# MILAB-IIT-CV/ATDN_vSLAM

Measured on AMD Instinct MI355X. Metric: frame-pairs/sec, KITTI 1241x376 odometry inference at 1/2/4/8 MI355X, higher is better.
Workload: dtype f32 via 3xf16 split MFMA (fp32 accumulate); 1 GPU; KITTI seq-03-shaped 376x1241 uint8 frames (resident in HBM) resized to 376x1232, GMA flow 12 GRU iters + CLVO head -> 6-DoF trajectory (BASELINE configs[1]); streams_per_gpu=2, gru_iters=12, parallelism=pairs sharded x1, one all-gather of 512-d features, replicated LSTM scan

## Files before the change

### atdn_vslam_amd/_lib.py

```python
import ctypes as C
import os

_HERE = os.path.dirname(os.path.abspath(__file__))
LIB_PATH = os.environ.get("ATDN_LIB_PATH") or os.path.join(_HERE, "libatdn_hip.so")

_f32p = C.POINTER(C.c_float)
_i64p = C.POINTER(C.c_int64)
_vp = C.c_void_p

SIGNATURES = {
    "atdn_version": (C.c_int, []),
    "atdn_last_error": (C.c_char_p, []),
    "atdn_gma_create": (C.c_int, [C.POINTER(_vp), C.c_int, C.c_int, C.c_int, C.c_int]),
    "atdn_gma_set_low_latency": (C.c_int, [_vp, C.c_int]),
    "atdn_gma_load": (C.c_int, [_vp, C.c_char_p, _vp, _i64p, C.c_int]),
    "atdn_gma_finalize": (C.c_int, [_vp]),
    "atdn_gma_forward": (C.c_int, [_vp, _vp, _vp, C.c_int, C.c_int, _vp, _vp, _vp, _vp]),
    "atdn_gma_forward_predictions": (C.c_int, [_vp, _vp, _vp, C.c_int, C.c_int, _vp, _vp, _vp]),
    "atdn_gma_forward_sequence": (C.c_int, [_vp, _vp, C.c_int, C.c_int, _vp, _vp, _vp, _vp]),
    "atdn_gma_forward_sequence_continued": (C.c_int, [_vp, _vp, C.c_int, C.c_int, _vp, _vp, _vp, _vp]),
    "atdn_gma_debug_read": (C.c_long, [_vp, C.c_char_p, _vp, C.c_long, _vp]),
    "atdn_gma_profile": (C.c_int, [_vp, C.c_int, C.c_int, C.c_int, _f32p, _vp]),
    "atdn_gma_profile_mode": (C.c_int, [_vp, C.c_int, C.c_int, C.c_int, C.c_int, _f32p, _vp]),
    "atdn_gma_set_range_probe": (C.c_int, [_vp, C.c_int]),
    "atdn_gma_range_rows": (C.c_long, [_vp]),
    "atdn_gma_range_row": (C.c_int, [_vp, C.c_long, C.c_char_p, C.c_int, C.POINTER(C.c_int), C.POINTER(C.c_int), _f32p, _i64p, _i64p]),
    "atdn_range_probe": (C.c_int, [_vp, C.c_int64, C.c_int64, C.c_int64, _f32p, _i64p, _i64p, _vp]),
    "atdn_range_probe_launch": (C.c_int, [_vp, C.c_int64, C.c_int64, C.c_int64, _vp, _vp]),
    "atdn_gma_workspace_bytes": (C.c_size_t, [_vp]),
    "atdn_gma_destroy": (None, [_vp]),
    "atdn_clvo_create": (C.c_int, [C.POINTER(_vp), C.c_int, C.c_int, C.c_int]),
    "atdn_clvo_load": (C.c_int, [_vp, C.c_char_p, _vp, _i64p, C.c_int]),
    "atdn_clvo_finalize": (C.c_int, [_vp]),
    "atdn_clvo_encode": (C.c_int, [_vp, _vp, C.c_int, _vp, _vp]),
    "atdn_clvo_step": (C.c_int, [_vp, _vp, C.c_int, C.c_int, _vp, _vp, _vp, _vp]),
    "atdn_clvo_destroy": (None, [_vp]),
    "atdn_vae_create": (C.c_int, [C.POINTER(_vp), C.c_int, C.c_int, C.c_int]),
    "atdn_vae_load": (C.c_int, [_vp, C.c_char_p, _vp, _i64p, C.c_int]),
    "atdn_vae_finalize": (C.c_int, [_vp]),
    "atdn_vae_embedding_shape": (C.c_int, [_vp, C.POINTER(C.c_int), C.POINTER(C.c_int)]),
    "atdn_vae_encode": (C.c_int, [_vp, _vp, C.c_int, _vp, _vp]),
    "atdn_vae_destroy": (None, [_vp]),
    "atdn_clvo_trainer_create": (C.c_int, [C.POINTER(_vp), C.c_int, C.c_int, C.c_int, C.c_int]),
    "atdn_clvo_trainer_load": (C.c_int, [_vp, C.c_char_p, _vp, _i64p, C.c_int]),
    "atdn_clvo_trainer_finalize": (C.c_int, [_vp]),
    "atdn_clvo_trainer_forward_backward": (C.c_int, [_vp, _vp, _vp, _vp, _vp, _vp, _f32p, _vp]),
    "atdn_clvo_trainer_gradients": (C.c_int, [_vp, C.POINTER(_vp), C.POINTER(C.c_long)]),
    "atdn_clvo_trainer_adamw_step": (C.c_int, [_vp, C.c_float, C.c_float, C.c_float, C.c_int, _vp]),
    "atdn_clvo_trainer_set_loss": (C.c_int, [_vp, C.c_float, C.c_int, C.c_int]),
    "atdn_clvo_trainer_loss_terms": (C.c_int, [_vp, _f32p]),
    "atdn_clvo_loss": (C.c_int, [_vp, _vp, _vp, _vp, C.c_int, C.c_int, C.c_float, C.c_int, C.c_int, _f32p, _vp, _vp, _vp]),
    "atdn_clvo_trainer_read": (C.c_long, [_vp, C.c_char_p, C.c_int, _vp, C.c_long, _vp]),
    "atdn_clvo_trainer_destroy": (None, [_vp]),
    "atdn_pose_transform_f32": (C.c_int, [_vp, _vp, _vp]),
    "atdn_pose_rel2abs": (C.c_int, [_vp, _vp, C.c_int, _vp]),
    "atdn_pose_accumulate_f32": (C.c_int, [_vp, _vp, _vp]),
    "atdn_resize_frames": (C.c_int, [_vp, C.c_int, C.c_int, C.c_int, C.c_int, C.c_int, _vp, _vp]),
    "atdn_resize_frames_mode": (C.c_int, [_vp, C.c_int, C.c_int, C.c_int, C.c_int, C.c_int, C.c_int, _vp, _vp]),
    "atdn_resize_frames_u8": (C.c_int, [_vp, C.c_int, C.c_int, C.c_int, C.c_int, C.c_int, C.c_int, _vp, _vp]),
    "atdn_pad_frames": (C.c_int, [_vp, C.c_int, C.c_int, C.c_int, C.c_int, C.c_int, C.c_int, C.c_int, _vp, _vp]),
    "atdn_ingest_create": (C.c_int, [C.POINTER(_vp), C.c_int, C.c_int, C.c_int, C.c_int, C.c_int, C.c_int]),
    "atdn_ingest_frames_u8": (C.c_int, [_vp, _vp, C.c_int, _vp, _vp]),
    "atdn_ingest_destroy": (None, [_vp]),
    "atdn_flow_pack_f16": (C.c_int, [_vp, C.c_int, C.c_int, C.c_int, C.c_int, C.c_int, _vp, _vp]),
    "atdn_flow_gather_clips": (C.c_int, [_vp, C.c_int, C.c_int, C.c_int, _vp, _vp, C.c_int, C.c_int, _vp, _vp]),
    "atdn_map_search": (C.c_int, [_vp, C.c_int, C.c_int, _vp, C.c_int, C.c_int, _vp, _vp, _vp]),
    "atdn_map_gather_images_u8": (C.c_int, [_vp, C.c_int, C.c_long, _vp, C.c_int, _vp, _vp]),
    "atdn_corr_lookup": (C.c_int, [_vp, _vp, _vp, _vp, C.c_int, C.c_int, C.c_int, _vp, _vp, C.c_int, _vp]),
    "atdn_corr_pyramid": (C.c_int, [_vp, _vp, C.c_int, C.c_int, C.c_int, C.c_int, _vp, _vp, _vp, _vp, _vp]),
    "atdn_corr_lookup_bricks": (C.c_int, [_vp, _vp, C.c_int, C.c_int, C.c_int, C.c_int, _vp, _vp, _vp, _vp, _vp, _vp, _vp, _vp,
                                          _vp, _vp]),
    "atdn_conv2d_nhwc": (C.c_int, [_vp, C.c_int, C.c_int, C.c_int, C.c_int, _vp, _vp, C.c_int, C.c_int, C.c_int,
                                   C.c_int, C.c_int, C.c_int, C.c_int, _vp, _vp]),
    "atdn_conv2d_nhwc_sf": (C.c_int, [_vp, C.c_int, C.c_int, C.c_int, C.c_int, _vp, _vp, C.c_int, C.c_int, C.c_int,
                                      C.c_int, C.c_int, C.c_int, _vp, _vp]),
    "atdn_conv2d_nhwc_sf_epi": (C.c_int, [_vp, C.c_int, C.c_int, C.c_int, C.c_int, _vp, _vp, C.c_int, C.c_int, C.c_int,
                                      C.c_int, C.c_int, C.c_int, C.c_int, _vp, _vp]),
}

GMA_STAGES = ("fnet", "corr", "pool", "cnet", "attention", "lookup", "motion_encoder", "aggregate", "gru_zr", "gru_q",
              "flow_head", "mask", "gru_ctx", "attn_logits", "agg_vt", "convc1", "gru_zr_v", "gru_q_v")

_lib = None


def lib():
    global _lib
    if _lib is None:
        if not os.path.exists(LIB_PATH):
            raise RuntimeError(
                "%s is missing: the HIP extension has not been built (python -m atdn_vslam_amd.build). "
                "There is no CPU fallback for the product path." % LIB_PATH)
        import torch
        handle = C.CDLL(LIB_PATH)
        for name, (res, args) in SIGNATURES.items():
            fn = getattr(handle, name)
            fn.restype = res
            fn.argtypes = args
        _lib = handle
    return _lib


def check(rc):
    if rc != 0:
        raise RuntimeError("libatdn_hip: " + lib().atdn_last_error().decode("utf-8", "replace"))


def load_state(load_fn, handle, state):
    import numpy as np
    import torch
    for key, val in state.items():
        if isinstance(val, torch.Tensor):
            if not val.dtype.is_floating_point:
                continue
            arr = val.detach().to("cpu", torch.float32).contiguous().numpy()
        else:
            arr = np.asarray(val)
            if arr.dtype.kind != "f":
                continue
            arr = np.ascontiguousarray(arr, dtype=np.float32)
        shape = (C.c_int64 * max(arr.ndim, 1))(*arr.shape) if arr.ndim else (C.c_int64 * 1)(1)
        check(load_fn(handle, key.encode(), arr.ctypes.data_as(_vp), shape, arr.ndim))
```

### atdn_vslam_amd/csrc/capi.hip

```cpp
#include "../../include/atdn_hip.h"

#include <cmath>
#include <cstring>

#include "clvo.h"
#include "gma.h"
#include "vae.h"
#include "clvo_train.h"
#include "frontend.h"
#include "conv_sf.h"
#include "epilogues_sf.h"

namespace atdn {
extern template TileChoice conv_dispatch<MODE_TAP, EpiBias<ACT_NONE>>(const ConvShape&, EpiBias<ACT_NONE>, hipStream_t);
extern template TileChoice conv_dispatch<MODE_TAP, EpiBias<ACT_RELU>>(const ConvShape&, EpiBias<ACT_RELU>, hipStream_t);
extern template TileChoice conv_dispatch<MODE_ROW, EpiBias<ACT_NONE>>(const ConvShape&, EpiBias<ACT_NONE>, hipStream_t);
extern template TileChoice conv_dispatch<MODE_ROW, EpiBias<ACT_RELU>>(const ConvShape&, EpiBias<ACT_RELU>, hipStream_t);
extern template TileChoice conv_dispatch<MODE_TAP, EpiScale>(const ConvShape&, EpiScale, hipStream_t);

extern template TileChoice conv_sf_dispatch<EpiBias<ACT_NONE>>(const ConvShape&, float, EpiBias<ACT_NONE>, hipStream_t);
extern template TileChoice conv_sf_dispatch<SfBias<ACT_NONE>>(const ConvShape&, float, SfBias<ACT_NONE>, hipStream_t);

static thread_local std::string g_last_error;
void set_last_error(const std::string& msg) { g_last_error = msg; }
}

using namespace atdn;

struct atdn_gma { GmaNet net; atdn_gma(int H, int W, int B, int prec) : net(H, W, B, prec) {} };
struct atdn_clvo { ClvoNet net; atdn_clvo(int H, int W, int B) : net(H, W, B) {} };
struct atdn_vae { VaeEncoder net; atdn_vae(int H, int W, int B) : net(H, W, B) {} };
struct atdn_ingest { FrameIngest in; atdn_ingest(int a, int b, int c, int d, int n, int aa) : in(a, b, c, d, n, aa) {} };
struct atdn_clvo_trainer { ClvoTrainer net; atdn_clvo_trainer(int H, int W, int B, int T) : net(H, W, B, T) {} };

#define ATDN_API_BEGIN try {
#define ATDN_API_END                                      \
  return 0;                                               \
  } catch (const std::exception& e) {                     \
    set_last_error(e.what());                             \
    return 1;                                             \
  } catch (...) {                                         \
    set_last_error("unknown error");                      \
    return 1;                                             \
  }

template <class T>
static void euler_yxz(const T* r, T* R) {
  const T c1 = std::cos(r[0]), c2 = std::cos(r[1]), c3 = std::cos(r[2]);
  const T s1 = std::sin(r[0]), s2 = std::sin(r[1]), s3 = std::sin(r[2]);
  R[0] = c1 * c3 + s1 * s2 * s3; R[1] = c3 * s1 * s2 - c1 * s3; R[2] = c2 * s1;
  R[3] = c2 * s3;                R[4] = c2 * c3;                R[5] = -s2;
  R[6] = c1 * s2 * s3 - c3 * s1; R[7] = c1 * c3 * s2 + s1 * s3; R[8] = c1 * c2;
}
template <class T>
static void make_transform(const T* rot, const T* tr, T* m) {
  T R[9];
  euler_yxz(rot, R);
  for (int i = 0; i < 3; ++i) { for (int j = 0; j < 3; ++j) m[i * 4 + j] = R[i * 3 + j]; m[i * 4 + 3] = tr[i]; }
  m[12] = 0; m[13] = 0; m[14] = 0; m[15] = 1;
}
template <class T>
static void matmul4(const T* a, const T* b, T* c) {
  for (int i = 0; i < 4; ++i)
    for (int j = 0; j < 4; ++j) {
      T s = 0;
      for (int k = 0; k < 4; ++k) s += a[i * 4 + k] * b[k * 4 + j];
      c[i * 4 + j] = s;
    }
}

extern "C" {

int atdn_version(void) { return 100; }
const char* atdn_last_error(void) { return g_last_error.c_str(); }

int atdn_gma_create(atdn_gma** out, int H, int W, int max_batch, int precision) {
  ATDN_API_BEGIN
  ATDN_CHECK(out, "null out pointer");
  *out = new atdn_gma(H, W, max_batch, precision);
  ATDN_API_END
}
int atdn_gma_set_low_latency(atdn_gma* h, int on) {
  ATDN_API_BEGIN
  ATDN_CHECK(h, "null handle");
  h->net.set_low_latency(on != 0);
  ATDN_API_END
}
int atdn_gma_load(atdn_gma* h, const char* key, const float* data, const int64_t* shape, int rank) {
  ATDN_API_BEGIN
  ATDN_CHECK(h && key && data && rank >= 0 && rank <= 4, "bad state-dict entry");
  h->net.state().put(key, data, shape, rank);
  ATDN_API_END
}
int atdn_gma_finalize(atdn_gma* h) {
  ATDN_API_BEGIN
  ATDN_CHECK(h, "null handle");
  h->net.finalize();
  ATDN_API_END
}
int atdn_gma_forward(atdn_gma* h, const float* im1, const float* im2, int B, int iters, const float* flow_init,
                     float* flow_low, float* flow_up, void* stream) {
  ATDN_API_BEGIN
  ATDN_CHECK(h, "null handle");
  h->net.forward(im1, im2, B, iters, flow_init, flow_low, flow_up, (hipStream_t)stream);
  ATDN_API_END
}
int atdn_gma_forward_predictions(atdn_gma* h, const float* im1, const float* im2, int B, int iters, const float* flow_init,
                                 float* flow_predictions, void* stream) {
  ATDN_API_BEGIN
  ATDN_CHECK(h, "null handle");
  h->net.forward_predictions(im1, im2, B, iters, flow_init, flow_predictions, (hipStream_t)stream);
  ATDN_API_END
}
int atdn_gma_forward_sequence(atdn_gma* h, const float* frames, int B, int iters, const float* flow_init,
                              float* flow_low, float* flow_up, void* stream) {
  ATDN_API_BEGIN
  ATDN_CHECK(h, "null handle");
  h->net.forward_sequence(frames, B, iters, flow_init, flow_low, flow_up, (hipStream_t)stream);
  ATDN_API_END
}
int atdn_gma_forward_sequence_continued(atdn_gma* h, const float* frames, int B, int iters, const float* flow_init,
                                        float* flow_low, float* flow_up, void* stream) {
  ATDN_API_BEGIN
  ATDN_CHECK(h, "null handle");
  h->net.forward_sequence(frames, B, iters, flow_init, flow_low, flow_up, (hipStream_t)stream, true);
  ATDN_API_END
}
long atdn_gma_debug_read(atdn_gma* h, const char* name, float* host, long capacity, void* stream) {
  try {
    if (!h || !name || !host) throw Error("null argument");
    const long n = h->net.debug_read(name, host, capacity, (hipStream_t)stream);
    if (n < 0) throw Error(std::string("unknown tensor name: ") + name);
    return n;
  } catch (const std::exception& e) {
    set_last_error(e.what());
    return -1;
  }
}
int atdn_gma_profile(atdn_gma* h, int B, int iters, int reps, float* ms_out, void* stream) {
  ATDN_API_BEGIN
  ATDN_CHECK(h && ms_out, "null argument");
  static_assert(GmaNet::ST_COUNT == ATDN_GMA_STAGES, "stage table out of sync with the header");
  h->net.profile(B, iters, reps, ms_out, (hipStream_t)stream, 0);
  ATDN_API_END
}
int atdn_gma_profile_mode(atdn_gma* h, int B, int iters, int reps, int mode, float* ms_out, void* stream) {
  ATDN_API_BEGIN
  ATDN_CHECK(h && ms_out, "null argument");
  ATDN_CHECK(mode >= 0 && mode <= 2, "mode must be 0 (pair), 1 (sequence) or 2 (continued sequence)");
  h->net.profile(B, iters, reps, ms_out, (hipStream_t)stream, mode);
  ATDN_API_END
}
int atdn_gma_set_range_probe(atdn_gma* h, int on) {
  ATDN_API_BEGIN
  ATDN_CHECK(h, "null handle");
  h->net.set_probe(on != 0);
  ATDN_API_END
}
long atdn_gma_range_rows(atdn_gma* h) {
  if (!h) { set_last_error("null handle"); return -1; }
  return (long)h->net.probe_rows().size();
}
int atdn_gma_range_row(atdn_gma* h, long index, char* name, int name_capacity, int* iteration, int* limited, float* max_abs,
                       int64_t* over, int64_t* nonfinite) {
// ... 172 lines not shown
  } catch (...) { loss3.release(); throw; }
  loss3.release();
  ATDN_API_END
}
long atdn_clvo_trainer_read(atdn_clvo_trainer* h, const char* key, int kind, float* host, long capacity, void* stream) {
  try {
    ATDN_CHECK(h && key && host, "null argument");
    return h->net.read(key, kind, host, capacity, (hipStream_t)stream);
  } catch (const std::exception& e) {
    set_last_error(e.what());
    return -1;
  }
}
void atdn_clvo_trainer_destroy(atdn_clvo_trainer* h) { delete h; }

int atdn_pose_transform_f32(const float* rot, const float* tr, float* mat16) {
  ATDN_API_BEGIN
  ATDN_CHECK(rot && tr && mat16, "null argument");
  make_transform(rot, tr, mat16);
  ATDN_API_END
}
int atdn_pose_rel2abs(const float* rot, const float* tr, int T, double* poses) {
  ATDN_API_BEGIN
  ATDN_CHECK(rot && tr && poses && T >= 0, "bad argument");
  for (int i = 0; i < 16; ++i) poses[i] = (i % 5 == 0) ? 1.0 : 0.0;
  for (int t = 0; t < T; ++t) {
    const double r[3] = {rot[t * 3], rot[t * 3 + 1], rot[t * 3 + 2]};
    const double x[3] = {tr[t * 3], tr[t * 3 + 1], tr[t * 3 + 2]};
    double m[16];
    make_transform(r, x, m);
    matmul4(poses + (long)t * 16, m, poses + (long)(t + 1) * 16);
  }
  ATDN_API_END
}
int atdn_pose_accumulate_f32(float* pose16, const float* rot, const float* tr) {
  ATDN_API_BEGIN
  ATDN_CHECK(pose16 && rot && tr, "null argument");
  float m[16], o[16];
  make_transform(rot, tr, m);
  matmul4(pose16, m, o);
  for (int i = 0; i < 16; ++i) pose16[i] = o[i];
  ATDN_API_END
}

int atdn_corr_lookup(const float* pyr0, const float* pyr1, const float* pyr2, const float* pyr3, int B, int H8,
                     int W8, const float* coords, float* out, int ldo, void* stream) {
  ATDN_API_BEGIN
  ATDN_CHECK(pyr0 && pyr1 && pyr2 && pyr3 && coords && out && B >= 1, "null argument");
  ATDN_CHECK((H8 >> 3) >= 2 && (W8 >> 3) >= 2, "map too small for four pyramid levels");
  PyramidLevels pl;
  const float* b[4] = {pyr0, pyr1, pyr2, pyr3};
  for (int l = 0; l < 4; ++l) { pl.base[l] = b[l]; pl.H[l] = H8 >> l; pl.W[l] = W8 >> l; }
  launch_lookup(pl, coords, (long)B * H8 * W8, out, ldo, (hipStream_t)stream);
  ATDN_API_END
}

int atdn_corr_pyramid(const float* fmap1, const float* fmap2, int B, int H8, int W8, int C, float* pyr0, float* pyr1,
                      float* pyr2, float* pyr3, void* stream) {
  ATDN_API_BEGIN
  ATDN_CHECK(fmap1 && fmap2 && pyr0 && pyr1 && pyr2 && pyr3 && B >= 1 && C % 32 == 0, "bad argument");
  const int N = H8 * W8;
  ConvShape c;
  c.src0 = fmap1; c.ld0 = C; c.sb0 = (long)N * C; c.C0 = C; c.H = 1; c.W = N;
  c.w = fmap2; c.wb = (long)N * C; c.ldw = C; c.N = N; c.nimg = B;
  conv_dispatch<MODE_TAP>(c, EpiScale{1.0f / sqrtf((float)C), pyr0, (long)N * N, N}, (hipStream_t)stream);
  float* p[4] = {pyr0, pyr1, pyr2, pyr3};
  for (int l = 1; l < 4; ++l) launch_avgpool(p[l - 1], H8 >> (l - 1), W8 >> (l - 1), p[l], (long)B * N, (hipStream_t)stream);
  ATDN_API_END
}

int atdn_corr_lookup_bricks(const float* fmap1, const float* fmap2, int B, int H8, int W8, int C, const float* coords,
                            float* pyr0, float* pyr1, float* pyr2, float* pyr3, float* samples,
                            const float* convc1_weight_host, const float* convc1_bias_host, float* cor1, void* stream) {
  ATDN_API_BEGIN
  ATDN_CHECK(fmap1 && fmap2 && B >= 1 && H8 >= 1 && W8 >= 1, "bad argument");
  ATDN_CHECK(C == 256, "the correlation kernel keeps a source strip's whole K = 256 in registers: C must be 256");
  ATDN_CHECK((H8 >> 3) >= 2 && (W8 >> 3) >= 2, "map too small for four pyramid levels");
  ATDN_CHECK(!(samples || cor1) || coords, "a lookup needs coordinates");
  ATDN_CHECK(!cor1 || (convc1_weight_host && convc1_bias_host), "cor1 needs convc1's weight [256][324] and bias [256]");
  hipStream_t st = (hipStream_t)stream;
  const int N = H8 * W8;
  const long n8 = (long)B * N;
  BrickPyramid bp;
  bp.N = N; bp.NPB = brick_pixel_blocks(N);
  DeviceBuf f1, f2, plain[3], fbrick[4], pyr[4], scratch, outsf;
  DeviceBuf* all[] = {&f1, &f2, &plain[0], &plain[1], &plain[2], &fbrick[0], &fbrick[1], &fbrick[2], &fbrick[3],
                      &pyr[0], &pyr[1], &pyr[2], &pyr[3], &scratch, &outsf};
  WeightArena A;
  try {
    sf_counter_attach();
    f1.alloc(n8 * 256); f2.alloc(n8 * 256);
    launch_to_sf(fmap1, f1.p, n8, 256, st);
    launch_to_sf(fmap2, f2.p, n8, 256, st);
    float* rowmajor[4] = {pyr0, pyr1, pyr2, pyr3};
    int pH[4], pW[4];
    for (int l = 0; l < 4; ++l) {
      pH[l] = H8 >> l; pW[l] = W8 >> l;
      bp.H[l] = pH[l]; bp.W[l] = pW[l]; bp.BW[l] = cdiv(pW[l], 8); bp.BH[l] = cdiv(pH[l], 4); bp.NB[l] = bp.BW[l] * bp.BH[l] * 32;
      const float* src = f2.p;
      long src_sb = (long)N * 256;
      if (l > 0) {
        const float* prev = l == 1 ? f2.p : plain[l - 2].p;
        const long prev_sb = l == 1 ? (long)N * 256 : (long)pH[l - 1] * pW[l - 1] * 256;
        src_sb = (long)pH[l] * pW[l] * 256;
        plain[l - 1].alloc((long)B * src_sb);
        launch_pool_features_sf(prev, B, pH[l - 1], pW[l - 1], 256, prev_sb, plain[l - 1].p, src_sb, st);
        src = plain[l - 1].p;
      }
      fbrick[l].alloc((long)B * bp.NB[l] * 256);
      launch_brick_rows(src, src_sb, B, pH[l], pW[l], 256, fbrick[l].p, (long)bp.NB[l] * 256, st);
      pyr[l].alloc((long)B * bp.NPB * kBrickPixelBlock * bp.NB[l]);
      launch_corr_bricks(f1.p, (long)N * 256, fbrick[l].p, (long)bp.NB[l] * 256, B, N, bp.NB[l], 1.0f / sqrtf(256.0f), pyr[l].p, false, st);
      bp.base[l] = pyr[l].p;
      if (rowmajor[l]) launch_unbrick(pyr[l].p, bp.NB[l], N, pH[l], pW[l], n8, rowmajor[l], st);
    }
    if (samples) {
      outsf.alloc(n8 * 352);
      launch_lookup_bricks(bp, coords, n8, outsf.p, st);
      scratch.alloc(n8 * 352);
      launch_from_sf(outsf.p, scratch.p, n8, 352, st);
      ATDN_HIP(hipMemcpy2DAsync(samples, 324 * sizeof(float), scratch.p, 352 * sizeof(float), 324 * sizeof(float), (size_t)n8,
                                hipMemcpyDeviceToDevice, st));
    }
    if (cor1) {
      StateDict sd;
      const int64_t ws[4] = {256, 324, 1, 1}, bs[1] = {256};
      sd.put("c.weight", convc1_weight_host, ws, 4);
      sd.put("c.bias", convc1_bias_host, bs, 1);
      PackedConv L = pack_conv_sf(A, sd, {"c"});
      pack_fragment_major16(A, L);
      A.upload();
      resolve(A, L);
      DeviceBuf csf;
      csf.alloc(n8 * 256);
      try {
        launch_lookup_conv(bp, coords, n8, nullptr, L.wf16, L.wscale, L.b, csf.p, false, st);
        launch_from_sf(csf.p, cor1, n8, 256, st);
        ATDN_HIP(hipStreamSynchronize(st));
      } catch (...) { csf.release(); throw; }
      csf.release();
    }
    ATDN_HIP(hipStreamSynchronize(st));
  } catch (...) {
    (void)hipDeviceSynchronize();
    for (auto* b : all) b->release();
    A.release();
    throw;
  }
  for (auto* b : all) b->release();
  A.release();
  ATDN_API_END
}

int atdn_conv2d_nhwc(const float* src, int nimg, int H, int W, int Cin, const float* weight_host,
                     const float* bias_host, int Cout, int KH, int KW, int stride, int padH, int padW, int relu,
                     float* dst, void* stream) {
  ATDN_API_BEGIN
  ATDN_CHECK(src && weight_host && dst && nimg >= 1, "null argument");
  const bool row = (Cin == 4 || Cin == 16);
  ATDN_CHECK(row || Cin % 32 == 0, "Cin must be 4, 16 or a multiple of 32");
  StateDict sd;
  const int64_t ws[4] = {Cout, Cin, KH, KW};
  sd.put("c.weight", weight_host, ws, 4);
  std::vector<float> zb(Cout, 0.f);
  const int64_t bs[1] = {Cout};
  sd.put("c.bias", bias_host ? bias_host : zb.data(), bs, 1);
  WeightArena A;
  PackedConv L = pack_conv(A, sd, {"c"}, row ? MODE_ROW : MODE_TAP, Cin);
  A.upload();
  resolve(A, L);
  ConvShape s;
  s.src0 = src; s.ld0 = Cin; s.sb0 = (long)H * W * Cin; s.C0 = L.C; s.H = H; s.W = W;
  s.KH = KH; s.KW = KW; s.stride = stride; s.padH = padH; s.padW = padW;
  s.w = L.w; s.ldw = L.ldw; s.N = Cout; s.nimg = nimg;
  const int Ho = conv_out(H, KH, stride, padH), Wo = conv_out(W, KW, stride, padW);
  hipStream_t st = (hipStream_t)stream;
  try {
    if (row) {
      if (relu) conv_dispatch<MODE_ROW>(s, EpiBias<ACT_RELU>{L.b, dst, (long)Ho * Wo * Cout, Cout, 1.f}, st);
      else conv_dispatch<MODE_ROW>(s, EpiBias<ACT_NONE>{L.b, dst, (long)Ho * Wo * Cout, Cout, 1.f}, st);
    } else {
      if (relu) conv_dispatch<MODE_TAP>(s, EpiBias<ACT_RELU>{L.b, dst, (long)Ho * Wo * Cout, Cout, 1.f}, st);
      else conv_dispatch<MODE_TAP>(s, EpiBias<ACT_NONE>{L.b, dst, (long)Ho * Wo * Cout, Cout, 1.f}, st);
    }
    ATDN_HIP(hipStreamSynchronize(st));
  } catch (...) {
    A.release();
    throw;
  }
  A.release();
  ATDN_API_END
}

int atdn_resize_frames(const float* src, int planes, int Hin, int Win, int Hout, int Wout, float* dst, void* stream) {
  return atdn_resize_frames_mode(src, planes, Hin, Win, Hout, Wout, ATDN_RESIZE_ANTIALIAS, dst, stream);
}
int atdn_resize_frames_mode(const float* src, int planes, int Hin, int Win, int Hout, int Wout, int antialias, float* dst,
                            void* stream) {
  ATDN_API_BEGIN
  ATDN_CHECK(src && dst && planes >= 1 && Hin >= 1 && Win >= 1 && Hout >= 1 && Wout >= 1, "bad argument");
  ATDN_CHECK(antialias == 0 || antialias == 1, "antialias must be ATDN_RESIZE_BILINEAR or ATDN_RESIZE_ANTIALIAS");
  launch_resize<float>(src, planes, Hin, Win, Hout, Wout, antialias, dst, (hipStream_t)stream);
  ATDN_API_END
}
int atdn_resize_frames_u8(const uint8_t* src, int planes, int Hin, int Win, int Hout, int Wout, int antialias, float* dst,
                          void* stream) {
  ATDN_API_BEGIN
  ATDN_CHECK(src && dst && planes >= 1 && Hin >= 1 && Win >= 1 && Hout >= 1 && Wout >= 1, "bad argument");
  ATDN_CHECK(antialias == 0 || antialias == 1, "antialias must be ATDN_RESIZE_BILINEAR or ATDN_RESIZE_ANTIALIAS");
  launch_resize<unsigned char>(src, planes, Hin, Win, Hout, Wout, antialias, dst, (hipStream_t)stream);
  ATDN_API_END
}
int atdn_pad_frames(const float* src, int planes, int H, int W, int left, int right, int top, int bottom, float* dst,
                    void* stream) {
  ATDN_API_BEGIN
  ATDN_CHECK(src && dst && planes >= 1 && H >= 1 && W >= 1 && left >= 0 && right >= 0 && top >= 0 && bottom >= 0, "bad argument");
  launch_pad_replicate(src, planes, H, W, left, right, top, bottom, dst, (hipStream_t)stream);
  ATDN_API_END
}
int atdn_ingest_create(atdn_ingest** out, int Hin, int Win, int Hout, int Wout, int max_frames, int antialias) {
  ATDN_API_BEGIN
  ATDN_CHECK(out, "null out pointer");
  ATDN_CHECK(antialias == 0 || antialias == 1, "antialias must be ATDN_RESIZE_BILINEAR or ATDN_RESIZE_ANTIALIAS");
  *out = new atdn_ingest(Hin, Win, Hout, Wout, max_frames, antialias);
  ATDN_API_END
}
int atdn_ingest_frames_u8(atdn_ingest* h, const uint8_t* host_frames, int n_frames, float* dst, void* stream) {
  ATDN_API_BEGIN
  ATDN_CHECK(h, "null handle");
  h->in.ingest(host_frames, n_frames, dst, (hipStream_t)stream);
  ATDN_API_END
}
void atdn_ingest_destroy(atdn_ingest* h) { delete h; }

int atdn_conv2d_nhwc_sf_epi(const float* src, int nimg, int H, int W, int Cin, const float* weight_host,
                            const float* bias_host, int Cout, int KH, int KW, int stride, int padH, int padW, int sf_store,
                            float* dst, void* stream) {
  ATDN_API_BEGIN
  ATDN_CHECK(src && weight_host && dst && nimg >= 1 && Cin % 32 == 0, "bad argument (Cin must be a multiple of 32)");
  ATDN_CHECK(!sf_store || Cout % 32 == 0, "the split-f16 store needs Cout % 32 == 0");
  StateDict sd;
  const int64_t ws[4] = {Cout, Cin, KH, KW};
  sd.put("c.weight", weight_host, ws, 4);
  std::vector<float> zb(Cout, 0.f);
  const int64_t bs[1] = {Cout};
  sd.put("c.bias", bias_host ? bias_host : zb.data(), bs, 1);
  WeightArena A;
  PackedConv L = pack_conv_sf(A, sd, {"c"});
  A.upload();
  resolve(A, L);
  hipStream_t st = (hipStream_t)stream;
  float* tmp = nullptr;
  const long rows = (long)nimg * H * W;
  ATDN_HIP(hipMalloc(&tmp, (size_t)rows * Cin * sizeof(float)));
  try {
    launch_to_sf(src, tmp, rows, Cin, st);
    ConvShape s;
    s.src0 = tmp; s.ld0 = Cin; s.sb0 = (long)H * W * Cin; s.C0 = L.C; s.H = H; s.W = W;
    s.KH = KH; s.KW = KW; s.stride = stride; s.padH = padH; s.padW = padW;
    s.w = L.w; s.ldw = L.ldw; s.N = Cout; s.nimg = nimg;
    const int Ho = conv_out(H, KH, stride, padH), Wo = conv_out(W, KW, stride, padW);
    s.wfrag16 = L.wf16;
    if (sf_store) {
      float* osf = nullptr;
      const long orows = (long)nimg * Ho * Wo;
      ATDN_HIP(hipMalloc(&osf, (size_t)orows * Cout * sizeof(float)));
      try {
        conv_sf_dispatch(s, L.wscale, SfBias<ACT_NONE>{L.b, osf, (long)Ho * Wo * Cout, Cout}, st);
        launch_from_sf(osf, dst, orows, Cout, st);
        ATDN_HIP(hipStreamSynchronize(st));
      } catch (...) {
        (void)hipFree(osf);
        throw;
      }
      (void)hipFree(osf);
    } else {
      conv_sf_dispatch(s, L.wscale, EpiBias<ACT_NONE>{L.b, dst, (long)Ho * Wo * Cout, Cout, 1.f}, st);
      ATDN_HIP(hipStreamSynchronize(st));
    }
  } catch (...) {
    (void)hipFree(tmp);
    A.release();
    throw;
  }
  (void)hipFree(tmp);
  A.release();
  ATDN_API_END
}

int atdn_conv2d_nhwc_sf(const float* src, int nimg, int H, int W, int Cin, const float* weight_host,
                        const float* bias_host, int Cout, int KH, int KW, int stride, int padH, int padW, float* dst,
                        void* stream) {
  return atdn_conv2d_nhwc_sf_epi(src, nimg, H, W, Cin, weight_host, bias_host, Cout, KH, KW, stride, padH, padW, 0, dst, stream);
}

}
```

### atdn_vslam_amd/csrc/conv_sf6.h

```cpp
#pragma once
#include <cstdlib>
#include <type_traits>
#include "conv_sf.h"

namespace atdn {

struct Conv2Geom {
  const float* src0; const float* src1;
  long sb0, sb1;
  int ld0, ld1, C0, C1;
  int H, W, Ho, Wo;
  int KH, KW, padH, padW;
  int PH, PW;
  int tiles_x, tiles_y;
  int nimg, ntile_n;
  const float* w; int ldw; int N;
  float wscale;
  const float* in_mean; const float* in_rstd;
};

inline bool conv_halo_eligible(const ConvShape& s) {
  if (s.stride != 1 || s.wb != 0) return false;
  return (s.KH == 3 && s.KW == 3) || (s.KH == 1 && s.KW == 5) || (s.KH == 5 && s.KW == 1);
}

template <class E, class = void> struct epi_gen6 : std::integral_constant<int, 0> {};
template <class E> struct epi_gen6<E, std::void_t<decltype(E::kGen6)>> : std::integral_constant<int, E::kGen6> {};
template <class E, class = void> struct EpiAux4 { struct type {}; };
template <class E> struct EpiAux4<E, std::void_t<typename E::Aux4>> { using type = typename E::Aux4; };
template <class E, class = void> struct epi_flowhead : std::false_type {};
template <class E> struct epi_flowhead<E, std::void_t<decltype(E::kFlowHead)>> : std::bool_constant<E::kFlowHead> {};
template <class E, class = void> struct epi_ring3 : std::false_type {};
template <class E> struct epi_ring3<E, std::void_t<decltype(E::kRing3)>> : std::bool_constant<E::kRing3> {};
template <class E, class = void> struct epi_rawacc : std::false_type {};
template <class E> struct epi_rawacc<E, std::void_t<decltype(E::kRawAcc)>> : std::bool_constant<E::kRawAcc> {};
template <class E, class = void> struct epi_vec4 : std::false_type {};
template <class E> struct epi_vec4<E, std::void_t<decltype(E::kVec4)>> : std::bool_constant<E::kVec4> {};

typedef float f32x4v __attribute__((ext_vector_type(4)));
struct SfAcc { f32x4v b[2][2]; };

#ifdef ATDN_CONV_STAMP
#define ATDN_CONV_STAMP_SLOTS 4096
extern __device__ unsigned long long atdn_conv_stamps_dev[4][ATDN_CONV_STAMP_SLOTS][12];
template <class E> struct conv_stamp_kind : std::integral_constant<int, -1> {};
#endif

template <int TH, int TW, int BN, int WM, int WN, int KH, int KW, class Epi, bool FAST = false, bool NORM = false, int ABL = 0>
__device__ __forceinline__ void conv_sf6_body(const Conv2Geom& g, const Epi& ep, const int bidx) {
  static_assert(ABL == 0 || !NORM, "ablation builds exist for the plain patch loader");
  static_assert(TW == 16, "the 16x16x32 loop is built for 16-pixel tile rows");
  constexpr int NIMG = 2;
  constexpr int NW = WM * WN, NT = NW * 64;
  constexpr int TM = TH * TW / 32 / WM, TN = BN / 32 / WN;
  static_assert(TM * WM * 32 == TH * TW && TN * WN * 32 == BN, "wave grid must tile the block");
  static_assert(32 % TW == 0 || TW % 32 == 0, "a 32-pixel MFMA row tile must cover whole tile rows");
  constexpr int NTAP = KH * KW;
  constexpr int RSTEP = NT / 8;
  constexpr int PROWS = (TH + KH - 1) * (TW + KW - 1);
  constexpr int PW = TW + KW - 1;
  constexpr int NP = (PROWS + RSTEP - 1) / RSTEP;
  constexpr int ROWB = 160;
  constexpr int RS = PW * ROWB;
  constexpr bool SWAP = epi_vec4<Epi>::value;
  constexpr int PSZ = (TH + KH - 1) * RS;
  __shared__ __attribute__((aligned(256))) char Pbytes[NIMG * PSZ];

  const int tid = threadIdx.x;
  const int tiles_img = g.tiles_x * g.tiles_y;
  const int nblk = g.nimg * tiles_img * g.ntile_n;
  const int id = xcd_remap(bidx, nblk);
  const int tile_n = id % g.ntile_n;
  const int tmg = id / g.ntile_n;
  const int img = tmg / tiles_img;
  const int tloc = tmg - img * tiles_img;
  const int ty0 = (tloc / g.tiles_x) * TH, tx0 = (tloc % g.tiles_x) * TW;
  const int n0 = tile_n * BN;
  const int lane = tid & 63, wave = tid >> 6;
#ifdef ATDN_CONV_STAMP
  constexpr int kStamp = conv_stamp_kind<Epi>::value;
  unsigned long long st_r0 = 0, st_t0 = 0, st_t1 = 0, st_t2 = 0, st_bar = 0;
  unsigned long long st_e_slab = 0, st_e_wait = 0, st_e_apply = 0;
  if constexpr (kStamp >= 0) { st_r0 = __builtin_amdgcn_s_memrealtime(); st_t0 = __builtin_amdgcn_s_memtime(); }
#endif

  const int jrow = (tid >> 3) & 7;
  const int s = tid & 7, r0 = !NORM ? tid >> 3 : ((tid >> 6) << 3) + 2 * (jrow & 1) + ((jrow >> 1) & 1) + 4 * (jrow >> 2);
  static_assert((TH + KH - 1) * RS / 16 <= 4096, "LDS offset field");
  unsigned pmeta[NP];
#pragma unroll
  for (int k = 0; k < NP; ++k) {
    const int prow = r0 + RSTEP * k;
    unsigned off = 0;
    const int py = prow / PW, px = prow - py * PW;
    if (prow < PROWS) {
      const int iy = ty0 - g.padH + py, ix = tx0 - g.padW + px;
      if ((unsigned)iy < (unsigned)g.H && (unsigned)ix < (unsigned)g.W) off = (unsigned)(iy * g.W + ix) + 1u;
    }
    pmeta[k] = (off << 12) | (unsigned)((py * RS + px * ROWB + 16 * s) >> 4);
    if (prow >= PROWS) pmeta[k] = pmeta[0];
  }
  const float* s0 = g.src0 + (long)img * g.sb0;
  const float* s1 = g.src1 ? g.src1 + (long)img * g.sb1 : nullptr;
  const int nck = (g.C0 + g.C1) >> 5;

  float4 pr[NP];
  auto fetch_patch = [&](int c) {
    const int cc = c << 5;
    const float* sp; int ld, co;
    if (cc < g.C0) { sp = s0; ld = g.ld0; co = cc; } else { sp = s1; ld = g.ld1; co = cc - g.C0; }
#pragma unroll
    for (int k = 0; k < NP; ++k)
      pr[k] = *reinterpret_cast<const float4*>(sp + (long)((pmeta[k] >> 12) ? (pmeta[k] >> 12) - 1 : 0) * ld + co + 4 * s);
  };
  auto store_patch = [&](int buf) {
#pragma unroll
    for (int k = 0; k < NP; ++k)
      *reinterpret_cast<float4*>(Pbytes + buf * PSZ + ((pmeta[k] & 0xFFFu) << 4)) = keep_if((pmeta[k] >> 12) != 0, pr[k]);
  };
  float4 nmu = make_float4(0.f, 0.f, 0.f, 0.f), nrs = make_float4(1.f, 1.f, 1.f, 1.f);
  auto fetch_norm = [&](int c) {
    nmu = *reinterpret_cast<const float4*>(g.in_mean + (long)img * g.C0 + (c << 5) + 4 * s);
    nrs = *reinterpret_cast<const float4*>(g.in_rstd + (long)img * g.C0 + (c << 5) + 4 * s);
  };
  bool norm_sat = false;
  auto store_row_norm = [&](int buf, int k, float4 mu, float4 rs) {
    const float hi = (pmeta[k] >> 12) != 0 ? 65504.f : 0.f;
    float4 v = pr[k];
    v.x = (v.x - mu.x) * rs.x; v.y = (v.y - mu.y) * rs.y; v.z = (v.z - mu.z) * rs.z; v.w = (v.w - mu.w) * rs.w;
    const float m = fmaxf(fmaxf(v.x, v.y), fmaxf(v.z, v.w));
    norm_sat |= !(m <= 65504.f);
    v.x = __builtin_amdgcn_fmed3f(v.x, 0.f, hi); v.y = __builtin_amdgcn_fmed3f(v.y, 0.f, hi);
    v.z = __builtin_amdgcn_fmed3f(v.z, 0.f, hi); v.w = __builtin_amdgcn_fmed3f(v.w, 0.f, hi);
    const unsigned h0 = sf_cvt_pk_(v.x, v.y), h1 = sf_cvt_pk_(v.z, v.w);
    const unsigned l0 = sf_residual_pk_(h0, v.x, v.y), l1 = sf_residual_pk_(h1, v.z, v.w);
    char* px = Pbytes + buf * PSZ + (((pmeta[k] & 0xFFFu) - (unsigned)s) << 4);
    *reinterpret_cast<uint2*>(px + 8 * s) = make_uint2(h0, h1);
    *reinterpret_cast<uint2*>(px + 64 + 8 * s) = make_uint2(l0, l1);
  };

  const int wm = wave / WN, wn = wave % WN;
  SfAcc acc[TM][TN];
#pragma unroll
  for (int i = 0; i < TM; ++i)
#pragma unroll
    for (int j = 0; j < TN; ++j) {
#pragma unroll
      for (int e = 0; e < 16; ++e) acc[i][j].b[e >> 3][(e >> 2) & 1][e & 3] = 0.f;
    }
  {
    const int n16 = lane & 15, g16 = lane >> 4;
    int a_off[TM];
#pragma unroll
    for (int i = 0; i < TM; ++i) a_off[i] = ((wm * TM + i) * 2) * RS + n16 * ROWB + 16 * g16;
    const char* Pb = Pbytes;
    const int nblk16 = (g.N + 15) >> 4;
    const float* wrow[TN][2];
#pragma unroll
    for (int j = 0; j < TN; ++j)
#pragma unroll
      for (int cb = 0; cb < 2; ++cb)
        wrow[j][cb] = g.w + (long)min(((n0 >> 4) + (wn * TN + j) * 2 + cb), nblk16 - 1) * (NTAP * nck) * 512 + lane * 4;
    constexpr int RT = (NTAP % 3 == 0 || epi_ring3<Epi>::value) ? 3 : 2;
    constexpr int CU = (NTAP % RT == 0) ? 1 : RT;
    constexpr int NS = CU * NTAP;
    static_assert(NS % RT == 0, "ring size must divide the K steps of an unrolled iteration");
    struct WFrag { f16x8 hi[TN][2], lo[TN][2]; };
    WFrag wr[RT];
    auto load_w = [&](WFrag& f, int c0, int st, int cb) __attribute__((always_inline)) {
      const int cc = min(c0 + st / NTAP, nck - 1);
      const int q = (st % NTAP) * nck + cc;
#pragma unroll
      for (int j = 0; j < TN; ++j) {
        f.hi[j][cb] = *reinterpret_cast<const f16x8*>(wrow[j][cb] + (long)q * 512);
        if constexpr (!FAST) f.lo[j][cb] = *reinterpret_cast<const f16x8*>(wrow[j][cb] + (long)q * 512 + 256);
      }
    };
    fetch_patch(0);
    if constexpr (NORM) fetch_norm(0);
#pragma unroll
    for (int st = 0; st < RT - 1; ++st) { load_w(wr[st], 0, st, 0); load_w(wr[st], 0, st, 1); }
    if constexpr ((ABL & 1) != 0) { load_w(wr[RT - 1], 0, RT - 1, 0); load_w(wr[RT - 1], 0, RT - 1, 1); }
    if constexpr (NORM) {
#pragma unroll
      for (int k = 0; k < NP; ++k) store_row_norm(0, k, nmu, nrs);
    } else {
      store_patch(0);
    }
    __syncthreads();
#ifdef ATDN_CONV_STAMP
    if constexpr (kStamp >= 0) st_t1 = __builtin_amdgcn_s_memtime();
#endif
    f16x8 ah[2][TM], al[2][TM];
    auto read_a = [&](int half, int tap) __attribute__((always_inline)) {
      const char* arow = Pb + (tap / KW + half) * RS + (tap % KW) * ROWB;
#pragma unroll
      for (int i = 0; i < TM; ++i) {
        ah[half][i] = *reinterpret_cast<const f16x8*>(arow + a_off[i]);
        if constexpr (!FAST) al[half][i] = *reinterpret_cast<const f16x8*>(arow + a_off[i] + 64);
      }
    };
    auto mfma_half = [&](int half, const WFrag& w) __attribute__((always_inline)) {
#pragma unroll
      for (int i = 0; i < TM; ++i)
#pragma unroll
        for (int j = 0; j < TN; ++j)
#pragma unroll
          for (int cb = 0; cb < 2; ++cb) {
            f32x4v c = acc[i][j].b[half][cb];
            if constexpr (SWAP) {
              if constexpr (!FAST) {
                c = __builtin_amdgcn_mfma_f32_16x16x32_f16(w.hi[j][cb], al[half][i], c, 0, 0, 0);
                c = __builtin_amdgcn_mfma_f32_16x16x32_f16(w.lo[j][cb], ah[half][i], c, 0, 0, 0);
              }
              c = __builtin_amdgcn_mfma_f32_16x16x32_f16(w.hi[j][cb], ah[half][i], c, 0, 0, 0);
            } else {
              if constexpr (!FAST) {
                c = __builtin_amdgcn_mfma_f32_16x16x32_f16(al[half][i], w.hi[j][cb], c, 0, 0, 0);
                c = __builtin_amdgcn_mfma_f32_16x16x32_f16(ah[half][i], w.lo[j][cb], c, 0, 0, 0);
              }
              c = __builtin_amdgcn_mfma_f32_16x16x32_f16(ah[half][i], w.hi[j][cb], c, 0, 0, 0);
            }
            acc[i][j].b[half][cb] = c;
          }
    };
    constexpr int NMF = (FAST ? 1 : 3) * TM * TN * 2;
    constexpr int NH = 2 * NTAP;
    static_assert(!NORM || NH - 1 - NP >= 1, "normalise-on-load spreads its NP patch rows over the half-steps of a chunk");
    read_a(0, 0);
    if constexpr (KH != 3 || !Epi::kStats) __builtin_amdgcn_s_setprio(2);
    for (int c0 = 0; c0 < nck; c0 += CU) {
#pragma unroll
      for (int cu = 0; cu < CU; ++cu) {
        const int c = c0 + cu;
        const bool live = CU == 1 || c < nck;
        const int cn = min(c + 1, nck - 1);
#pragma unroll
        for (int hs = 0; hs < NH; ++hs) {
          const int tap = hs >> 1, half = hs & 1;
          const int st = cu * NTAP + tap;
          __builtin_amdgcn_sched_barrier(0);
          if (!(ABL & 2) && hs == 0) { fetch_patch(cn); if constexpr (NORM) fetch_norm(cn); }
          if (!(ABL & 1)) {
            if (RT == 2) { if (half == 0) { load_w(wr[(st + 1) % RT], c0, st + 1, 0); load_w(wr[(st + 1) % RT], c0, st + 1, 1); } }
            else load_w(wr[(st + RT - 1) % RT], c0, st + RT - 1, half);
          }
          if (!(ABL & 4) && hs + 1 < NH) read_a((hs + 1) & 1, (hs + 1) >> 1);
          if constexpr (NORM) {
            if (hs >= NH - 1 - NP && hs <= NH - 2) store_row_norm((c + 1) & 1, hs - (NH - 1 - NP), nmu, nrs);
          } else {
            if (!(ABL & 2) && hs == NH - 2) store_patch((c + 1) & 1);
          }
          if (live) mfma_half(half, wr[st % RT]);
          {
            constexpr int nds = 2 * TM;
            const int nvm = (RT == 2 ? (half == 0 ? 4 * TN : 0) : 2 * TN) + (hs == 0 ? NP : 0);
            const int ndw = NORM ? ((hs >= NH - 1 - NP && hs <= NH - 2) ? 2 : 0) : ((hs == NH - 2) ? NP : 0);
#pragma unroll
            for (int k = 0; k < NMF; ++k) {
              __builtin_amdgcn_sched_group_barrier(0x008, 1, 0);
              if (hs + 1 < NH && k < nds) __builtin_amdgcn_sched_group_barrier(0x100, 1, 0);
              else if (k - ((hs + 1 < NH) ? nds : 0) < nvm) __builtin_amdgcn_sched_group_barrier(0x020, 1, 0);
              else if (k - ((hs + 1 < NH) ? nds : 0) - nvm < ndw) __builtin_amdgcn_sched_group_barrier(0x200, 1, 0);
            }
          }
        }
        if (!(ABL & 2)) {
#ifdef ATDN_CONV_STAMP
          unsigned long long st_b0 = 0;
          if constexpr (kStamp >= 0) { asm volatile("s_waitcnt lgkmcnt(0)" ::: "memory"); st_b0 = __builtin_amdgcn_s_memtime(); }
#endif
          asm volatile("s_waitcnt lgkmcnt(0)\n\ts_barrier" ::: "memory");
#ifdef ATDN_CONV_STAMP
          if constexpr (kStamp >= 0) st_bar += __builtin_amdgcn_s_memtime() - st_b0;
#endif
          Pb = Pbytes + ((c + 1) & 1) * PSZ;
        }
        if (!(ABL & 4)) read_a(0, 0);
      }
    }
  }

#ifdef ATDN_CONV_STAMP
  if constexpr (kStamp >= 0) st_t2 = __builtin_amdgcn_s_memtime();
  auto stamp_out = [&]() __attribute__((always_inline)) {
    if constexpr (kStamp >= 0) {
      asm volatile("s_waitcnt vmcnt(0) lgkmcnt(0)" ::: "memory");
      const unsigned long long t3 = __builtin_amdgcn_s_memtime(), r1 = __builtin_amdgcn_s_memrealtime();
      const unsigned hw = __builtin_amdgcn_s_getreg((31 << 11) | 4), xcc = __builtin_amdgcn_s_getreg((31 << 11) | 20);
      if (wave == 0 && lane == 0 && bidx < ATDN_CONV_STAMP_SLOTS) {
        unsigned long long* o = atdn_conv_stamps_dev[kStamp * 2 + (KH == 5 ? 1 : 0)][bidx];
        o[0] = st_r0; o[1] = r1; o[2] = st_t1 - st_t0; o[3] = st_t2 - st_t1; o[4] = st_bar; o[5] = t3 - st_t2;
        o[6] = ((unsigned long long)xcc << 32) | hw; o[7] = t3 - st_t0;
        o[8] = st_e_slab; o[9] = st_e_wait; o[10] = st_e_apply; o[11] = 0;
      }
    }
  };
#endif
  if constexpr (KH != 3 || !Epi::kStats) __builtin_amdgcn_s_setprio(0);
  if constexpr (NORM) sf_report(norm_sat);
  if constexpr ((ABL & 8) != 0) {
    float tot = 0.f;
#pragma unroll
    for (int i = 0; i < TM; ++i)
#pragma unroll
      for (int j = 0; j < TN; ++j)
#pragma unroll
        for (int e = 0; e < 16; ++e) tot += acc[i][j].b[e >> 3][(e >> 2) & 1][e & 3];
    if (tot == 1.2345e-30f) ep(img, 0, 0, tot);
    return;
  }
  if constexpr (SWAP) {
    static_assert(NW * 32 * LDS_LD * 4 <= NIMG * PSZ, "transpose slabs must fit in the patch images");
    __syncthreads();
    float* tb = reinterpret_cast<float*>(Pbytes) + wave * (32 * LDS_LD);
    const int trow = lane >> 3, tcol = (lane & 7) * 4;
    auto tile_pixel = [&](int i, int q) {
      const int p = (wm * TM + i) * 32 + 8 * q + trow;
      const int oy = ty0 + p / TW, ox = tx0 + p % TW;
      if constexpr ((ABL & 16) != 0) return p;
      return (oy < g.Ho && ox < g.Wo) ? oy * g.Wo + ox : -1;
    };
    constexpr bool RAW = epi_rawacc<Epi>::value && !epi_flowhead<Epi>::value;
    auto slab_write = [&](const SfAcc& a) __attribute__((always_inline)) {
      const float sc = RAW ? 1.0f : g.wscale;
#pragma unroll
      for (int hh = 0; hh < 2; ++hh)
#pragma unroll
        for (int cb = 0; cb < 2; ++cb)
          *reinterpret_cast<float4*>(tb + (16 * hh + (lane & 15)) * LDS_LD + 16 * cb + 4 * (lane >> 4)) =
              RAW ? make_float4(a.b[hh][cb][0], a.b[hh][cb][1], a.b[hh][cb][2], a.b[hh][cb][3])
                  : make_float4(a.b[hh][cb][0] * sc, a.b[hh][cb][1] * sc, a.b[hh][cb][2] * sc, a.b[hh][cb][3] * sc);
    };
    if constexpr (epi_flowhead<Epi>::value) {
      static_assert(!epi_flowhead<Epi>::value || (WM == 1 && TN == 1 && TW == 16), "one block holds all output channels of its pixels");
      constexpr int RP = 20;
      static_assert(32 * RP <= 32 * LDS_LD, "the exchange rows live inside the wave's slab");
      {
        const int n16 = lane & 15, g16 = lane >> 4;
        const int c8 = n0 + wn * 32 + 8 * g16;
        const float4 bq0 = *reinterpret_cast<const float4*>(ep.bias + c8), bq1 = *reinterpret_cast<const float4*>(ep.bias + c8 + 4);
        const float b8[8] = {bq0.x, bq0.y, bq0.z, bq0.w, bq1.x, bq1.y, bq1.z, bq1.w};
        f16x8 w2h[2], w2l[2];
#pragma unroll
        for (int rbk = 0; rbk < 2; ++rbk) {
          const int u = 16 * rbk + n16;
          const float* wr = ep.w2 + (long)min(u, 17) * g.N + c8;
          const float4 wa = *reinterpret_cast<const float4*>(wr), wb = *reinterpret_cast<const float4*>(wr + 4);
          const float w8[8] = {wa.x, wa.y, wa.z, wa.w, wb.x, wb.y, wb.z, wb.w};
#pragma unroll
          for (int e = 0; e < 8; ++e) {
            const float w = u < 18 ? w8[e] * ep.w2mul : 0.f;
            w2h[rbk][e] = (_Float16)w;
            w2l[rbk][e] = (_Float16)(w - (float)w2h[rbk][e]);
          }
        }
        bool sat = false;
#pragma unroll
        for (int i = 0; i < TM; ++i) {
          slab_write(acc[i][0]);
          asm volatile("s_waitcnt lgkmcnt(0)" ::: "memory");
          __builtin_amdgcn_wave_barrier();
          f16x8 xh[2], xl[2];
#pragma unroll
          for (int pb = 0; pb < 2; ++pb) {
            const float* src = tb + (16 * pb + n16) * LDS_LD + 8 * g16;
            const float4 xa = *reinterpret_cast<const float4*>(src), xb = *reinterpret_cast<const float4*>(src + 4);
            const float x8[8] = {xa.x, xa.y, xa.z, xa.w, xb.x, xb.y, xb.z, xb.w};
#pragma unroll
            for (int e = 0; e < 8; ++e) {
              const SfPair sp = sf_split_flag(fmaxf(x8[e] + b8[e], 0.f), sat);
              xh[pb][e] = sp.hi; xl[pb][e] = sp.lo;
            }
          }
          asm volatile("s_waitcnt lgkmcnt(0)" ::: "memory");
          __builtin_amdgcn_wave_barrier();
#pragma unroll
          for (int pb = 0; pb < 2; ++pb) {
            f32x4v d0 = {0.f, 0.f, 0.f, 0.f}, d1 = {0.f, 0.f, 0.f, 0.f};
            if constexpr (!FAST) {
              d0 = __builtin_amdgcn_mfma_f32_16x16x32_f16(w2h[0], xl[pb], d0, 0, 0, 0);
              d0 = __builtin_amdgcn_mfma_f32_16x16x32_f16(w2l[0], xh[pb], d0, 0, 0, 0);
              d1 = __builtin_amdgcn_mfma_f32_16x16x32_f16(w2h[1], xl[pb], d1, 0, 0, 0);
              d1 = __builtin_amdgcn_mfma_f32_16x16x32_f16(w2l[1], xh[pb], d1, 0, 0, 0);
            }
            d0 = __builtin_amdgcn_mfma_f32_16x16x32_f16(w2h[0], xh[pb], d0, 0, 0, 0);
            d1 = __builtin_amdgcn_mfma_f32_16x16x32_f16(w2h[1], xh[pb], d1, 0, 0, 0);
            float* rp = tb + (16 * pb + n16) * RP;
            *reinterpret_cast<float4*>(rp + 4 * g16) = make_float4(d0[0] * ep.w2inv, d0[1] * ep.w2inv, d0[2] * ep.w2inv, d0[3] * ep.w2inv);
            if (g16 == 0) *reinterpret_cast<float2*>(rp + 16) = make_float2(d1[0] * ep.w2inv, d1[1] * ep.w2inv);
          }
          __syncthreads();
          for (int idx = tid; idx < 32 * 18; idx += NT) {
            const int px = idx / 18, u = idx - px * 18;
            const float* rq = reinterpret_cast<const float*>(Pbytes) + px * RP + u;
            float sum = 0.f;
#pragma unroll
            for (int w = 0; w < NW; ++w) sum += rq[w * (32 * LDS_LD)];
            const int p = i * 32 + px;
            const int oy = ty0 + p / TW, ox = tx0 + p % TW;
            if (oy < g.Ho && ox < g.Wo)
              ep.G[(long)(n0 / (NW * 32)) * ep.gstride + ((long)img * ep.npix + (long)oy * g.Wo + ox) * 18 + u] = sum;
          }
          __syncthreads();
// ... 430 lines not shown
```

### atdn_vslam_amd/csrc/gma.h

```cpp
#pragma once
#include <vector>
#include <map>
#include <memory>

#include "attention.h"
#include "conv_dispatch.h"
#include "kernels.h"
#include "range_probe.h"
#include "weights.h"

namespace atdn {

struct EncoderWeights {
  PackedConv stem;
  struct Block { PackedConv c1, c2, ds; bool has_ds = false; } blk[6];
  PackedConv head;
};

class DeviceBuf {
 public:
  float* p = nullptr;
  long n = 0;
  void alloc(long count) {
    n = count;
    ATDN_HIP(hipMalloc(&p, (size_t)count * sizeof(float)));
  }
  void release() { if (p) { (void)hipFree(p); p = nullptr; } }
};

class GmaNet {
 public:
  GmaNet(int H, int W, int max_batch, int precision);
  ~GmaNet();
  StateDict& state() { return sd_; }
  void finalize();
  void forward(const float* im1, const float* im2, int B, int iters, const float* flow_init, float* flow_low,
               float* flow_up, hipStream_t st);
  void forward_predictions(const float* im1, const float* im2, int B, int iters, const float* flow_init, float* preds,
                           hipStream_t st);
  void forward_sequence(const float* frames, int B, int iters, const float* flow_init, float* flow_low, float* flow_up,
                        hipStream_t st, bool continued = false);
  long debug_read(const char* name, float* host, long capacity, hipStream_t st);
  size_t workspace_bytes() const { return ws_bytes_; }
  enum Stage { ST_FNET = 0, ST_CORR, ST_POOL, ST_CNET, ST_ATTN, ST_LOOKUP, ST_MOTION, ST_AGG, ST_GRU_ZR, ST_GRU_Q, ST_FLOWHEAD,
               ST_MASK, ST_GRU_CTX, ST_ATTN_LOGITS, ST_AGG_VT, ST_CONVC1, ST_GRU_ZR_V, ST_GRU_Q_V, ST_COUNT };
  void profile(int B, int iters, int reps, float* ms, hipStream_t st, int mode = 0);

  int H, W, H8, W8, N, ldN, maxB, precision;
  int dev_ = 0;
  bool norm_on_load_ = false;
  bool classic_ = false;
  bool low_latency_ = false;
  void set_low_latency(bool on);
  DeviceBuf attn_part_;
  DeviceBuf enc2_[4];
  hipStream_t par_stream_ = nullptr;
  std::vector<hipEvent_t> par_events_;
  size_t par_next_ = 0;
  bool par_ = false;
  bool par_ok_ = true;
  void fork(hipStream_t from, hipStream_t to);
  DeviceBuf fbrick_[4], fplain_[3], coords_used_;
  int brickBW_[4], brickBH_[4], brickNB_[4];
  BrickPyramid brick_pyramid() const;
  DeviceBuf rowmax_, rinv_;

  struct ProbeRow { std::string name; int iter; bool limited; float max_abs; long long over, nonfinite; };
  static constexpr int kProbeMaxRows = 1536;
  void set_probe(bool on);
  const std::vector<ProbeRow>& probe_rows() const { return probe_rows_; }

 private:
  bool probe_ = false;
  int probe_it_ = -1;
  RangeSlot* probe_slots_ = nullptr;
  std::vector<ProbeRow> probe_rows_;
  void probe_begin(hipStream_t st);
  void probe_end(hipStream_t st);
  void probe(const std::string& name, bool limited, const float* p, long rows, long cols, long ld, hipStream_t st);
  void run_body(int B, int iters, hipStream_t st);
  void run_encoder(const EncoderWeights& E, bool instance, int nimg, hipStream_t st, float** out_buf, int* outH,
                   int* outW);
  void iteration(int B, hipStream_t st);
  void run_body_sf(int B, int iters, hipStream_t st);
  void run_encoder_sf(const EncoderWeights& E, bool instance, int nimg, hipStream_t st, float** out_buf, int first_img = 0,
                      DeviceBuf* bufs = nullptr);
  void iteration_sf(int B, hipStream_t st);
  void capture(int B, int iters);
  void launch_body(int B, int iters, hipStream_t st);
  int seq_ = 0;
  int last_frame_ = -1;
  float* preds_out_ = nullptr;
  long preds_stride_ = 0;
  void mask_head_sf(int B, hipStream_t st);
  void mask_head(int B, hipStream_t st);
  int last_B_ = 0;

  StateDict sd_;
  WeightArena arena_;
  bool ready_ = false;
  bool use_graph_ = true;
  EncoderWeights fnet_, cnet_;
  PackedConv convc1_, convc2_, convf1_, convf2_, convm_, to_v_, to_qk_;
  long convf1_sf_off_ = -1;
  float convf1_wscale_ = 1.f;
  float fh2_mul_ = 1.f;
  long fh2_w32_off_ = -1;
  DeviceBuf fhG_;
  PackedConv gru_zr_[2], gru_q_[2], fh1_, fh2_, mask0_, mask2_;
  PackedConv gru_zr_ctx_[2], gru_q_ctx_[2];
  const float* gamma_ = nullptr;
  long gamma_off_ = -1;

  DeviceBuf img4_, enc_[4], scratch_, pcnt_, fin_, fmap_, psum_, pm2_, mean_[3], rstd_[3];
  DeviceBuf pyr_[4], h_[2], x_, qk_, attn_, vT_, corrfeat_, cor1_, corflo_, flo1_, z_, rh_, fh_, mask_;
  DeviceBuf coords1_, flow4_, pre_zr_[2], pre_q_[2];
  int pyrH_[4], pyrW_[4];
  size_t ws_bytes_ = 0;

  struct Timer;
  Timer* timer_ = nullptr;
  void mark(int stage, hipStream_t st);

  hipStream_t cap_stream_ = nullptr;
  std::map<std::pair<int, int>, hipGraphExec_t> graphs_;
};

}
```

### atdn_vslam_amd/csrc/gma.hip

```cpp
#include "gma.h"
#include "small_convs.h"
#include "conv_sf.h"
#include "epilogues_sf.h"

namespace atdn { const float* zero_line(); }

namespace atdn {

extern template TileChoice conv_dispatch<MODE_TAP, EpiBias<ACT_NONE>>(const ConvShape&, EpiBias<ACT_NONE>, hipStream_t);
extern template TileChoice conv_dispatch<MODE_TAP, EpiBias<ACT_RELU>>(const ConvShape&, EpiBias<ACT_RELU>, hipStream_t);
extern template TileChoice conv_dispatch<MODE_ROW, EpiBias<ACT_RELU>>(const ConvShape&, EpiBias<ACT_RELU>, hipStream_t);
extern template TileChoice conv_dispatch<MODE_TAP, EpiBiasStats>(const ConvShape&, EpiBiasStats, hipStream_t);
extern template TileChoice conv_dispatch<MODE_ROW, EpiBiasStats>(const ConvShape&, EpiBiasStats, hipStream_t);
extern template TileChoice conv_dispatch<MODE_TAP, EpiBiasReluAddRelu>(const ConvShape&, EpiBiasReluAddRelu, hipStream_t);
extern template TileChoice conv_dispatch<MODE_TAP, EpiContextSplit>(const ConvShape&, EpiContextSplit, hipStream_t);
extern template TileChoice conv_dispatch<MODE_TAP, EpiScale>(const ConvShape&, EpiScale, hipStream_t);
extern template TileChoice conv_dispatch<MODE_TAP, EpiQK>(const ConvShape&, EpiQK, hipStream_t);
extern template TileChoice conv_dispatch<MODE_TAP, EpiStoreT>(const ConvShape&, EpiStoreT, hipStream_t);
extern template TileChoice conv_dispatch<MODE_TAP, EpiAggregate>(const ConvShape&, EpiAggregate, hipStream_t);
extern template TileChoice conv_dispatch<MODE_TAP, EpiGruZR>(const ConvShape&, EpiGruZR, hipStream_t);
extern template TileChoice conv_dispatch<MODE_TAP, EpiGruQ>(const ConvShape&, EpiGruQ, hipStream_t);
extern template TileChoice conv_dispatch<MODE_TAP, EpiFlowDelta>(const ConvShape&, EpiFlowDelta, hipStream_t);

extern template TileChoice conv_dispatch<MODE_ROW, SfBias<ACT_RELU>>(const ConvShape&, SfBias<ACT_RELU>, hipStream_t);
#define ATDN_EXTERN_SF(EPI) extern template TileChoice conv_sf_dispatch<EPI>(const ConvShape&, float, EPI, hipStream_t);
ATDN_EXTERN_SF(SfBias<ACT_NONE>) ATDN_EXTERN_SF(SfBias<ACT_RELU>) ATDN_EXTERN_SF(EpiBias<ACT_NONE>)
ATDN_EXTERN_SF(EpiBiasStats) ATDN_EXTERN_SF(SfBiasReluAddRelu) ATDN_EXTERN_SF(SfContextSplit)
ATDN_EXTERN_SF(SfQK) ATDN_EXTERN_SF(SfVT)
ATDN_EXTERN_SF(SfGruZR) ATDN_EXTERN_SF(SfGruQ)
extern template void conv_sf_dispatch_pair<SfBias<ACT_RELU>>(const ConvShape&, float, SfBias<ACT_RELU>, const ConvShape&, float,
                                                             SfBias<ACT_RELU>, hipStream_t);

namespace {

struct FastGuard {
  bool prev;
  explicit FastGuard(bool on) : prev(sf_fast_mode()) { sf_fast_mode() = on; }
  ~FastGuard() { sf_fast_mode() = prev; }
};

constexpr int XLD = 384;
constexpr int CORR_LD = 352;

ConvShape conv_shape(const PackedConv& L, const float* src, int ld, long sb, int nimg, int H, int W, int stride,
                     int padH, int padW) {
  ConvShape s;
  s.src0 = src; s.ld0 = ld; s.sb0 = sb; s.C0 = L.C;
  s.H = H; s.W = W; s.KH = L.KH; s.KW = L.KW; s.stride = stride; s.padH = padH; s.padW = padW;
  s.w = L.w; s.wfrag16 = L.wf16; s.ldw = L.ldw; s.N = L.N; s.nimg = nimg;
  return s;
}

EncoderWeights pack_encoder(WeightArena& A, const StateDict& sd, const std::string& p, bool batchnorm, bool sf) {
  EncoderWeights E;
  auto fold = [&](const std::string& norm) { return bn_affine(sd, norm); };
  auto pack_conv = [&](WeightArena& A_, const StateDict& sd_, const std::vector<std::string>& names, int mode, int cpix,
                       const ChannelAffine* f = nullptr) {
    return (sf && mode == MODE_TAP) ? pack_conv_sf(A_, sd_, names, f) : atdn::pack_conv(A_, sd_, names, mode, cpix, f);
  };
  if (batchnorm) { auto a = fold(p + "norm1"); E.stem = pack_conv(A, sd, {p + "conv1"}, MODE_ROW, 4, &a); }
  else E.stem = pack_conv(A, sd, {p + "conv1"}, MODE_ROW, 4);
  if (sf) pack_stem_sf(A, E.stem);
  int bi = 0;
  for (int li = 1; li <= 3; ++li)
    for (int k = 0; k < 2; ++k, ++bi) {
      const std::string q = p + "layer" + std::to_string(li) + "." + std::to_string(k) + ".";
      auto& B = E.blk[bi];
      B.has_ds = (li > 1 && k == 0);
      if (batchnorm) {
        auto a1 = fold(q + "norm1"), a2 = fold(q + "norm2");
        B.c1 = pack_conv(A, sd, {q + "conv1"}, MODE_TAP, 0, &a1);
        B.c2 = pack_conv(A, sd, {q + "conv2"}, MODE_TAP, 0, &a2);
        if (B.has_ds) { auto a3 = fold(q + "norm3"); B.ds = pack_conv(A, sd, {q + "downsample.0"}, MODE_TAP, 0, &a3); }
      } else {
        B.c1 = pack_conv(A, sd, {q + "conv1"}, MODE_TAP, 0);
        B.c2 = pack_conv(A, sd, {q + "conv2"}, MODE_TAP, 0);
        if (B.has_ds) B.ds = pack_conv(A, sd, {q + "downsample.0"}, MODE_TAP, 0);
      }
    }
  E.head = pack_conv(A, sd, {p + "conv2"}, MODE_TAP, 0);
  return E;
}

void resolve_encoder(const WeightArena& A, EncoderWeights& E) {
  resolve(A, E.stem);
  for (auto& b : E.blk) { resolve(A, b.c1); resolve(A, b.c2); if (b.has_ds) resolve(A, b.ds); }
  resolve(A, E.head);
}

}

struct GmaNet::Timer {
  std::vector<std::pair<int, hipEvent_t>> marks;
  hipEvent_t start = nullptr;
};

void GmaNet::mark(int stage, hipStream_t st) {
  if (!timer_) return;
  hipEvent_t e;
  ATDN_HIP(hipEventCreate(&e));
  ATDN_HIP(hipEventRecord(e, st));
  timer_->marks.emplace_back(stage, e);
}

void GmaNet::profile(int B, int iters, int reps, float* ms, hipStream_t st, int mode) {
  ATDN_CHECK(ready_ && B >= 1 && B <= maxB && reps >= 1, "bad profile request");
  ATDN_CHECK(mode == 0 || precision >= 1, "sequence modes are built for the split-f16 pipeline");
  ATDN_CHECK(!probe_, "switch the range probe off before profiling: its launches would be timed with the stages");
  for (int i = 0; i < ST_COUNT; ++i) ms[i] = 0.f;
  seq_ = mode;
  last_frame_ = 0;
  for (int r = 0; r < reps; ++r) {
    Timer t;
    timer_ = &t;
    if (precision >= 1) launch_init_coords_sf(nullptr, B, H8, W8, coords1_.p, flow4_.p, x_.p, XLD, 254, st);
    else launch_init_coords(nullptr, B, H8, W8, coords1_.p, flow4_.p, x_.p + 254, XLD, st);
    ATDN_HIP(hipEventCreate(&t.start));
    ATDN_HIP(hipEventRecord(t.start, st));
    try { if (precision >= 1) { FastGuard fg(precision == 2); run_body_sf(B, iters, st); } else run_body(B, iters, st); } catch (...) { timer_ = nullptr; throw; }
    timer_ = nullptr;
    ATDN_HIP(hipStreamSynchronize(st));
    hipEvent_t prev = t.start;
    for (auto& m : t.marks) {
      float d = 0.f;
      ATDN_HIP(hipEventElapsedTime(&d, prev, m.second));
      ms[m.first] += d;
      prev = m.second;
    }
    for (auto& m : t.marks) (void)hipEventDestroy(m.second);
    (void)hipEventDestroy(t.start);
  }
}

GmaNet::GmaNet(int H_, int W_, int max_batch, int precision_) : H(H_), W(W_), maxB(max_batch), precision(precision_) {
  ATDN_CHECK(precision >= 0 && precision <= 2, "precision must be 0 (fp32 MFMA), 1 (split-f16 MFMA) or 2 (plain f16 MFMA)");
  ATDN_CHECK(H % 8 == 0 && W % 8 == 0 && H >= 64 && W >= 64, "frame size must be a multiple of 8 (use the padder)");
  ATDN_CHECK(max_batch >= 1 && max_batch <= 64, "max_batch out of range");
  H8 = H / 8; W8 = W / 8; N = H8 * W8; ldN = round_up(N, 32);
  norm_on_load_ = precision == 1;
  classic_ = precision == 0;
  const char* ng = getenv("ATDN_NO_GRAPH");
  use_graph_ = !(ng && ng[0] == '1');
  (void)hipGetDevice(&dev_);
}

void GmaNet::fork(hipStream_t from, hipStream_t to) {
  ATDN_CHECK(par_next_ < par_events_.size(), "out of branch events");
  hipEvent_t e = par_events_[par_next_++];
  ATDN_HIP(hipEventRecord(e, from));
  ATDN_HIP(hipStreamWaitEvent(to, e, 0));
}

void GmaNet::set_low_latency(bool on) {
  ATDN_CHECK(!ready_, "set_low_latency: call it before finalize() (the workspace and the captured graphs depend on it)");
  low_latency_ = on;
}

GmaNet::~GmaNet() {
  DeviceGuard dg(dev_);
  (void)hipDeviceSynchronize();
  for (auto& kv : graphs_) (void)hipGraphExecDestroy(kv.second);
  if (cap_stream_) (void)hipStreamDestroy(cap_stream_);
  if (par_stream_) (void)hipStreamDestroy(par_stream_);
  for (auto& e : par_events_) (void)hipEventDestroy(e);
  DeviceBuf* all[] = {&img4_, &enc_[0], &enc_[1], &enc_[2], &enc_[3], &scratch_, &pcnt_, &fin_, &fmap_, &psum_, &pm2_, &mean_[0], &mean_[1], &mean_[2], &rstd_[0],
                      &rstd_[1], &rstd_[2], &pyr_[0], &pyr_[1], &pyr_[2], &pyr_[3], &h_[0], &h_[1], &x_, &qk_, &attn_, &vT_,
                      &corrfeat_, &cor1_, &corflo_, &flo1_, &z_, &rh_, &fh_, &mask_, &coords1_, &flow4_, &pre_zr_[0],
                      &pre_zr_[1], &pre_q_[0], &pre_q_[1], &rowmax_, &rinv_,
                      &fbrick_[0], &fbrick_[1], &fbrick_[2], &fbrick_[3], &fplain_[0], &fplain_[1], &fplain_[2], &coords_used_, &fhG_,
                      &attn_part_, &enc2_[0], &enc2_[1], &enc2_[2], &enc2_[3]};
  for (auto* b : all) b->release();
  if (probe_slots_) (void)hipFree(probe_slots_);
  arena_.release();
}

void GmaNet::set_probe(bool on) {
  ATDN_CHECK(!on || precision == 0,
             "the range probe needs an exact-fp32 handle (ATDN_PRECISION_F32): only that path writes every intermediate tensor "
             "as plain fp32 and never clamps; the split-f16 / f16 paths store range-limited values and fuse some tensors away");
  probe_ = on;
}

void GmaNet::probe_begin(hipStream_t st) {
  if (!probe_slots_) ATDN_HIP(hipMalloc(&probe_slots_, kProbeMaxRows * sizeof(RangeSlot)));
  ATDN_HIP(hipMemsetAsync(probe_slots_, 0, kProbeMaxRows * sizeof(RangeSlot), st));
  probe_rows_.clear();
  probe_it_ = -1;
}

void GmaNet::probe(const std::string& name, bool limited, const float* p, long rows, long cols, long ld, hipStream_t st) {
  ATDN_CHECK((int)probe_rows_.size() < kProbeMaxRows, "range probe: slot table full");
  launch_range_probe(p, rows, cols, ld, probe_slots_ + probe_rows_.size(), st);
  probe_rows_.push_back({name, probe_it_, limited, 0.f, 0, 0});
}

void GmaNet::probe_end(hipStream_t st) {
  std::vector<RangeSlot> host(probe_rows_.size());
  if (!host.empty())
    ATDN_HIP(hipMemcpyAsync(host.data(), probe_slots_, host.size() * sizeof(RangeSlot), hipMemcpyDeviceToHost, st));
  ATDN_HIP(hipStreamSynchronize(st));
  for (size_t i = 0; i < host.size(); ++i) {
    ProbeRow& r = probe_rows_[i];
    static_assert(sizeof(float) == sizeof(unsigned int), "fp32");
    memcpy(&r.max_abs, &host[i].max_bits, sizeof(float));
    r.over = (long long)host[i].over;
    r.nonfinite = (long long)host[i].nonfinite;
  }
}

void GmaNet::finalize() {
  ATDN_CHECK(!ready_, "finalize called twice");
  const std::string u = "update_block.";
  const bool sf = precision >= 1;
  auto tap = [&](const std::vector<std::string>& names, bool has_bias = true) {
    return sf ? pack_conv_sf(arena_, sd_, names, nullptr, has_bias)
              : pack_conv(arena_, sd_, names, MODE_TAP, 0, nullptr, has_bias);
  };
  fnet_ = pack_encoder(arena_, sd_, "fnet.", false, sf);
  cnet_ = pack_encoder(arena_, sd_, "cnet.", true, sf);
  convc1_ = tap({u + "encoder.convc1"});
  if (sf) pack_fragment_major16(arena_, convc1_);
  convc2_ = tap({u + "encoder.convc2"});
  convf1_ = pack_conv(arena_, sd_, {u + "encoder.convf1"}, MODE_ROW, 4);
  {
    const HostTensor& w = sd_.get(u + "encoder.convf1.weight");
    ATDN_CHECK(w.shape[0] == 128 && w.shape[1] == 2 && w.shape[2] == 7 && w.shape[3] == 7, "convf1 is 7x7, 2 -> 128");
    float mx = 0.f;
    for (float v : w.data) mx = std::max(mx, std::fabs(v));
    int e = 0;
    if (mx > 0.f) (void)std::frexp(mx, &e);
    const int p = 1 - e;
    convf1_wscale_ = std::ldexp(1.0f, -p);
    convf1_sf_off_ = arena_.alloc(4L * 2 * 4 * 2 * 64 * 4);
    _Float16* f = reinterpret_cast<_Float16*>(arena_.at(convf1_sf_off_));
    for (int wv = 0; wv < 4; ++wv)
      for (int cb = 0; cb < 2; ++cb)
        for (int s = 0; s < 4; ++s)
          for (int lane = 0; lane < 64; ++lane)
            for (int i = 0; i < 8; ++i) {
              const int n = 32 * wv + 16 * cb + (lane & 15), g = lane >> 4;
              const int ky = 2 * s + (g >> 1), kx = 4 * (g & 1) + (i >> 1), c = i & 1;
              const float v = (ky < 7 && kx < 7) ? std::ldexp(w.data[(((long)n * 2 + c) * 7 + ky) * 7 + kx], p) : 0.f;
              const _Float16 hi = (_Float16)v, lo = (_Float16)(v - (float)hi);
              const long frag = (((long)wv * 2 + cb) * 4 + s) * 2;
              f[(frag * 64 + lane) * 8 + i] = hi;
              f[((frag + 1) * 64 + lane) * 8 + i] = lo;
            }
  }
  convf2_ = tap({u + "encoder.convf2"});
  convm_ = tap({u + "encoder.conv"});
  to_v_ = tap({u + "aggregator.to_v"}, false);
  to_qk_ = tap({"att.to_qk"}, false);
  for (int p = 0; p < 2; ++p) {
    const std::string t = std::to_string(p + 1);
    if (sf) {
      const std::vector<std::pair<int, int>> rest = {{0, 128}, {256, 512}}, ctx = {{128, 256}};
      gru_zr_[p] = pack_conv_sf_channels(arena_, sd_, {u + "gru.convz" + t, u + "gru.convr" + t}, rest, true);
      gru_q_[p] = pack_conv_sf_channels(arena_, sd_, {u + "gru.convq" + t}, rest, true);
      gru_zr_ctx_[p] = pack_conv_sf_channels(arena_, sd_, {u + "gru.convz" + t, u + "gru.convr" + t}, ctx, false);
      gru_q_ctx_[p] = pack_conv_sf_channels(arena_, sd_, {u + "gru.convq" + t}, ctx, false);
    } else {
      gru_zr_[p] = tap({u + "gru.convz" + t, u + "gru.convr" + t});
      gru_q_[p] = tap({u + "gru.convq" + t});
    }
  }
  fh1_ = tap({u + "flow_head.conv1"});
  fh2_ = tap({u + "flow_head.conv2"});
  if (sf) {
    const HostTensor& w = sd_.get(u + "flow_head.conv2.weight");
    ATDN_CHECK(w.shape.size() == 4 && w.shape[0] == 2 && w.shape[1] == 256 && w.shape[2] == 3 && w.shape[3] == 3, "flow head conv2 shape");
    fh2_w32_off_ = arena_.alloc(18 * 256);
    for (int o = 0; o < 2; ++o)
      for (int c = 0; c < 256; ++c)
        for (int t = 0; t < 9; ++t) arena_.at(fh2_w32_off_)[(t * 2 + o) * 256 + c] = w.data[((long)o * 256 + c) * 9 + t];
    float mx = 0.f;
    for (float v : w.data) mx = std::max(mx, std::fabs(v));
    int e = 0;
    if (mx > 0.f) (void)std::frexp(mx, &e);
    fh2_mul_ = std::ldexp(1.0f, 1 - e);
  }
  mask0_ = tap({u + "mask.0"});
  mask2_ = tap({u + "mask.2"});
  gamma_off_ = pack_vector(arena_, sd_.get(u + "aggregator.gamma").data);
  arena_.upload();
  resolve_encoder(arena_, fnet_);
  resolve_encoder(arena_, cnet_);
  for (PackedConv* L : {&convc1_, &convc2_, &convf1_, &convf2_, &convm_, &to_v_, &to_qk_, &gru_zr_[0], &gru_zr_[1],
                        &gru_q_[0], &gru_q_[1], &fh1_, &fh2_, &mask0_, &mask2_})
    resolve(arena_, *L);
  if (sf) for (PackedConv* L : {&gru_zr_ctx_[0], &gru_zr_ctx_[1], &gru_q_ctx_[0], &gru_q_ctx_[1]}) resolve(arena_, *L);
  gamma_ = arena_.dev(gamma_off_);

  const int B = maxB;
  const int H2 = conv_out(H, 7, 2, 3), W2 = conv_out(W, 7, 2, 3);
  const long n8 = (long)B * N;
  img4_.alloc(2L * B * H * W * 4);
  for (int i = 0; i < (sf ? 4 : 3); ++i) enc_[i].alloc(2L * B * H2 * W2 * 64);
  fmap_.alloc(2L * B * N * 256);
  const long groups = (long)cdiv(H2 * W2, 64) * 4 + 8;
  psum_.alloc(2L * B * groups * 128); pm2_.alloc(2L * B * groups * 128); pcnt_.alloc(2L * B * groups); fin_.alloc(2L * B * 32 * 128 * 4 * 2);
  for (int i = 0; i < 3; ++i) { mean_[i].alloc(2L * B * 128); rstd_[i].alloc(2L * B * 128); }
  pyrH_[0] = H8; pyrW_[0] = W8;
  for (int l = 1; l < 4; ++l) { pyrH_[l] = pyrH_[l - 1] / 2; pyrW_[l] = pyrW_[l - 1] / 2; }
  ATDN_CHECK(pyrH_[3] >= 2 && pyrW_[3] >= 2, "frame too small for a 4-level pyramid");
  for (int l = 0; l < 4; ++l) {
    brickBW_[l] = cdiv(pyrW_[l], 8); brickBH_[l] = cdiv(pyrH_[l], 4); brickNB_[l] = brickBW_[l] * brickBH_[l] * 32;
    pyr_[l].alloc(classic_ ? n8 * pyrH_[l] * pyrW_[l] : (long)B * brick_pixel_blocks(N) * kBrickPixelBlock * brickNB_[l]);
  }
  if (sf) {
    for (int l = 0; l < 4; ++l) fbrick_[l].alloc((long)B * brickNB_[l] * 256);
    for (int l = 1; l < 4; ++l) fplain_[l - 1].alloc((long)B * pyrH_[l] * pyrW_[l] * 256);
    coords_used_.alloc(n8 * 2);
  }
  h_[0].alloc(n8 * 128); h_[1].alloc(n8 * 128); x_.alloc(n8 * XLD);
  const AttnGeom ag = attn_geom(B, N, ldN);
  qk_.alloc(n8 * 256); attn_.alloc(std::max(n8 * ldN, attn_floats(ag))); vT_.alloc((long)B * 128 * ldN);
  if (sf) { rowmax_.alloc((long)B * ag.Npad); rinv_.alloc((long)B * ag.Npad); }
  if (sf && low_latency_ && attn_v_splits(attn_geom(1, N, ldN)) > 1) attn_part_.alloc(8L * B * ag.Npad * 128);
  if (sf && low_latency_) {
    for (int i = 0; i < 4; ++i) enc2_[i].alloc((long)B * H2 * W2 * 64);
    ATDN_HIP(hipStreamCreateWithFlags(&par_stream_, hipStreamNonBlocking));
    par_events_.resize(2 * (1 + 64));
    for (auto& e : par_events_) ATDN_HIP(hipEventCreateWithFlags(&e, hipEventDisableTiming));
  }
  corrfeat_.alloc(n8 * CORR_LD); cor1_.alloc(n8 * 256); corflo_.alloc(n8 * 256); flo1_.alloc(n8 * 128);
  z_.alloc(n8 * 128); rh_.alloc(n8 * 128); fh_.alloc(n8 * 256); mask_.alloc(n8 * 576);
  if (sf) fhG_.alloc(2 * n8 * 18);
  coords1_.alloc(n8 * 2); flow4_.alloc(n8 * 4);
  if (sf) for (int p = 0; p < 2; ++p) { pre_zr_[p].alloc(n8 * 256); pre_q_[p].alloc(n8 * 128); }
  ATDN_HIP(hipMemset(corrfeat_.p, 0, corrfeat_.n * sizeof(float)));
  ATDN_HIP(hipMemset(vT_.p, 0, vT_.n * sizeof(float)));
  ATDN_HIP(hipMemset(attn_.p, 0, attn_.n * sizeof(float)));
  ATDN_HIP(hipMemset(flow4_.p, 0, flow4_.n * sizeof(float)));
  ATDN_HIP(hipDeviceSynchronize());
  ws_bytes_ = 0;
  DeviceBuf* all[] = {&img4_, &enc_[0], &enc_[1], &enc_[2], &enc_[3], &fmap_, &psum_, &pm2_, &pyr_[0], &pyr_[1], &pyr_[2],
                      &pyr_[3], &h_[0], &h_[1], &x_, &qk_, &attn_, &vT_, &corrfeat_, &cor1_, &corflo_, &flo1_, &z_,
                      &rh_, &fh_, &mask_, &coords1_, &flow4_};
  for (auto* b : all) ws_bytes_ += (size_t)b->n * sizeof(float);
  (void)zero_line();
  sf_counter_attach();
  ATDN_HIP(hipStreamCreateWithFlags(&cap_stream_, hipStreamNonBlocking));
  ready_ = true;
}

void GmaNet::run_encoder(const EncoderWeights& E, bool instance, int nimg, hipStream_t st, float** out_buf, int* outH,
                         int* outW) {
  int h = conv_out(H, 7, 2, 3), w = conv_out(W, 7, 2, 3);
  float* P = enc_[0].p; float* Q = enc_[1].p; float* R = enc_[2].p;
  auto stats_conv = [&](auto mode_tag, const PackedConv& L, const float* src, int ld, int ih, int iw, int stride,
                        int pad, float* dst, int slot) {
    constexpr int MODE = decltype(mode_tag)::value;
    ConvShape s = conv_shape(L, src, ld, (long)ih * iw * ld, nimg, ih, iw, stride, pad, pad);
    const int oh = conv_out(ih, L.KH, stride, pad), ow = conv_out(iw, L.KW, stride, pad);
    EpiBiasStats ep{L.b, dst, (long)oh * ow * L.N, L.N, psum_.p, pm2_.p, 0};
    TileChoice t = conv_dispatch<MODE>(s, ep, st);
    const int groups = cdiv(oh * ow, t.BM) * (t.BM / 32);
    ATDN_CHECK((long)nimg * groups * L.N <= psum_.n, "statistics scratch too small");
    launch_in_finalize_cnt(psum_.p, pm2_.p, nullptr, nimg, groups, oh * ow, L.N, 1e-5f, mean_[slot].p, rstd_[slot].p,
                           reinterpret_cast<double*>(fin_.p), st);
  };
  using TapT = std::integral_constant<int, MODE_TAP>;
  using RowT = std::integral_constant<int, MODE_ROW>;
  auto pr = [&](int bi, const char* leaf, bool limited, const float* p, long pixels, int ch) {
    if (!probe_) return;
    std::string name = instance ? "fnet." : "cnet.";
    if (bi >= 0) name += "layer" + std::to_string(bi / 2 + 1) + "." + std::to_string(bi % 2);
    probe(name + leaf, limited, p, (long)nimg * pixels, ch, ch, st);
  };

  if (instance) {
    stats_conv(RowT{}, E.stem, img4_.p, 4, H, W, 2, 3, P, 0);
    pr(-1, "conv1.raw", false, P, (long)h * w, 64);
    launch_in_apply(P, mean_[0].p, rstd_[0].p, nullptr, nullptr, nullptr, nimg, (long)h * w, 64, st);
  } else {
    ConvShape s = conv_shape(E.stem, img4_.p, 4, (long)H * W * 4, nimg, H, W, 2, 3, 3);
    conv_dispatch<MODE_ROW>(s, EpiBias<ACT_RELU>{E.stem.b, P, (long)h * w * 64, 64, 1.f}, st);
  }
  pr(-1, "conv1.out", true, P, (long)h * w, 64);
  int c = 64;
  for (int bi = 0; bi < 6; ++bi) {
    const auto& Bk = E.blk[bi];
    const int stride = Bk.has_ds ? 2 : 1;
    const int co = Bk.c1.N;
    const int oh = conv_out(h, 3, stride, 1), ow = conv_out(w, 3, stride, 1);
    const long ohw = (long)oh * ow;
    if (instance) {
      stats_conv(TapT{}, Bk.c1, P, c, h, w, stride, 1, Q, 0);
      pr(bi, ".conv1.raw", false, Q, ohw, co);
      launch_in_apply(Q, mean_[0].p, rstd_[0].p, nullptr, nullptr, nullptr, nimg, ohw, co, st);
      pr(bi, ".conv1.out", true, Q, ohw, co);
      stats_conv(TapT{}, Bk.c2, Q, co, oh, ow, 1, 1, R, 0);
      pr(bi, ".conv2.raw", false, R, ohw, co);
      if (Bk.has_ds) {
        stats_conv(TapT{}, Bk.ds, P, c, h, w, 2, 0, Q, 1);
        pr(bi, ".downsample.raw", false, Q, ohw, co);
        launch_in_apply(R, mean_[0].p, rstd_[0].p, Q, mean_[1].p, rstd_[1].p, nimg, ohw, co, st);
      } else {
        launch_in_apply(R, mean_[0].p, rstd_[0].p, P, nullptr, nullptr, nimg, ohw, co, st);
      }
      std::swap(P, R);
    } else {
      ConvShape s1 = conv_shape(Bk.c1, P, c, (long)h * w * c, nimg, h, w, stride, 1, 1);
      conv_dispatch<MODE_TAP>(s1, EpiBias<ACT_RELU>{Bk.c1.b, Q, ohw * co, co, 1.f}, st);
      pr(bi, ".conv1.out", true, Q, ohw, co);
      ConvShape s2 = conv_shape(Bk.c2, Q, co, ohw * co, nimg, oh, ow, 1, 1, 1);
      if (Bk.has_ds) {
        ConvShape sd = conv_shape(Bk.ds, P, c, (long)h * w * c, nimg, h, w, 2, 0, 0);
        conv_dispatch<MODE_TAP>(sd, EpiBias<ACT_NONE>{Bk.ds.b, R, ohw * co, co, 1.f}, st);
        pr(bi, ".downsample.out", true, R, ohw, co);
        conv_dispatch<MODE_TAP>(s2, EpiBiasReluAddRelu{Bk.c2.b, R, ohw * co, co, P, ohw * co, co}, st);
      } else {
        conv_dispatch<MODE_TAP>(s2, EpiBiasReluAddRelu{Bk.c2.b, P, ohw * co, co, R, ohw * co, co}, st);
        std::swap(P, R);
      }
    }
    pr(bi, "", true, P, ohw, co);
    h = oh; w = ow; c = co;
  }
  *out_buf = P; *outH = h; *outW = w;
}

void GmaNet::iteration(int B, hipStream_t st) {
  const long n8 = (long)B * N;
  PyramidLevels pl;
  for (int l = 0; l < 4; ++l) { pl.base[l] = pyr_[l].p; pl.H[l] = pyrH_[l]; pl.W[l] = pyrW_[l]; }
  launch_lookup(pl, coords1_.p, n8, corrfeat_.p, CORR_LD, st);
  mark(ST_LOOKUP, st);
  auto pr = [&](const char* name, bool limited, const float* p, long rows, long cols, long ld) {
    if (probe_) probe(name, limited, p, rows, cols, ld, st);
  };
  pr("corr_lookup", true, corrfeat_.p, n8, 324, CORR_LD);

  ConvShape s = conv_shape(convc1_, corrfeat_.p, CORR_LD, (long)N * CORR_LD, B, H8, W8, 1, 0, 0);
  conv_dispatch<MODE_TAP>(s, EpiBias<ACT_RELU>{convc1_.b, cor1_.p, (long)N * 256, 256, 1.f}, st);
  mark(ST_CONVC1, st);
  pr("encoder.convc1", true, cor1_.p, n8, 256, 256);
  s = conv_shape(convc2_, cor1_.p, 256, (long)N * 256, B, H8, W8, 1, 1, 1);
  conv_dispatch<MODE_TAP>(s, EpiBias<ACT_RELU>{convc2_.b, corflo_.p, (long)N * 256, 256, 1.f}, st);
  pr("encoder.convc2", true, corflo_.p, n8, convc2_.N, 256);
  s = conv_shape(convf1_, flow4_.p, 4, (long)N * 4, B, H8, W8, 1, 3, 3);
  conv_dispatch<MODE_ROW>(s, EpiBias<ACT_RELU>{convf1_.b, flo1_.p, (long)N * 128, 128, 1.f}, st);
  pr("encoder.convf1", true, flo1_.p, n8, 128, 128);
  s = conv_shape(convf2_, flo1_.p, 128, (long)N * 128, B, H8, W8, 1, 1, 1);
  conv_dispatch<MODE_TAP>(s, EpiBias<ACT_RELU>{convf2_.b, corflo_.p + 192, (long)N * 256, 256, 1.f}, st);
  pr("encoder.convf2", true, corflo_.p + 192, n8, convf2_.N, 256);
  s = conv_shape(convm_, corflo_.p, 256, (long)N * 256, B, H8, W8, 1, 1, 1);
  float* mf = x_.p + 128;
  conv_dispatch<MODE_TAP>(s, EpiBias<ACT_RELU>{convm_.b, mf, (long)N * XLD, XLD, 1.f}, st);
  mark(ST_MOTION, st);
  pr("encoder.conv", true, mf, n8, convm_.N, XLD);

  s = conv_shape(to_v_, mf, XLD, (long)N * XLD, B, H8, W8, 1, 0, 0);
  conv_dispatch<MODE_TAP>(s, EpiStoreT{vT_.p, (long)128 * ldN, ldN}, st);
  mark(ST_AGG_VT, st);
  pr("aggregator.to_v", true, vT_.p, (long)B * 128, N, ldN);
  ConvShape a;
  a.src0 = attn_.p; a.ld0 = ldN; a.sb0 = (long)N * ldN; a.C0 = ldN; a.H = 1; a.W = N;
  a.w = vT_.p; a.wb = (long)128 * ldN; a.ldw = ldN; a.N = 128; a.nimg = B;
  conv_dispatch<MODE_TAP>(a, EpiAggregate{gamma_, mf, (long)N * XLD, XLD, x_.p + 256, (long)N * XLD, XLD}, st);
  mark(ST_AGG, st);
  pr("aggregator.out", true, x_.p + 256, n8, 128, XLD);

  for (int p = 0; p < 2; ++p) {
    const float* hin = h_[p].p;
    float* hout = h_[p ^ 1].p;
    const int ph = p ? 2 : 0, pw = p ? 0 : 2;
    ConvShape g = conv_shape(gru_zr_[p], hin, 128, (long)N * 128, B, H8, W8, 1, ph, pw);
    g.C0 = 128; g.src1 = x_.p; g.ld1 = XLD; g.sb1 = (long)N * XLD; g.C1 = XLD;
    conv_dispatch<MODE_TAP>(g, EpiGruZR{gru_zr_[p].b, hin, z_.p, rh_.p, (long)N * 128}, st);
    mark(p ? ST_GRU_ZR_V : ST_GRU_ZR, st);
    pr(p ? "gru.z2" : "gru.z1", false, z_.p, n8, 128, 128);
    pr(p ? "gru.rh2" : "gru.rh1", true, rh_.p, n8, 128, 128);
    g.src0 = rh_.p; g.w = gru_q_[p].w; g.ldw = gru_q_[p].ldw; g.N = gru_q_[p].N;
    conv_dispatch<MODE_TAP>(g, EpiGruQ{gru_q_[p].b, hin, z_.p, hout, (long)N * 128}, st);
    mark(p ? ST_GRU_Q_V : ST_GRU_Q, st);
    pr(p ? "gru.h2" : "gru.h1", true, hout, n8, 128, 128);
  }

  s = conv_shape(fh1_, h_[0].p, 128, (long)N * 128, B, H8, W8, 1, 1, 1);
  conv_dispatch<MODE_TAP>(s, EpiBias<ACT_RELU>{fh1_.b, fh_.p, (long)N * 256, 256, 1.f}, st);
  pr("flow_head.conv1", true, fh_.p, n8, 256, 256);
  s = conv_shape(fh2_, fh_.p, 256, (long)N * 256, B, H8, W8, 1, 1, 1);
  conv_dispatch<MODE_TAP>(s, EpiFlowDelta{fh2_.b, coords1_.p, flow4_.p, x_.p + 254, XLD, (long)N * XLD, W8, (long)N}, st);
  mark(ST_FLOWHEAD, st);
  pr("flow", true, flow4_.p, n8, 2, 4);
  pr("coords1", false, coords1_.p, n8, 2, 2);
}

void GmaNet::run_body(int B, int iters, hipStream_t st) {
  float* f; int fh, fw;
// ... 3 lines not shown
  conv_dispatch<MODE_TAP>(s, EpiBias<ACT_NONE>{fnet_.head.b, fmap_.p, (long)N * 256, 256, 1.f}, st);
  mark(ST_FNET, st);
  auto pr = [&](const char* name, bool limited, const float* p, long rows, long cols, long ld) {
    if (probe_) probe(name, limited, p, rows, cols, ld, st);
  };
  pr("fnet.conv2", true, fmap_.p, 2L * B * N, 256, 256);

  ConvShape c;
  c.src0 = fmap_.p; c.ld0 = 256; c.sb0 = (long)N * 256; c.C0 = 256; c.H = 1; c.W = N;
  c.w = fmap_.p + (long)B * N * 256; c.wb = (long)N * 256; c.ldw = 256; c.N = N; c.nimg = B;
  conv_dispatch<MODE_TAP>(c, EpiScale{1.0f / sqrtf(256.0f), pyr_[0].p, (long)N * N, N}, st);
  mark(ST_CORR, st);
  pr("corr.0", false, pyr_[0].p, (long)B * N, N, N);
  for (int l = 1; l < 4; ++l) {
    launch_avgpool(pyr_[l - 1].p, pyrH_[l - 1], pyrW_[l - 1], pyr_[l].p, (long)B * N, st);
    if (probe_) probe("corr." + std::to_string(l), false, pyr_[l].p, (long)B * N, (long)pyrH_[l] * pyrW_[l], (long)pyrH_[l] * pyrW_[l], st);
  }
  mark(ST_POOL, st);

  run_encoder(cnet_, false, B, st, &f, &fh, &fw);
  s = conv_shape(cnet_.head, f, 128, (long)N * 128, B, H8, W8, 1, 0, 0);
  conv_dispatch<MODE_TAP>(s, EpiContextSplit{cnet_.head.b, h_[0].p, (long)N * 128, x_.p, (long)N * XLD, XLD}, st);
  mark(ST_CNET, st);
  pr("net0", true, h_[0].p, (long)B * N, 128, 128);
  pr("inp", true, x_.p, (long)B * N, 128, XLD);

  s = conv_shape(to_qk_, x_.p, XLD, (long)N * XLD, B, H8, W8, 1, 0, 0);
  conv_dispatch<MODE_TAP>(s, EpiQK{1.0f / sqrtf(128.0f), 128, qk_.p, (long)N * 256, 256}, st);
  pr("att.qk", true, qk_.p, (long)B * N, 256, 256);
  ConvShape q;
  q.src0 = qk_.p; q.ld0 = 256; q.sb0 = (long)N * 256; q.C0 = 128; q.H = 1; q.W = N;
  q.w = qk_.p + 128; q.wb = (long)N * 256; q.ldw = 256; q.N = N; q.nimg = B;
  conv_dispatch<MODE_TAP>(q, EpiScale{1.0f, attn_.p, (long)N * ldN, ldN}, st);
  mark(ST_ATTN_LOGITS, st);
  pr("att.logits", false, attn_.p, (long)B * N, N, ldN);
  launch_softmax_rows(attn_.p, (long)B * N, N, ldN, st);
  mark(ST_ATTN, st);
  pr("att.attn", false, attn_.p, (long)B * N, N, ldN);

  for (int it = 0; it < iters; ++it) {
    probe_it_ = it;
    iteration(B, st);
    if (preds_out_) {
      mask_head(B, st);
      launch_upsample(mask_.p, flow4_.p, B, H8, W8, nullptr, preds_out_ + it * preds_stride_, st);
      pr("flow_up", false, preds_out_ + it * preds_stride_, 1, preds_stride_, preds_stride_);
    }
  }
  probe_it_ = -1;
  if (!preds_out_) mask_head(B, st);
  mark(ST_MASK, st);
}

void GmaNet::mask_head(int B, hipStream_t st) {
  ConvShape s = conv_shape(mask0_, h_[0].p, 128, (long)N * 128, B, H8, W8, 1, 1, 1);
  conv_dispatch<MODE_TAP>(s, EpiBias<ACT_RELU>{mask0_.b, fh_.p, (long)N * 256, 256, 1.f}, st);
  if (probe_) probe("mask.0", true, fh_.p, (long)B * N, 256, 256, st);
  s = conv_shape(mask2_, fh_.p, 256, (long)N * 256, B, H8, W8, 1, 0, 0);
  conv_dispatch<MODE_TAP>(s, EpiBias<ACT_NONE>{mask2_.b, mask_.p, (long)N * 576, 576, 0.25f}, st);
  if (probe_) probe("mask", false, mask_.p, (long)B * N, 576, 576, st);
}

void GmaNet::run_encoder_sf(const EncoderWeights& E, bool instance, int nimg, hipStream_t st, float** out_buf, int first_img,
                            DeviceBuf* bufs) {
  const float* images = img4_.p + (long)first_img * H * W * 4;
  int h = conv_out(H, 7, 2, 3), w = conv_out(W, 7, 2, 3);
  DeviceBuf* eb = bufs ? bufs : enc_;
  float* X = eb[0].p; float* R = eb[1].p; float* Y = eb[2].p; float* O = eb[3].p;
  auto stats_sf = [&](const PackedConv& L, const float* src, int ld, int ih, int iw, int stride, int pad, float* dst,
                      int slot, int in_slot = -1) {
    ConvShape s = conv_shape(L, src, ld, (long)ih * iw * ld, nimg, ih, iw, stride, pad, pad);
    if (in_slot >= 0) { s.in_mean = mean_[in_slot].p; s.in_rstd = rstd_[in_slot].p; }
    const int oh = conv_out(ih, L.KH, stride, pad), ow = conv_out(iw, L.KW, stride, pad);
    EpiBiasStats ep{L.b, dst, (long)oh * ow * L.N, L.N, psum_.p, pm2_.p, 0, pcnt_.p};
    TileChoice t = conv_sf_dispatch(s, L.wscale, ep, st);
    const int groups = t.groups_per_img;
    ATDN_CHECK((long)nimg * groups * L.N <= psum_.n && (long)nimg * groups <= pcnt_.n, "statistics scratch too small");
    if (t.counted)
      launch_in_finalize_cnt(psum_.p, pm2_.p, pcnt_.p, nimg, groups, oh * ow, L.N, 1e-5f, mean_[slot].p,
                             rstd_[slot].p, reinterpret_cast<double*>(fin_.p), st);
    else
      launch_in_finalize_cnt(psum_.p, pm2_.p, nullptr, nimg, groups, oh * ow, L.N, 1e-5f, mean_[slot].p, rstd_[slot].p,
                             reinterpret_cast<double*>(fin_.p), st);
  };
  const bool stem_raw = instance && norm_on_load_;
  if (stem_raw) {
    const int groups = stem_sf_groups(h, w);
    ATDN_CHECK((long)nimg * groups * 64 <= psum_.n && (long)nimg * groups <= pcnt_.n, "statistics scratch too small");
    launch_stem_sf(3, images, nimg, H, W, E.stem.wf, E.stem.wscale, E.stem.b, X, psum_.p, pm2_.p, pcnt_.p, nullptr, nullptr, st);
    launch_in_finalize_cnt(psum_.p, pm2_.p, pcnt_.p, nimg, groups, h * w, 64, 1e-5f, mean_[2].p, rstd_[2].p,
                           reinterpret_cast<double*>(fin_.p), st);
  } else if (instance) {
    const int groups = stem_sf_groups(h, w);
    ATDN_CHECK((long)nimg * groups * 64 <= psum_.n && (long)nimg * groups <= pcnt_.n, "statistics scratch too small");
    launch_stem_sf(1, images, nimg, H, W, E.stem.wf, E.stem.wscale, E.stem.b, nullptr, psum_.p, pm2_.p, pcnt_.p, nullptr,
                   nullptr, st);
    launch_in_finalize_cnt(psum_.p, pm2_.p, pcnt_.p, nimg, groups, h * w, 64, 1e-5f, mean_[0].p, rstd_[0].p,
                           reinterpret_cast<double*>(fin_.p), st);
    launch_stem_sf(2, images, nimg, H, W, E.stem.wf, E.stem.wscale, E.stem.b, X, nullptr, nullptr, nullptr, mean_[0].p,
                   rstd_[0].p, st);
  } else {
    launch_stem_sf(0, images, nimg, H, W, E.stem.wf, E.stem.wscale, E.stem.b, X, nullptr, nullptr, nullptr, nullptr,
                   nullptr, st);
  }
  int c = 64;
  for (int bi = 0; bi < 6; ++bi) {
    const auto& Bk = E.blk[bi];
    const int stride = Bk.has_ds ? 2 : 1;
    const int co = Bk.c1.N;
    const int oh = conv_out(h, 3, stride, 1), ow = conv_out(w, 3, stride, 1);
    const long ohw = (long)oh * ow;
    if (instance && norm_on_load_) {
      const bool raw_in = stem_raw && bi == 0;
      ATDN_CHECK(!raw_in || !Bk.has_ds, "the block behind the stem has no downsample branch");
      stats_sf(Bk.c1, X, c, h, w, stride, 1, R, 0, raw_in ? 2 : -1);
      stats_sf(Bk.c2, R, co, oh, ow, 1, 1, Y, 1, 0);
      if (Bk.has_ds) {
        stats_sf(Bk.ds, X, c, h, w, 2, 0, R, 0);
        launch_in_apply_sf(Y, O, mean_[1].p, rstd_[1].p, nullptr, R, mean_[0].p, rstd_[0].p, nimg, ohw, co, st);
      } else if (raw_in) {
        launch_in_apply_sf(Y, O, mean_[1].p, rstd_[1].p, nullptr, X, mean_[2].p, rstd_[2].p, nimg, ohw, co, st, true);
      } else {
        launch_in_apply_sf(Y, O, mean_[1].p, rstd_[1].p, X, nullptr, nullptr, nullptr, nimg, ohw, co, st);
      }
    } else if (instance) {
      stats_sf(Bk.c1, X, c, h, w, stride, 1, R, 0);
      launch_in_apply_sf(R, Y, mean_[0].p, rstd_[0].p, nullptr, nullptr, nullptr, nullptr, nimg, ohw, co, st);
      stats_sf(Bk.c2, Y, co, oh, ow, 1, 1, R, 0);
      if (Bk.has_ds) {
        stats_sf(Bk.ds, X, c, h, w, 2, 0, Y, 1);
        launch_in_apply_sf(R, O, mean_[0].p, rstd_[0].p, nullptr, Y, mean_[1].p, rstd_[1].p, nimg, ohw, co, st);
      } else {
        launch_in_apply_sf(R, O, mean_[0].p, rstd_[0].p, X, nullptr, nullptr, nullptr, nimg, ohw, co, st);
      }
    } else {
      const float* res = X;
      if (Bk.has_ds) {
        ConvShape sd = conv_shape(Bk.ds, X, c, (long)h * w * c, nimg, h, w, 2, 0, 0);
        conv_sf_dispatch(sd, Bk.ds.wscale, SfBias<ACT_NONE>{Bk.ds.b, R, ohw * co, co}, st);
        res = R;
      }
      ConvShape s1 = conv_shape(Bk.c1, X, c, (long)h * w * c, nimg, h, w, stride, 1, 1);
      conv_sf_dispatch(s1, Bk.c1.wscale, SfBias<ACT_RELU>{Bk.c1.b, Y, ohw * co, co}, st);
      ConvShape s2 = conv_shape(Bk.c2, Y, co, ohw * co, nimg, oh, ow, 1, 1, 1);
      conv_sf_dispatch(s2, Bk.c2.wscale, SfBiasReluAddRelu{Bk.c2.b, res, ohw * co, co, O, ohw * co, co}, st);
    }
    std::swap(X, O);
    h = oh; w = ow; c = co;
  }
  ATDN_CHECK(h == H8 && w == W8, "encoder geometry mismatch");
  *out_buf = X;
}

void GmaNet::iteration_sf(int B, hipStream_t st) {
  const long n8 = (long)B * N;
  ConvShape s;
  if (par_) fork(st, par_stream_);
  launch_lookup_conv(brick_pyramid(), coords1_.p, n8, coords_used_.p, convc1_.wf16, convc1_.wscale, convc1_.b, cor1_.p,
                     sf_fast_mode(), st);
  mark(ST_LOOKUP, st);
  s = conv_shape(convc2_, cor1_.p, 256, (long)N * 256, B, H8, W8, 1, 1, 1);
  const ConvShape sf2 = conv_shape(convf2_, flo1_.p, 128, (long)N * 128, B, H8, W8, 1, 1, 1);
  if (par_) {
    launch_flow_conv7_sf(flow4_.p, B, H8, W8, arena_.dev(convf1_sf_off_), convf1_wscale_, convf1_.b, flo1_.p, sf_fast_mode(), par_stream_);
    conv_sf_dispatch(sf2, convf2_.wscale, SfBias<ACT_RELU>{convf2_.b, corflo_.p + 192, (long)N * 256, 256}, par_stream_);
    conv_sf_dispatch(s, convc2_.wscale, SfBias<ACT_RELU>{convc2_.b, corflo_.p, (long)N * 256, 256}, st);
    fork(par_stream_, st);
  } else {
    launch_flow_conv7_sf(flow4_.p, B, H8, W8, arena_.dev(convf1_sf_off_), convf1_wscale_, convf1_.b, flo1_.p, sf_fast_mode(), st);
    conv_sf_dispatch_pair(s, convc2_.wscale, SfBias<ACT_RELU>{convc2_.b, corflo_.p, (long)N * 256, 256},
                          sf2, convf2_.wscale, SfBias<ACT_RELU>{convf2_.b, corflo_.p + 192, (long)N * 256, 256}, st);
  }
  s = conv_shape(convm_, corflo_.p, 256, (long)N * 256, B, H8, W8, 1, 1, 1);
  float* mf = x_.p + 128;
  conv_sf_dispatch(s, convm_.wscale, SfBias<ACT_RELU>{convm_.b, mf, (long)N * XLD, XLD}, st);
  mark(ST_MOTION, st);

  ConvShape v;
  v.src0 = to_v_.w; v.ld0 = 128; v.sb0 = 0; v.C0 = 128; v.H = 1; v.W = 128;
  v.w = mf; v.wb = (long)N * XLD; v.ldw = XLD; v.N = N; v.nimg = B;
  conv_sf_dispatch(v, to_v_.wscale, SfVT{vT_.p, (long)128 * ldN, ldN}, st);
  mark(ST_AGG_VT, st);
  launch_attn_v(attn_.p, rinv_.p, attn_geom(B, N, ldN), vT_.p, gamma_, mf, x_.p + 256, (long)N * XLD, XLD,
                sf_fast_mode(), st, attn_part_.p);
  mark(ST_AGG, st);

  for (int p = 0; p < 2; ++p) {
    const float* hin = h_[p].p;
    float* hout = h_[p ^ 1].p;
    const int ph = p ? 2 : 0, pw = p ? 0 : 2;
    ConvShape g = conv_shape(gru_zr_[p], hin, 128, (long)N * 128, B, H8, W8, 1, ph, pw);
    g.C0 = 128; g.src1 = x_.p + 128; g.ld1 = XLD; g.sb1 = (long)N * XLD; g.C1 = 256;
    conv_sf_dispatch(g, gru_zr_[p].wscale,
                     SfGruZR{gru_zr_[p].b, hin, z_.p, rh_.p, (long)N * 128, pre_zr_[p].p, (long)N * 256}, st);
    mark(p ? ST_GRU_ZR_V : ST_GRU_ZR, st);
    g.src0 = rh_.p; g.w = gru_q_[p].w; g.wfrag16 = gru_q_[p].wf16; g.ldw = gru_q_[p].ldw; g.N = gru_q_[p].N;
    conv_sf_dispatch(g, gru_q_[p].wscale, SfGruQ{gru_q_[p].b, hin, z_.p, hout, (long)N * 128, pre_q_[p].p}, st);
    mark(p ? ST_GRU_Q_V : ST_GRU_Q, st);
  }

  s = conv_shape(fh1_, h_[0].p, 128, (long)N * 128, B, H8, W8, 1, 1, 1);
  const SfFlowDelta fd{fh2_.b, coords1_.p, flow4_.p, x_.p, XLD, (long)N * XLD, 254, W8, (long)N};
  const long fh_gs = (long)maxB * N * 18;
  launch_flow_head_fused(s, fh1_.wscale, SfFlowHeadPartial{fh1_.b, arena_.dev(fh2_w32_off_), fhG_.p, (long)N, fh2_mul_, 1.0f / fh2_mul_, fh_gs}, st);
  launch_flow_gather(fhG_.p, fh_gs, B, H8, W8, fd, st);
  mark(ST_FLOWHEAD, st);
}

void GmaNet::run_body_sf(int B, int iters, hipStream_t st) {
  float* f;
  const int nfeat = seq_ == 0 ? 2 * B : seq_ == 1 ? B + 1 : B;
  hipStream_t sB = par_ ? par_stream_ : st;
  if (par_) fork(st, sB);
  run_encoder_sf(fnet_, true, nfeat, st, &f, seq_ == 2 ? 1 : 0);
  ConvShape s = conv_shape(fnet_.head, f, 128, (long)N * 128, nfeat, H8, W8, 1, 0, 0);
  float* fdst = fmap_.p + (seq_ == 2 ? (long)N * 256 : 0);
  conv_sf_dispatch(s, fnet_.head.wscale, SfBias<ACT_NONE>{fnet_.head.b, fdst, (long)N * 256, 256}, st);
  mark(ST_FNET, st);

  const float* target = fmap_.p + (long)(seq_ ? 1 : B) * N * 256;
  for (int l = 0; l < 4; ++l) {
    const float* plain = target;
    long plain_sb = (long)N * 256;
    if (l > 0) {
      const float* prev = l == 1 ? target : fplain_[l - 2].p;
      const long prev_sb = l == 1 ? (long)N * 256 : (long)pyrH_[l - 1] * pyrW_[l - 1] * 256;
      plain_sb = (long)pyrH_[l] * pyrW_[l] * 256;
      launch_pool_features_sf(prev, B, pyrH_[l - 1], pyrW_[l - 1], 256, prev_sb, fplain_[l - 1].p, plain_sb, st);
      plain = fplain_[l - 1].p;
    }
    launch_brick_rows(plain, plain_sb, B, pyrH_[l], pyrW_[l], 256, fbrick_[l].p, (long)brickNB_[l] * 256, st);
    launch_corr_bricks(fmap_.p, (long)N * 256, fbrick_[l].p, (long)brickNB_[l] * 256, B, N, brickNB_[l], 1.0f / sqrtf(256.0f), pyr_[l].p,
                       sf_fast_mode(), st);
    if (l == 0) mark(ST_CORR, st);
  }
  mark(ST_POOL, st);

  run_encoder_sf(cnet_, false, B, sB, &f, 0, par_ ? enc2_ : nullptr);
  s = conv_shape(cnet_.head, f, 128, (long)N * 128, B, H8, W8, 1, 0, 0);
  conv_sf_dispatch(s, cnet_.head.wscale,
                   SfContextSplit{cnet_.head.b, h_[0].p, (long)N * 128, x_.p, (long)N * XLD, XLD}, sB);
  mark(ST_CNET, st);

  s = conv_shape(to_qk_, x_.p, XLD, (long)N * XLD, B, H8, W8, 1, 0, 0);
  conv_sf_dispatch(s, to_qk_.wscale, SfQK{1.0f / sqrtf(128.0f), 128, qk_.p, (long)N * 256, 256}, sB);
  {
    const AttnGeom ag = attn_geom(B, N, ldN);
    launch_qk_rowmax(qk_.p, ag, rowmax_.p, sB);
    mark(ST_ATTN_LOGITS, st);
    launch_qk_softmax(qk_.p, ag, rowmax_.p, attn_.p, rinv_.p, sf_fast_mode(), sB);
  }
  mark(ST_ATTN, st);

  for (int p = 0; p < 2; ++p) {
    const int ph = p ? 2 : 0, pw = p ? 0 : 2;
    ConvShape g = conv_shape(gru_zr_ctx_[p], x_.p, XLD, (long)N * XLD, B, H8, W8, 1, ph, pw);
    conv_sf_dispatch(g, gru_zr_ctx_[p].wscale, EpiBias<ACT_NONE>{nullptr, pre_zr_[p].p, (long)N * 256, 256, 1.f}, sB);
    g = conv_shape(gru_q_ctx_[p], x_.p, XLD, (long)N * XLD, B, H8, W8, 1, ph, pw);
    conv_sf_dispatch(g, gru_q_ctx_[p].wscale, EpiBias<ACT_NONE>{nullptr, pre_q_[p].p, (long)N * 128, 128, 1.f}, sB);
  }
  mark(ST_GRU_CTX, st);
  if (par_) fork(sB, st);

  for (int it = 0; it < iters; ++it) {
    iteration_sf(B, st);
    if (preds_out_) {
      mask_head_sf(B, st);
      launch_upsample(mask_.p, flow4_.p, B, H8, W8, nullptr, preds_out_ + it * preds_stride_, st);
    }
  }
  if (!preds_out_) mask_head_sf(B, st);
  mark(ST_MASK, st);
}

void GmaNet::mask_head_sf(int B, hipStream_t st) {
  ConvShape s = conv_shape(mask0_, h_[0].p, 128, (long)N * 128, B, H8, W8, 1, 1, 1);
  conv_sf_dispatch(s, mask0_.wscale, SfBias<ACT_RELU>{mask0_.b, fh_.p, (long)N * 256, 256}, st);
  s = conv_shape(mask2_, fh_.p, 256, (long)N * 256, B, H8, W8, 1, 0, 0);
  conv_sf_dispatch(s, mask2_.wscale, EpiBias<ACT_NONE>{mask2_.b, mask_.p, (long)N * 576, 576, 0.25f}, st);
}

void GmaNet::capture(int B, int iters) {
  static const bool par_force = getenv("ATDN_PAR_FORCE") && getenv("ATDN_PAR_FORCE")[0] == '1';
  const bool want_par = low_latency_ && precision >= 1 && (B <= 2 || par_force) && par_stream_ != nullptr && !preds_out_ && par_ok_;
  for (int attempt = want_par ? 0 : 1; attempt < 2; ++attempt) {
    hipGraph_t graph = nullptr;
    hipGraphExec_t exec = nullptr;
    ATDN_HIP(hipStreamBeginCapture(cap_stream_, hipStreamCaptureModeThreadLocal));
    par_ = attempt == 0;
    par_next_ = 0;
    try {
      if (precision >= 1) { FastGuard fg(precision == 2); run_body_sf(B, iters, cap_stream_); } else run_body(B, iters, cap_stream_);
      par_ = false;
      ATDN_HIP(hipStreamEndCapture(cap_stream_, &graph));
      ATDN_HIP(hipGraphInstantiate(&exec, graph, nullptr, nullptr, 0));
    } catch (...) {
      const bool was_par = par_ || attempt == 0;
      par_ = false;
      hipGraph_t g2 = nullptr;
      (void)hipStreamEndCapture(cap_stream_, &g2);
      if (g2) (void)hipGraphDestroy(g2);
      if (graph) (void)hipGraphDestroy(graph);
      (void)hipGetLastError();
      if (attempt == 0 && was_par) {
        fprintf(stderr, "atdn: the flow graph could not be captured with parallel branches; capturing it as one chain\n");
        par_ok_ = false;
        continue;
      }
      throw;
    }
    (void)hipGraphDestroy(graph);
    graphs_[{B, iters * 4 + seq_}] = exec;
    return;
  }
}

void GmaNet::forward_sequence(const float* frames, int B, int iters, const float* flow_init, float* flow_low,
                               float* flow_up, hipStream_t st, bool continued) {
  ATDN_CHECK(ready_, "weights not finalized");
  ATDN_CHECK(precision >= 1, "sequence mode is built for the split-f16 pipeline");
  ATDN_CHECK(B >= 1 && B <= maxB, "batch exceeds max_batch of this handle");
  ATDN_CHECK(iters >= 1 && iters <= 64, "iters out of range");
  ATDN_CHECK(frames && flow_low && flow_up, "null tensor");
  const long frame = 3L * H * W;
  if (continued) {
    ATDN_CHECK(last_frame_ >= 1, "continued sequence call without a previous sequence call on this handle");
    ATDN_HIP(hipMemcpyAsync(fmap_.p, fmap_.p + (long)last_frame_ * N * 256, (size_t)N * 256 * sizeof(float),
                            hipMemcpyDeviceToDevice, st));
    seq_ = 2;
  } else {
    seq_ = 1;
  }
  last_frame_ = 0;
  launch_prep_images(frames, frames + (long)B * frame, B, H, W, img4_.p, st, 1);
  launch_init_coords_sf(flow_init, B, H8, W8, coords1_.p, flow4_.p, x_.p, XLD, 254, st);
  launch_body(B, iters, st);
  launch_upsample(mask_.p, flow4_.p, B, H8, W8, flow_low, flow_up, st);
  last_frame_ = B;
}

void GmaNet::launch_body(int B, int iters, hipStream_t st) {
  last_B_ = B;
  if (use_graph_ && !probe_) {
    auto key = std::make_pair(B, iters * 4 + seq_);
    if (!graphs_.count(key)) capture(B, iters);
    ATDN_HIP(hipGraphLaunch(graphs_[key], st));
  } else {
    if (precision >= 1) { FastGuard fg(precision == 2); run_body_sf(B, iters, st); } else run_body(B, iters, st);
  }
}

void GmaNet::forward(const float* im1, const float* im2, int B, int iters, const float* flow_init, float* flow_low,
                     float* flow_up, hipStream_t st) {
  ATDN_CHECK(ready_, "weights not finalized");
  ATDN_CHECK(B >= 1 && B <= maxB, "batch exceeds max_batch of this handle");
  ATDN_CHECK(iters >= 1 && iters <= 64, "iters out of range");
  ATDN_CHECK(im1 && im2 && flow_low && flow_up, "null tensor");
  seq_ = 0;
  last_frame_ = 0;
  if (probe_) probe_begin(st);
  launch_prep_images(im1, im2, B, H, W, img4_.p, st, B);
  if (precision >= 1) launch_init_coords_sf(flow_init, B, H8, W8, coords1_.p, flow4_.p, x_.p, XLD, 254, st);
  else launch_init_coords(flow_init, B, H8, W8, coords1_.p, flow4_.p, x_.p + 254, XLD, st);
  if (probe_) {
    probe("image", true, img4_.p, 2L * B * H * W, 3, 4, st);
    probe("flow_init", true, flow4_.p, (long)B * N, 2, 4, st);
  }
  launch_body(B, iters, st);
  launch_upsample(mask_.p, flow4_.p, B, H8, W8, flow_low, flow_up, st);
  if (probe_) {
    probe("flow_low", false, flow_low, 1, 2L * B * N, 2L * B * N, st);
    probe("flow_up", false, flow_up, 1, 2L * B * H * W, 2L * B * H * W, st);
    probe_end(st);
  }
}

void GmaNet::forward_predictions(const float* im1, const float* im2, int B, int iters, const float* flow_init, float* preds,
                                 hipStream_t st) {
  ATDN_CHECK(ready_, "weights not finalized");
  ATDN_CHECK(B >= 1 && B <= maxB, "batch exceeds max_batch of this handle");
  ATDN_CHECK(iters >= 1 && iters <= 64, "iters out of range");
  ATDN_CHECK(im1 && im2 && preds, "null tensor");
  seq_ = 0;
  last_frame_ = 0;
  last_B_ = B;
  if (probe_) probe_begin(st);
  launch_prep_images(im1, im2, B, H, W, img4_.p, st, B);
  if (precision >= 1) launch_init_coords_sf(flow_init, B, H8, W8, coords1_.p, flow4_.p, x_.p, XLD, 254, st);
  else launch_init_coords(flow_init, B, H8, W8, coords1_.p, flow4_.p, x_.p + 254, XLD, st);
  if (probe_) {
    probe("image", true, img4_.p, 2L * B * H * W, 3, 4, st);
    probe("flow_init", true, flow4_.p, (long)B * N, 2, 4, st);
  }
  struct Guard {
    GmaNet* n; ~Guard() { n->preds_out_ = nullptr; n->preds_stride_ = 0; }
  } guard{this};
  preds_out_ = preds;
  preds_stride_ = (long)B * 2 * H * W;
  if (precision >= 1) { FastGuard fg(precision == 2); run_body_sf(B, iters, st); } else run_body(B, iters, st);
  if (probe_) probe_end(st);
}

BrickPyramid GmaNet::brick_pyramid() const {
  BrickPyramid bp;
  for (int l = 0; l < 4; ++l) {
    bp.base[l] = pyr_[l].p; bp.H[l] = pyrH_[l]; bp.W[l] = pyrW_[l];
    bp.BW[l] = brickBW_[l]; bp.BH[l] = brickBH_[l]; bp.NB[l] = brickNB_[l];
  }
  bp.N = N; bp.NPB = brick_pixel_blocks(N);
  return bp;
}

long GmaNet::debug_read(const char* name, float* host, long capacity, hipStream_t st) {
  const std::string k(name);
  if (!classic_ && k.size() == 4 && k.compare(0, 3, "pyr") == 0 && k[3] >= '0' && k[3] <= '3') {
    const int l = k[3] - '0';
    const long rows = (long)maxB * N, total = rows * pyrH_[l] * pyrW_[l];
    if (scratch_.n < total) { scratch_.release(); scratch_.alloc(total); }
    launch_unbrick(pyr_[l].p, brickNB_[l], N, pyrH_[l], pyrW_[l], rows, scratch_.p, st);
    ATDN_HIP(hipStreamSynchronize(st));
    const long n = std::min(capacity, total);
    ATDN_HIP(hipMemcpy(host, scratch_.p, (size_t)n * sizeof(float), hipMemcpyDeviceToHost));
    return n;
  }
  if (!classic_ && k == "corrfeat") {
    launch_lookup_bricks(brick_pyramid(), coords_used_.p, (long)(last_B_ > 0 ? last_B_ : maxB) * N, corrfeat_.p, st);
  }
  if (k == "sf_clamped") {
    ATDN_CHECK(capacity >= 1, "sf_clamped needs room for one float");
    host[0] = (float)sf_counter_read_reset(st);
    return 1;
  }
  const DeviceBuf* b = nullptr;
  if (k == "fmap") b = &fmap_; else if (k == "pyr0") b = &pyr_[0]; else if (k == "pyr1") b = &pyr_[1];
  else if (k == "pyr2") b = &pyr_[2]; else if (k == "pyr3") b = &pyr_[3]; else if (k == "net") b = &h_[0];
  else if (k == "x") b = &x_; else if (k == "attn") b = &attn_; else if (k == "corrfeat") b = &corrfeat_;
  else if (k == "mask") b = &mask_; else if (k == "coords1") b = &coords1_; else if (k == "flow4") b = &flow4_;
  else if (k == "qk") b = &qk_; else if (k == "img4") b = &img4_;
  else if (k == "cor1") b = &cor1_;
  if (!b) return -1;
  long n = std::min(capacity, b->n);
  if (k == "attn" && !classic_) {
    const long rows = (long)maxB * N * ldN;
    if (scratch_.n < rows) { scratch_.release(); scratch_.alloc(rows); }
    ATDN_HIP(hipMemsetAsync(scratch_.p, 0, (size_t)rows * sizeof(float), st));
    launch_attn_decode(attn_.p, rinv_.p, attn_geom(maxB, N, ldN), scratch_.p, st);
    ATDN_HIP(hipStreamSynchronize(st));
    n = std::min(capacity, rows);
    ATDN_HIP(hipMemcpy(host, scratch_.p, (size_t)n * sizeof(float), hipMemcpyDeviceToHost));
    return n;
  }
  const bool is_sf = precision >= 1 && (k == "fmap" || k == "net" || k == "x" || k == "attn" || k == "corrfeat" || k == "qk" || k == "cor1");
  const float* src = b->p;
  if (is_sf) {
    if (scratch_.n < b->n) { scratch_.release(); scratch_.alloc(b->n); }
    launch_from_sf(b->p, scratch_.p, b->n / 32, 32, st);
    src = scratch_.p;
  }
  ATDN_HIP(hipStreamSynchronize(st));
  ATDN_HIP(hipMemcpy(host, src, (size_t)n * sizeof(float), hipMemcpyDeviceToHost));
  return n;
}

}
```

### atdn_vslam_amd/csrc/sf.h

```cpp
#pragma once
#include "common.h"

namespace atdn {

typedef _Float16 f16x8 __attribute__((ext_vector_type(8)));

struct SfPair { _Float16 hi, lo; };

namespace {
__device__ unsigned int* sf_clamp_counter_tu_ = nullptr;
__global__ void sf_counter_set_kernel_(unsigned int* p) { sf_clamp_counter_tu_ = p; }
void sf_counter_set_tu_(unsigned int* p) {
  hipLaunchKernelGGL(sf_counter_set_kernel_, dim3(1), dim3(1), 0, nullptr, p);
}
}
void sf_counter_register(void (*setter)(unsigned int*));
namespace {
struct SfCounterRegistration { SfCounterRegistration() { sf_counter_register(&sf_counter_set_tu_); } };
static SfCounterRegistration sf_counter_registration_;
}
void sf_counter_attach();
unsigned int sf_counter_read_reset(hipStream_t st);

__device__ __forceinline__ SfPair sf_split_flag(float v, bool& clamped) {
  clamped |= !(fabsf(v) <= 65504.f);
  v = fminf(fmaxf(v, -65504.f), 65504.f);
  SfPair p;
  p.hi = (_Float16)v;
  p.lo = (_Float16)(v - (float)p.hi);
  return p;
}
__device__ __forceinline__ void sf_report(bool clamped) {
  if (__builtin_expect(clamped, 0)) {
    unsigned int* c = *const_cast<unsigned int* volatile*>(&sf_clamp_counter_tu_);
    const unsigned long long act = __builtin_amdgcn_ballot_w64(true);
    if (c && (unsigned)__builtin_amdgcn_mbcnt_hi((unsigned)(act >> 32), __builtin_amdgcn_mbcnt_lo((unsigned)act, 0u)) == 0u)
      atomicAdd(c, (unsigned)__builtin_popcountll(act));
  }
}

__device__ __forceinline__ SfPair sf_split(float v) {
  if (__builtin_expect(!(fabsf(v) <= 65504.f), 0)) {
    unsigned int* c = *const_cast<unsigned int* volatile*>(&sf_clamp_counter_tu_);
    const unsigned long long act = __builtin_amdgcn_ballot_w64(true);
    if (c && (unsigned)__builtin_amdgcn_mbcnt_hi((unsigned)(act >> 32), __builtin_amdgcn_mbcnt_lo((unsigned)act, 0u)) == 0u)
      atomicAdd(c, (unsigned)__builtin_popcountll(act));
  }
  v = fminf(fmaxf(v, -65504.f), 65504.f);
  SfPair p;
  p.hi = (_Float16)v;
  p.lo = (_Float16)(v - (float)p.hi);
  return p;
}

__device__ __forceinline__ _Float16* sf_ptr(float* base, long off, int c) {
  return reinterpret_cast<_Float16*>(base + off + (c & ~31)) + (c & 31);
}
__device__ __forceinline__ const _Float16* sf_ptr(const float* base, long off, int c) {
  return reinterpret_cast<const _Float16*>(base + off + (c & ~31)) + (c & 31);
}
__device__ __forceinline__ void sf_store(float* base, long off, int c, float v) {
  const SfPair p = sf_split(v);
  _Float16* q = sf_ptr(base, off, c);
  q[0] = p.hi;
  q[32] = p.lo;
}
typedef _Float16 f16x4 __attribute__((ext_vector_type(4)));
__device__ __forceinline__ SfPair sf_split_nocheck_(float v) {
  SfPair p;
  p.hi = (_Float16)v;
  p.lo = (_Float16)(v - (float)p.hi);
  return p;
}
__device__ __forceinline__ void sf_store4(float* base, long off, int c, float4 v) {
  const float m = (fabsf(v.x) + fabsf(v.y)) + (fabsf(v.z) + fabsf(v.w));
  if (__builtin_expect(!(m <= 65504.f), 0)) {
    const SfPair a = sf_split(v.x), b = sf_split(v.y), d = sf_split(v.z), e = sf_split(v.w);
    _Float16* q = sf_ptr(base, off, c);
    *reinterpret_cast<f16x4*>(q) = f16x4{a.hi, b.hi, d.hi, e.hi};
    *reinterpret_cast<f16x4*>(q + 32) = f16x4{a.lo, b.lo, d.lo, e.lo};
    return;
  }
  const SfPair a = sf_split_nocheck_(v.x), b = sf_split_nocheck_(v.y), d = sf_split_nocheck_(v.z), e = sf_split_nocheck_(v.w);
  _Float16* q = sf_ptr(base, off, c);
  *reinterpret_cast<f16x4*>(q) = f16x4{a.hi, b.hi, d.hi, e.hi};
  *reinterpret_cast<f16x4*>(q + 32) = f16x4{a.lo, b.lo, d.lo, e.lo};
}
typedef _Float16 f16x2 __attribute__((ext_vector_type(2)));
typedef float f32x2 __attribute__((ext_vector_type(2)));
__device__ __forceinline__ unsigned sf_cvt_pk_(float a, float b) {
  const f32x2 x = {a, b};
  return __builtin_bit_cast(unsigned, __builtin_convertvector(x, f16x2));
}
__device__ __forceinline__ unsigned sf_residual_pk_(unsigned hp, float a, float b) {
  unsigned d;
  asm("v_fma_mixlo_f16 %0, %1, -1.0, %2 op_sel_hi:[1,0,0]" : "=v"(d) : "v"(hp), "v"(a));
  asm("v_fma_mixhi_f16 %0, %1, -1.0, %2 op_sel:[1,0,0] op_sel_hi:[1,0,0]" : "+v"(d) : "v"(hp), "v"(b));
  return d;
}
__device__ __forceinline__ void sf_store4_flag(float* base, long off, int c, float4 v, bool& clamped) {
  const float lim = 65504.f;
  const float m = fmaxf(fmaxf(fabsf(v.x), fabsf(v.y)), fmaxf(fabsf(v.z), fabsf(v.w)));
  clamped |= !(m <= lim) | __builtin_isunordered(v.x, v.y) | __builtin_isunordered(v.z, v.w);
  v.x = __builtin_amdgcn_fmed3f(v.x, -lim, lim); v.y = __builtin_amdgcn_fmed3f(v.y, -lim, lim);
  v.z = __builtin_amdgcn_fmed3f(v.z, -lim, lim); v.w = __builtin_amdgcn_fmed3f(v.w, -lim, lim);
  const unsigned h0 = sf_cvt_pk_(v.x, v.y), h1 = sf_cvt_pk_(v.z, v.w);
  const unsigned l0 = sf_residual_pk_(h0, v.x, v.y), l1 = sf_residual_pk_(h1, v.z, v.w);
  _Float16* q = sf_ptr(base, off, c);
  *reinterpret_cast<uint2*>(q) = make_uint2(h0, h1);
  *reinterpret_cast<uint2*>(q + 32) = make_uint2(l0, l1);
}
__device__ __forceinline__ float sf_join_lo_(unsigned hi, unsigned lo) {
  return (float)__builtin_bit_cast(f16x2, hi)[0] + (float)__builtin_bit_cast(f16x2, lo)[0];
}
__device__ __forceinline__ float sf_join_hi_(unsigned hi, unsigned lo) {
  return (float)__builtin_bit_cast(f16x2, hi)[1] + (float)__builtin_bit_cast(f16x2, lo)[1];
}
__device__ __forceinline__ float4 sf_load4(const float* base, long off, int c) {
  const _Float16* q = sf_ptr(base, off, c);
  const uint2 hi = *reinterpret_cast<const uint2*>(q), lo = *reinterpret_cast<const uint2*>(q + 32);
  return make_float4(sf_join_lo_(hi.x, lo.x), sf_join_hi_(hi.x, lo.x), sf_join_lo_(hi.y, lo.y), sf_join_hi_(hi.y, lo.y));
}
__device__ __forceinline__ unsigned sf_byte_offset_(unsigned off, int c) {
  return 4u * (off + (unsigned)(c & ~31)) + 2u * (unsigned)(c & 31);
}
__device__ __forceinline__ void sf_store4_flag_u(float* base, unsigned off, int c, float4 v, bool& clamped) {
  const float lim = 65504.f;
  const float m = fmaxf(fmaxf(fabsf(v.x), fabsf(v.y)), fmaxf(fabsf(v.z), fabsf(v.w)));
  clamped |= !(m <= lim) | __builtin_isunordered(v.x, v.y) | __builtin_isunordered(v.z, v.w);
  v.x = __builtin_amdgcn_fmed3f(v.x, -lim, lim); v.y = __builtin_amdgcn_fmed3f(v.y, -lim, lim);
  v.z = __builtin_amdgcn_fmed3f(v.z, -lim, lim); v.w = __builtin_amdgcn_fmed3f(v.w, -lim, lim);
  const unsigned h0 = sf_cvt_pk_(v.x, v.y), h1 = sf_cvt_pk_(v.z, v.w);
  const unsigned l0 = sf_residual_pk_(h0, v.x, v.y), l1 = sf_residual_pk_(h1, v.z, v.w);
  char* q = reinterpret_cast<char*>(base) + sf_byte_offset_(off, c);
  *reinterpret_cast<uint2*>(q) = make_uint2(h0, h1);
  *reinterpret_cast<uint2*>(q + 64) = make_uint2(l0, l1);
}
__device__ __forceinline__ float4 sf_load4u(const float* base, unsigned off, int c) {
  const char* q = reinterpret_cast<const char*>(base) + sf_byte_offset_(off, c);
  const uint2 hi = *reinterpret_cast<const uint2*>(q), lo = *reinterpret_cast<const uint2*>(q + 64);
  return make_float4(sf_join_lo_(hi.x, lo.x), sf_join_hi_(hi.x, lo.x), sf_join_lo_(hi.y, lo.y), sf_join_hi_(hi.y, lo.y));
}
__device__ __forceinline__ float sf_load(const float* base, long off, int c) {
  const _Float16* q = sf_ptr(base, off, c);
  return (float)q[0] + (float)q[32];
}

}
```

### atdn_vslam_amd/csrc/small_convs.h

```cpp
#pragma once
#include "common.h"
#include "epilogues_sf.h"

namespace atdn {

void launch_flow_conv7_sf(const float* flow4, int nimg, int H, int W, const float* wfrag, float wscale, const float* bias,
                          float* out_sf, bool fast, hipStream_t st);
struct ConvShape;
void launch_flow_head_fused(const ConvShape& s, float wscale, const SfFlowHeadPartial& ep, hipStream_t st);
void launch_flow_gather(const float* G, long gstride, int nimg, int H, int W, const SfFlowDelta& ep, hipStream_t st);

}
```

### atdn_vslam_amd/csrc/small_convs.hip

```cpp
#include <algorithm>
#include "small_convs.h"
#include "sf.h"

namespace atdn {

constexpr int FC_PR = 2 + 6 + 1;
constexpr int FC_PP = 24;
template <bool FAST>
__global__ __launch_bounds__(256, 3) void flow_conv7_sf_kernel(const float4* __restrict__ flow4, int nimg, int H, int W,
                                                               const float* __restrict__ wfrag, float wscale,
                                                               const float* __restrict__ bias, float* __restrict__ out, long ob,
                                                               int tiles_x, int tiles_img) {
  typedef float f32x4v __attribute__((ext_vector_type(4)));
  typedef unsigned int u32x4 __attribute__((ext_vector_type(4)));
  __shared__ unsigned int plane[2][2][FC_PR * FC_PP];
  const int tid = threadIdx.x, lane = tid & 63, wave = tid >> 6;
  const int n16 = lane & 15, g16 = lane >> 4;
  const int ntiles = nimg * tiles_img;

  f16x8 wh[2][4], wl[2][4];
  {
    const char* wb = reinterpret_cast<const char*>(wfrag) + lane * 16;
#pragma unroll
    for (int cb = 0; cb < 2; ++cb)
#pragma unroll
      for (int s = 0; s < 4; ++s) {
        const long f = (((long)wave * 2 + cb) * 4 + s) * 2;
        wh[cb][s] = *reinterpret_cast<const f16x8*>(wb + f * 1024);
        if (!FAST) wl[cb][s] = *reinterpret_cast<const f16x8*>(wb + (f + 1) * 1024);
      }
  }
  float4 b4[2];
#pragma unroll
  for (int cb = 0; cb < 2; ++cb) b4[cb] = *reinterpret_cast<const float4*>(bias + 32 * wave + 16 * cb + 4 * g16);

  const int ppy = tid / FC_PP, ppx = tid - ppy * FC_PP;
  const bool pin = tid < FC_PR * FC_PP;
  bool clamped = false;
  auto fetch = [&](int t) -> float2 {
    const int img = t / tiles_img, tloc = t - img * tiles_img;
    const int iy = (tloc / tiles_x) * 2 - 3 + ppy, ix = (tloc % tiles_x) * 16 - 3 + ppx;
    float2 v = make_float2(0.f, 0.f);
    if (pin && (unsigned)iy < (unsigned)H && (unsigned)ix < (unsigned)W) {
      const float4 f = flow4[((long)img * H + iy) * W + ix];
      v = make_float2(f.x, f.y);
    }
    return v;
  };
  auto stash = [&](int buf, float2 v) {
    if (pin) {
      const SfPair x = sf_split_flag(v.x, clamped), y = sf_split_flag(v.y, clamped);
      typedef _Float16 f16x2 __attribute__((ext_vector_type(2)));
      plane[buf][0][tid] = __builtin_bit_cast(unsigned int, f16x2{x.hi, y.hi});
      plane[buf][1][tid] = __builtin_bit_cast(unsigned int, f16x2{x.lo, y.lo});
    }
  };

  int t = blockIdx.x;
  if (t < ntiles) stash(0, fetch(t));
  __syncthreads();
  for (int it = 0; t < ntiles; t += gridDim.x, ++it) {
    const int buf = it & 1;
    const int tn = t + gridDim.x;
    float2 nxt = make_float2(0.f, 0.f);
    if (tn < ntiles) nxt = fetch(tn);

    f32x4v acc[2][2];
#pragma unroll
    for (int rb = 0; rb < 2; ++rb)
#pragma unroll
      for (int cb = 0; cb < 2; ++cb)
#pragma unroll
        for (int e = 0; e < 4; ++e) acc[rb][cb][e] = 0.f;
#pragma unroll
    for (int s = 0; s < 4; ++s)
#pragma unroll
      for (int rb = 0; rb < 2; ++rb) {
        const int p = (rb + 2 * s + (g16 >> 1)) * FC_PP + n16 + 4 * (g16 & 1);
        u32x4 h4, l4;
#pragma unroll
        for (int k = 0; k < 4; ++k) { h4[k] = plane[buf][0][p + k]; if (!FAST) l4[k] = plane[buf][1][p + k]; }
        const f16x8 ph = __builtin_bit_cast(f16x8, h4);
#pragma unroll
        for (int cb = 0; cb < 2; ++cb) {
          f32x4v c = acc[rb][cb];
          if (!FAST) {
            const f16x8 pl = __builtin_bit_cast(f16x8, l4);
            c = __builtin_amdgcn_mfma_f32_16x16x32_f16(wh[cb][s], pl, c, 0, 0, 0);
            c = __builtin_amdgcn_mfma_f32_16x16x32_f16(wl[cb][s], ph, c, 0, 0, 0);
          }
          c = __builtin_amdgcn_mfma_f32_16x16x32_f16(wh[cb][s], ph, c, 0, 0, 0);
          acc[rb][cb] = c;
        }
      }
    {
      const int img = t / tiles_img, tloc = t - img * tiles_img;
      const int oy0 = (tloc / tiles_x) * 2, ox = (tloc % tiles_x) * 16 + n16;
#pragma unroll
      for (int rb = 0; rb < 2; ++rb) {
        const int oy = oy0 + rb;
        if (oy < H && ox < W) {
          const long off = (long)img * ob + ((long)oy * W + ox) * 128;
#pragma unroll
          for (int cb = 0; cb < 2; ++cb) {
            const float4 o = make_float4(fmaxf(acc[rb][cb][0] * wscale + b4[cb].x, 0.f), fmaxf(acc[rb][cb][1] * wscale + b4[cb].y, 0.f),
                                         fmaxf(acc[rb][cb][2] * wscale + b4[cb].z, 0.f), fmaxf(acc[rb][cb][3] * wscale + b4[cb].w, 0.f));
            sf_store4_flag(out, off, 32 * wave + 16 * cb + 4 * g16, o, clamped);
          }
        }
      }
    }
    if (tn < ntiles) stash(buf ^ 1, nxt);
    __syncthreads();
  }
  sf_report(clamped);
}

void launch_flow_conv7_sf(const float* flow4, int nimg, int H, int W, const float* wfrag, float wscale, const float* bias,
                          float* out_sf, bool fast, hipStream_t st) {
  const int tx = cdiv(W, 16), ty = cdiv(H, 2);
  const int ntiles = nimg * tx * ty;
  const int grid = std::min(ntiles, 256 * 3);
  if (fast)
    hipLaunchKernelGGL(flow_conv7_sf_kernel<true>, dim3(grid), dim3(256), 0, st, reinterpret_cast<const float4*>(flow4), nimg, H, W,
                       wfrag, wscale, bias, out_sf, (long)H * W * 128, tx, tx * ty);
  else
    hipLaunchKernelGGL(flow_conv7_sf_kernel<false>, dim3(grid), dim3(256), 0, st, reinterpret_cast<const float4*>(flow4), nimg, H, W,
                       wfrag, wscale, bias, out_sf, (long)H * W * 128, tx, tx * ty);
  ATDN_HIP(hipGetLastError());
}

__global__ __launch_bounds__(256) void flow_gather_kernel(const float* __restrict__ G, long gstride, int H, int W, long total,
                                                          const SfFlowDelta ep) {
  const long i = (long)blockIdx.x * 256 + threadIdx.x;
  if (i >= total) return;
  const long HW = (long)H * W;
  const int img = (int)(i / HW), m = (int)(i - img * HW);
  const int y = m / W, x = m - y * W;
  float s0 = 0.f, s1 = 0.f;
#pragma unroll
  for (int t = 0; t < 9; ++t) {
    const int sy = y + t / 3 - 1, sx = x + t % 3 - 1;
    if ((unsigned)sy < (unsigned)H && (unsigned)sx < (unsigned)W) {
      const float* gp = G + ((long)img * HW + (long)sy * W + sx) * 18 + 2 * t;
      float2 g = *reinterpret_cast<const float2*>(gp);
      if (gstride) {
        const float2 g1 = *reinterpret_cast<const float2*>(gp + gstride);
        g.x += g1.x; g.y += g1.y;
      }
      s0 += g.x; s1 += g.y;
    }
  }
  const SfFlowDelta::Aux a0 = ep.load(img, m, 0), a1 = ep.load(img, m, 1);
  ep.apply(img, m, 0, s0, a0);
  ep.apply(img, m, 1, s1, a1);
}

void launch_flow_gather(const float* G, long gstride, int nimg, int H, int W, const SfFlowDelta& ep, hipStream_t st) {
  const long total = (long)nimg * H * W;
  hipLaunchKernelGGL(flow_gather_kernel, dim3((unsigned)cdivl(total, 256)), dim3(256), 0, st, G, gstride, H, W, total, ep);
  ATDN_HIP(hipGetLastError());
}

}
```

### atdn_vslam_amd/csrc/weights.h

```cpp
#pragma once
#include <cmath>
#include <cstring>
#include <map>
#include <string>
#include <vector>

#include "conv_mfma.h"

namespace atdn {

struct HostTensor {
  std::vector<int64_t> shape;
  std::vector<float> data;
  long numel() const { long n = 1; for (auto d : shape) n *= d; return n; }
};

class StateDict {
 public:
  void put(const std::string& key, const float* data, const int64_t* shape, int rank) {
    std::string k = key;
    if (k.rfind("module.", 0) == 0) k = k.substr(7);
    HostTensor t;
    t.shape.assign(shape, shape + rank);
    const long n = t.numel();
// ... 58 lines not shown
  const auto& rm = sd.get(p + ".running_mean"); const auto& rv = sd.get(p + ".running_var");
  ChannelAffine a;
  const size_t n = w.data.size();
  a.scale.resize(n); a.shift.resize(n);
  for (size_t i = 0; i < n; ++i) {
    a.scale[i] = (double)w.data[i] / std::sqrt((double)rv.data[i] + eps);
    a.shift[i] = (double)b.data[i] - (double)rm.data[i] * a.scale[i];
  }
  return a;
}

inline PackedConv pack_conv(WeightArena& A, const StateDict& sd, const std::vector<std::string>& names, int mode,
                            int Cpix, const ChannelAffine* fold = nullptr, bool has_bias = true) {
  PackedConv L;
  const HostTensor& w0 = sd.get(names[0] + ".weight");
  ATDN_CHECK(w0.shape.size() == 4, "conv weight must be 4-d");
  const int Cin = (int)w0.shape[1], KH = (int)w0.shape[2], KW = (int)w0.shape[3];
  L.mode = mode; L.KH = KH; L.KW = KW;
  L.C = (mode == MODE_TAP) ? round_up(Cin, 32) : Cpix;
  ATDN_CHECK(L.C >= Cin, "channel padding smaller than Cin");
  L.ldw = packed_k(mode, KH, KW, L.C);
  int N = 0;
  for (auto& nm : names) N += (int)sd.get(nm + ".weight").shape[0];
  L.N = N;
  L.w_off = A.alloc((long)N * L.ldw);
  L.b_off = A.alloc(N);
  int n0 = 0;
  for (auto& nm : names) {
    const HostTensor& w = sd.get(nm + ".weight");
    ATDN_CHECK((int)w.shape[1] == Cin && (int)w.shape[2] == KH && (int)w.shape[3] == KW, "stacked convs must agree");
    const int Co = (int)w.shape[0];
    const float* bias = (has_bias && sd.has(nm + ".bias")) ? sd.get(nm + ".bias").data.data() : nullptr;
    for (int n = 0; n < Co; ++n) {
      const double sc = fold ? fold->scale[n0 + n] : 1.0;
      float* row = A.at(L.w_off + (long)(n0 + n) * L.ldw);
      for (int c = 0; c < Cin; ++c)
        for (int ky = 0; ky < KH; ++ky)
          for (int kx = 0; kx < KW; ++kx) {
            const double v = (double)w.data[(((long)n * Cin + c) * KH + ky) * KW + kx] * sc;
            const long k = (mode == MODE_TAP) ? ((long)(ky * KW + kx) * L.C + c)
                                              : ((long)ky * round_up(KW * L.C, 32) + kx * L.C + c);
            row[k] = (float)v;
          }
      double bv = bias ? (double)bias[n] : 0.0;
      if (fold) bv = bv * sc + fold->shift[n0 + n];
      A.at(L.b_off)[n0 + n] = (float)bv;
    }
    n0 += Co;
  }
  return L;
}

inline void pack_fragment_major16(WeightArena& A, PackedConv& L) {
  const int nq = L.ldw / 32, nblk = (L.N + 15) / 16;
  L.wf16_off = A.alloc((long)nblk * nq * 512);
  const float* w = A.at(L.w_off);
  float* f = A.at(L.wf16_off);
  for (int nb = 0; nb < nblk; ++nb)
    for (int q = 0; q < nq; ++q)
      for (int hl = 0; hl < 2; ++hl)
        for (int lane = 0; lane < 64; ++lane) {
          const int r = lane & 15, gq = lane >> 4, row = nb * 16 + r, slot = 4 * hl + gq;
          float* d = f + ((((long)nb * nq + q) * 2 + hl) * 64 + lane) * 4;
          if (row < L.N) std::memcpy(d, w + (long)row * L.ldw + q * 32 + slot * 4, 16);
          else std::memset(d, 0, 16);
        }
}

inline PackedConv pack_conv_sf(WeightArena& A, const StateDict& sd, const std::vector<std::string>& names,
                               const ChannelAffine* fold = nullptr, bool has_bias = true) {
  PackedConv L = pack_conv(A, sd, names, MODE_TAP, 0, fold, has_bias);
  float* w = A.at(L.w_off);
  const long total = (long)L.N * L.ldw;
  float mx = 0.f;
  for (long i = 0; i < total; ++i) mx = std::max(mx, std::fabs(w[i]));
  int e = 0;
  if (mx > 0.f) (void)std::frexp(mx, &e);
  const int p = 1 - e;
  L.wscale = std::ldexp(1.0f, -p);
  std::vector<float> row(L.ldw);
  for (int n = 0; n < L.N; ++n) {
    float* r = w + (long)n * L.ldw;
    std::memcpy(row.data(), r, L.ldw * sizeof(float));
    _Float16* hrow = reinterpret_cast<_Float16*>(r);
    for (int q = 0; q < L.ldw / 32; ++q)
      for (int j = 0; j < 32; ++j) {
        const float v = std::ldexp(row[q * 32 + j], p);
        const _Float16 hi = (_Float16)v;
        const _Float16 lo = (_Float16)(v - (float)hi);
        hrow[q * 64 + j] = hi;
        hrow[q * 64 + 32 + j] = lo;
      }
  }
  if ((L.KH == 3 && L.KW == 3) || (L.KH == 1 && L.KW == 5) || (L.KH == 5 && L.KW == 1)) {
    pack_fragment_major16(A, L);
  }
  return L;
}

inline void pack_stem_sf(WeightArena& A, PackedConv& L) {
  ATDN_CHECK(L.mode == MODE_ROW && L.KH == 7 && L.KW == 7 && L.C == 4 && L.ldw == 224 && L.N == 64, "stem shape");
  L.wf_off = A.alloc(2L * 14 * 2 * 256);
  const float* w = A.at(L.w_off);
  float mx = 0.f;
  for (long i = 0; i < (long)L.N * L.ldw; ++i) mx = std::max(mx, std::fabs(w[i]));
  int e = 0;
  if (mx > 0.f) (void)std::frexp(mx, &e);
  const int p = 1 - e;
  L.wscale = std::ldexp(1.0f, -p);
  _Float16* f = reinterpret_cast<_Float16*>(A.at(L.wf_off));
  for (int nt = 0; nt < 2; ++nt)
    for (int q = 0; q < 14; ++q)
      for (int lane = 0; lane < 64; ++lane) {
        const int r = lane & 31, h = lane >> 5;
        for (int m = 0; m < 8; ++m) {
          const float v = std::ldexp(w[(long)(nt * 32 + r) * L.ldw + 16 * q + 8 * h + m], p);
          const _Float16 hi = (_Float16)v;
          f[(((long)(nt * 14 + q) * 2 + 0) * 64 + lane) * 8 + m] = hi;
          f[(((long)(nt * 14 + q) * 2 + 1) * 64 + lane) * 8 + m] = (_Float16)(v - (float)hi);
        }
      }
}

inline PackedConv pack_conv_sf_channels(WeightArena& A, const StateDict& sd, const std::vector<std::string>& names,
                                        const std::vector<std::pair<int, int>>& ranges, bool has_bias) {
  StateDict tmp;
  std::vector<std::string> tnames;
  for (size_t t = 0; t < names.size(); ++t) {
    const HostTensor& w = sd.get(names[t] + ".weight");
    const int Co = (int)w.shape[0], Ci = (int)w.shape[1], KH = (int)w.shape[2], KW = (int)w.shape[3];
    int Cn = 0;
    for (auto& r : ranges) Cn += r.second - r.first;
    std::vector<float> out((size_t)Co * Cn * KH * KW);
    for (int n = 0; n < Co; ++n) {
      int c2 = 0;
      for (auto& r : ranges)
        for (int c = r.first; c < r.second; ++c, ++c2)
          std::memcpy(&out[((size_t)n * Cn + c2) * KH * KW], &w.data[((size_t)n * Ci + c) * KH * KW],
                      sizeof(float) * KH * KW);
    }
    const std::string key = "s" + std::to_string(t);
    const int64_t shp[4] = {Co, Cn, KH, KW};
    tmp.put(key + ".weight", out.data(), shp, 4);
    if (has_bias && sd.has(names[t] + ".bias")) {
      const HostTensor& b = sd.get(names[t] + ".bias");
      const int64_t bs[1] = {Co};
      tmp.put(key + ".bias", b.data.data(), bs, 1);
    }
    tnames.push_back(key);
  }
  return pack_conv_sf(A, tmp, tnames, nullptr, has_bias);
}

inline long pack_vector(WeightArena& A, const std::vector<float>& v) {
  const long off = A.alloc((long)v.size());
  std::memcpy(A.at(off), v.data(), v.size() * sizeof(float));
  return off;
}

inline void resolve(const WeightArena& A, PackedConv& L) {
  L.w = A.dev(L.w_off);
  L.b = A.dev(L.b_off);
  L.wf = L.wf_off >= 0 ? A.dev(L.wf_off) : nullptr;
  L.wf16 = L.wf16_off >= 0 ? A.dev(L.wf16_off) : nullptr;
}

}
```

### include/atdn_hip.h

```cpp
#ifndef ATDN_HIP_H
#define ATDN_HIP_H

#include <stddef.h>
#include <stdint.h>

#ifdef __cplusplus
extern "C" {
#endif

typedef struct atdn_gma atdn_gma;
typedef struct atdn_clvo atdn_clvo;
typedef struct atdn_vae atdn_vae;
typedef struct atdn_clvo_trainer atdn_clvo_trainer;

int atdn_version(void);
const char* atdn_last_error(void);


#define ATDN_PRECISION_F32 0
#define ATDN_PRECISION_SPLIT_F16 1
#define ATDN_PRECISION_F16 2
int atdn_gma_create(atdn_gma** out, int H, int W, int max_batch, int precision);

int atdn_gma_set_low_latency(atdn_gma* h, int on);

int atdn_gma_load(atdn_gma* h, const char* key, const float* data, const int64_t* shape, int rank);

int atdn_gma_finalize(atdn_gma* h);

int atdn_gma_forward(atdn_gma* h, const float* im1, const float* im2, int B, int iters, const float* flow_init,
                     float* flow_low, float* flow_up, void* stream);

int atdn_gma_forward_predictions(atdn_gma* h, const float* im1, const float* im2, int B, int iters, const float* flow_init,
                                 float* flow_predictions, void* stream);

int atdn_gma_forward_sequence(atdn_gma* h, const float* frames, int B, int iters, const float* flow_init,
                              float* flow_low, float* flow_up, void* stream);
int atdn_gma_forward_sequence_continued(atdn_gma* h, const float* frames, int B, int iters, const float* flow_init,
                                        float* flow_low, float* flow_up, void* stream);

long atdn_gma_debug_read(atdn_gma* h, const char* name, float* host, long capacity, void* stream);

#define ATDN_GMA_STAGES 18
int atdn_gma_profile(atdn_gma* h, int B, int iters, int reps, float* ms_out, void* stream);
int atdn_gma_profile_mode(atdn_gma* h, int B, int iters, int reps, int mode, float* ms_out, void* stream);

int atdn_gma_set_range_probe(atdn_gma* h, int on);
long atdn_gma_range_rows(atdn_gma* h);
int atdn_gma_range_row(atdn_gma* h, long index, char* name, int name_capacity, int* iteration, int* limited, float* max_abs,
                       int64_t* over, int64_t* nonfinite);
int atdn_range_probe(const float* x, int64_t rows, int64_t cols, int64_t ld, float* max_abs, int64_t* over, int64_t* nonfinite,
                     void* stream);
int atdn_range_probe_launch(const float* x, int64_t rows, int64_t cols, int64_t ld, void* slot, void* stream);

size_t atdn_gma_workspace_bytes(atdn_gma* h);
void atdn_gma_destroy(atdn_gma* h);


int atdn_clvo_create(atdn_clvo** out, int H, int W, int max_batch);
int atdn_clvo_load(atdn_clvo* h, const char* key, const float* data, const int64_t* shape, int rank);
int atdn_clvo_finalize(atdn_clvo* h);

int atdn_clvo_encode(atdn_clvo* h, const float* flow, int B, float* feat, void* stream);

int atdn_clvo_step(atdn_clvo* h, const float* feat, int T, int Bs, float* state, float* rot, float* tr, void* stream);
void atdn_clvo_destroy(atdn_clvo* h);

int atdn_clvo_trainer_create(atdn_clvo_trainer** out, int H, int W, int batch, int sequence_length);
int atdn_clvo_trainer_load(atdn_clvo_trainer* h, const char* key, const float* data, const int64_t* shape, int rank);
int atdn_clvo_trainer_finalize(atdn_clvo_trainer* h);
int atdn_clvo_trainer_forward_backward(atdn_clvo_trainer* h, const float* flows, const float* true_rot, const float* true_tr,
                                       float* pred_rot, float* pred_tr, float* loss_out, void* stream);
int atdn_clvo_trainer_gradients(atdn_clvo_trainer* h, float** device_ptr, long* count);
int atdn_clvo_trainer_set_loss(atdn_clvo_trainer* h, float alpha, int w, int mode);
int atdn_clvo_trainer_loss_terms(atdn_clvo_trainer* h, float* terms3_host);
int atdn_clvo_loss(const float* pred_rot, const float* pred_tr, const float* true_rot, const float* true_tr, int B, int T, float alpha,
                   int w, int mode, float* loss3_host, float* d_rot, float* d_tr, void* stream);
int atdn_clvo_trainer_adamw_step(atdn_clvo_trainer* h, float lr, float weight_decay, float eps, int step, void* stream);
long atdn_clvo_trainer_read(atdn_clvo_trainer* h, const char* key, int kind, float* host, long capacity, void* stream);
void atdn_clvo_trainer_destroy(atdn_clvo_trainer* h);

int atdn_vae_create(atdn_vae** out, int H, int W, int max_batch);
int atdn_vae_load(atdn_vae* h, const char* key, const float* data, const int64_t* shape, int rank);
int atdn_vae_finalize(atdn_vae* h);
int atdn_vae_embedding_shape(const atdn_vae* h, int* out_h, int* out_w);
int atdn_vae_encode(atdn_vae* h, const float* images, int B, float* mu, void* stream);
void atdn_vae_destroy(atdn_vae* h);


int atdn_pose_transform_f32(const float* rot, const float* tr, float* mat16);
int atdn_pose_rel2abs(const float* rot, const float* tr, int T, double* poses);
int atdn_pose_accumulate_f32(float* pose16, const float* rot, const float* tr);


#define ATDN_RESIZE_BILINEAR 0
#define ATDN_RESIZE_ANTIALIAS 1

int atdn_resize_frames(const float* src, int planes, int Hin, int Win, int Hout, int Wout, float* dst, void* stream);
int atdn_resize_frames_mode(const float* src, int planes, int Hin, int Win, int Hout, int Wout, int antialias, float* dst,
                            void* stream);
int atdn_resize_frames_u8(const uint8_t* src, int planes, int Hin, int Win, int Hout, int Wout, int antialias, float* dst,
                          void* stream);

int atdn_pad_frames(const float* src, int planes, int H, int W, int left, int right, int top, int bottom, float* dst,
                    void* stream);

typedef struct atdn_ingest atdn_ingest;
int atdn_ingest_create(atdn_ingest** out, int Hin, int Win, int Hout, int Wout, int max_frames, int antialias);
int atdn_ingest_frames_u8(atdn_ingest* h, const uint8_t* host_frames, int n_frames, float* dst, void* stream);
void atdn_ingest_destroy(atdn_ingest* h);


int atdn_flow_pack_f16(const float* flow_up, int B, int H, int Wsrc, int x0, int W, uint16_t* dst, void* stream);

int atdn_flow_gather_clips(const uint16_t* bank, int n_flows, int H, int W, const int* start, const int* reverse, int B, int T,
                           float* out, void* stream);


int atdn_map_search(const float* bank, int K, int D, const float* queries, int Q, int topk, float* dist, int* idx, void* stream);

int atdn_map_gather_images_u8(const uint8_t* bank, int K, long plane_bytes, const int* index_host, int n, float* out, void* stream);


int atdn_corr_lookup(const float* pyr0, const float* pyr1, const float* pyr2, const float* pyr3, int B, int H8,
                     int W8, const float* coords, float* out, int ldo, void* stream);

int atdn_corr_pyramid(const float* fmap1, const float* fmap2, int B, int H8, int W8, int C, float* pyr0, float* pyr1,
                      float* pyr2, float* pyr3, void* stream);

int atdn_corr_lookup_bricks(const float* fmap1, const float* fmap2, int B, int H8, int W8, int C, const float* coords,
                            float* pyr0, float* pyr1, float* pyr2, float* pyr3, float* samples,
                            const float* convc1_weight_host, const float* convc1_bias_host, float* cor1, void* stream);

int atdn_conv2d_nhwc(const float* src, int nimg, int H, int W, int Cin, const float* weight_host,
                     const float* bias_host, int Cout, int KH, int KW, int stride, int padH, int padW, int relu,
                     float* dst, void* stream);

int atdn_conv2d_nhwc_sf(const float* src, int nimg, int H, int W, int Cin, const float* weight_host,
                        const float* bias_host, int Cout, int KH, int KW, int stride, int padH, int padW, float* dst,
                        void* stream);
int atdn_conv2d_nhwc_sf_epi(const float* src, int nimg, int H, int W, int Cin, const float* weight_host,
                            const float* bias_host, int Cout, int KH, int KW, int stride, int padH, int padW, int sf_store,
                            float* dst, void* stream);

#ifdef __cplusplus
}
#endif
#endif
```

Baseline: 419.6 frame-pairs/s.

## Fuse flow gather, convf1 7x7 and convf2 3x3 into one flow-branch kernel

Adds a kernel that computes the coordinate update from the flow-head gather, then evaluates convf1 (7x7, 2->128) into shared memory. It does this through a feed hook in the sf6 conv body, which then runs convf2 directly, so the flo1 intermediate never goes to global memory. The coords and flow4 buffers are double-buffered (ping-pong), which replaces a device copy because the halo reads need a separate output buffer. The iteration function gains first/last flags, and graphs record which buffer is current. The cost is that convf1 is recomputed on the halo pixels of every tile, and register and LDS pressure goes up in the combined kernel.

```diff
diff --git a/atdn_vslam_amd/_lib.py b/atdn_vslam_amd/_lib.py
--- a/atdn_vslam_amd/_lib.py
+++ b/atdn_vslam_amd/_lib.py
@@ -70,6 +70,8 @@
     "atdn_corr_pyramid": (C.c_int, [_vp, _vp, C.c_int, C.c_int, C.c_int, C.c_int, _vp, _vp, _vp, _vp, _vp]),
     "atdn_corr_lookup_bricks": (C.c_int, [_vp, _vp, C.c_int, C.c_int, C.c_int, C.c_int, _vp, _vp, _vp, _vp, _vp, _vp, _vp, _vp,
                                           _vp, _vp]),
+    "atdn_flow_branch_debug": (C.c_int, [C.c_int, C.c_int, C.c_int, C.c_int, C.c_int, _vp, _vp, _vp, _vp, _vp, _vp, _vp, _vp, _vp,
+                                         _vp, _vp, _vp]),
     "atdn_conv2d_nhwc": (C.c_int, [_vp, C.c_int, C.c_int, C.c_int, C.c_int, _vp, _vp, C.c_int, C.c_int, C.c_int,
                                    C.c_int, C.c_int, C.c_int, C.c_int, _vp, _vp]),
     "atdn_conv2d_nhwc_sf": (C.c_int, [_vp, C.c_int, C.c_int, C.c_int, C.c_int, _vp, _vp, C.c_int, C.c_int, C.c_int,
diff --git a/atdn_vslam_amd/csrc/capi.hip b/atdn_vslam_amd/csrc/capi.hip
--- a/atdn_vslam_amd/csrc/capi.hip
+++ b/atdn_vslam_amd/csrc/capi.hip
@@ -10,6 +10,7 @@
 #include "frontend.h"
 #include "conv_sf.h"
 #include "epilogues_sf.h"
+#include "small_convs.h"
 
 namespace atdn {
 extern template TileChoice conv_dispatch<MODE_TAP, EpiBias<ACT_NONE>>(const ConvShape&, EpiBias<ACT_NONE>, hipStream_t);
@@ -488,6 +489,74 @@
   ATDN_API_END
 }
 
+int atdn_flow_branch_debug(int fused, int fast, int B, int H8, int W8, const float* G, const float* coords_in,
+                           const float* fh2_bias_host, const float* convf1_weight_host, const float* convf1_bias_host,
+                           const float* convf2_weight_host, const float* convf2_bias_host, float* coords_out, float* flow4_out,
+                           float* x_sf, float* corflo_sf, void* stream) {
+  ATDN_API_BEGIN
+  ATDN_CHECK(G && coords_in && fh2_bias_host && convf1_weight_host && convf1_bias_host && convf2_weight_host && convf2_bias_host &&
+             coords_out && flow4_out && x_sf && corflo_sf, "null argument");
+  ATDN_CHECK(B >= 1 && H8 >= 1 && W8 >= 1 && coords_in != coords_out, "bad argument");
+  constexpr int kXld = 384, kFlowCh = 254;
+  hipStream_t st = (hipStream_t)stream;
+  const int N = H8 * W8;
+  const long n8 = (long)B * N;
+  StateDict sd;
+  const int64_t w1s[4] = {128, 2, 7, 7}, b1s[1] = {128}, w2s[4] = {64, 128, 3, 3}, b2s[1] = {64}, fbs[1] = {2};
+  sd.put("f1.weight", convf1_weight_host, w1s, 4);
+  sd.put("f1.bias", convf1_bias_host, b1s, 1);
+  sd.put("f2.weight", convf2_weight_host, w2s, 4);
+  sd.put("f2.bias", convf2_bias_host, b2s, 1);
+  sd.put("fh2.bias", fh2_bias_host, fbs, 1);
+  WeightArena A;
+  PackedConv f1 = pack_conv(A, sd, {"f1"}, MODE_ROW, 4);
+  float w1scale = 1.f;
+  const long w1off = pack_convf1_sf(A, sd.get("f1.weight"), &w1scale);
+  PackedConv f2 = pack_conv_sf(A, sd, {"f2"});
+  const long fboff = pack_vector(A, sd.get("fh2.bias").data);
+  A.upload();
+  resolve(A, f1);
+  resolve(A, f2);
+  DeviceBuf flo1;
+  const bool prev_fast = sf_fast_mode();
+  try {
+    sf_counter_attach();
+    sf_fast_mode() = fast != 0;
+    ConvShape s2;
+    s2.src0 = nullptr; s2.ld0 = 128; s2.sb0 = (long)N * 128; s2.C0 = f2.C; s2.H = H8; s2.W = W8;
+    s2.KH = 3; s2.KW = 3; s2.stride = 1; s2.padH = 1; s2.padW = 1;
+    s2.w = f2.w; s2.wfrag16 = f2.wf16; s2.ldw = f2.ldw; s2.N = 64; s2.nimg = B;
+    const SfBias<ACT_RELU> ep2{f2.b, corflo_sf + 192, (long)N * 256, 256};
+    if (fused) {
+      FlowBranchArgs fa;
+      fa.G = G; fa.gstride = n8 * 18; fa.fh2_bias = A.dev(fboff);
+      fa.coords_in = coords_in; fa.coords_out = coords_out; fa.flow4_out = flow4_out;
+      fa.x = x_sf; fa.ldx = kXld; fa.xb = (long)N * kXld; fa.cflow = kFlowCh;
+      fa.w1frag = A.dev(w1off); fa.w1scale = w1scale; fa.b1 = f1.b;
+      launch_flow_branch_sf(s2, f2.wscale, ep2, fa, fast != 0, st);
+    } else {
+      flo1.alloc(n8 * 128);
+      s2.src0 = flo1.p;
+      ATDN_HIP(hipMemcpyAsync(coords_out, coords_in, (size_t)n8 * 2 * sizeof(float), hipMemcpyDeviceToDevice, st));
+      const SfFlowDelta fd{A.dev(fboff), coords_out, flow4_out, x_sf, kXld, (long)N * kXld, kFlowCh, W8, (long)N};
+      launch_flow_gather(G, n8 * 18, B, H8, W8, fd, st);
+      launch_flow_conv7_sf(flow4_out, B, H8, W8, A.dev(w1off), w1scale, f1.b, flo1.p, fast != 0, st);
+      conv_sf_dispatch(s2, f2.wscale, ep2, st);
+    }
+    ATDN_HIP(hipStreamSynchronize(st));
+  } catch (...) {
+    sf_fast_mode() = prev_fast;
+    (void)hipDeviceSynchronize();
+    flo1.release();
+    A.release();
+    throw;
+  }
+  sf_fast_mode() = prev_fast;
+  flo1.release();
+  A.release();
+  ATDN_API_END
+}
+
 int atdn_conv2d_nhwc(const float* src, int nimg, int H, int W, int Cin, const float* weight_host,
                      const float* bias_host, int Cout, int KH, int KW, int stride, int padH, int padW, int relu,
                      float* dst, void* stream) {
diff --git a/atdn_vslam_amd/csrc/conv_sf6.h b/atdn_vslam_amd/csrc/conv_sf6.h
--- a/atdn_vslam_amd/csrc/conv_sf6.h
+++ b/atdn_vslam_amd/csrc/conv_sf6.h
@@ -46,9 +46,13 @@
 template <class E> struct conv_stamp_kind : std::integral_constant<int, -1> {};
 #endif
 
-template <int TH, int TW, int BN, int WM, int WN, int KH, int KW, class Epi, bool FAST = false, bool NORM = false, int ABL = 0>
-__device__ __forceinline__ void conv_sf6_body(const Conv2Geom& g, const Epi& ep, const int bidx) {
+struct NoFeed {};
+template <int TH, int TW, int BN, int WM, int WN, int KH, int KW, class Epi, bool FAST = false, bool NORM = false, int ABL = 0,
+          class Feed = NoFeed>
+__device__ __forceinline__ void conv_sf6_body(const Conv2Geom& g, const Epi& ep, const int bidx, Feed feed = Feed{}) {
   static_assert(ABL == 0 || !NORM, "ablation builds exist for the plain patch loader");
+  constexpr bool FED = !std::is_same<Feed, NoFeed>::value;
+  static_assert(!FED || (!NORM && ABL == 0), "a feed replaces the plain patch loader");
   static_assert(TW == 16, "the 16x16x32 loop is built for 16-pixel tile rows");
   constexpr int NIMG = 2;
   constexpr int NW = WM * WN, NT = NW * 64;
@@ -106,6 +110,7 @@
 
   float4 pr[NP];
   auto fetch_patch = [&](int c) {
+    if constexpr (FED) return;
     const int cc = c << 5;
     const float* sp; int ld, co;
     if (cc < g.C0) { sp = s0; ld = g.ld0; co = cc; } else { sp = s1; ld = g.ld1; co = cc - g.C0; }
@@ -113,7 +118,8 @@
     for (int k = 0; k < NP; ++k)
       pr[k] = *reinterpret_cast<const float4*>(sp + (long)((pmeta[k] >> 12) ? (pmeta[k] >> 12) - 1 : 0) * ld + co + 4 * s);
   };
-  auto store_patch = [&](int buf) {
+  auto store_patch = [&](int buf, int c) {
+    if constexpr (FED) { feed.produce(c, Pbytes + buf * PSZ); return; }
 #pragma unroll
     for (int k = 0; k < NP; ++k)
       *reinterpret_cast<float4*>(Pbytes + buf * PSZ + ((pmeta[k] & 0xFFFu) << 4)) = keep_if((pmeta[k] >> 12) != 0, pr[k]);
@@ -185,7 +191,7 @@
 #pragma unroll
       for (int k = 0; k < NP; ++k) store_row_norm(0, k, nmu, nrs);
     } else {
-      store_patch(0);
+      store_patch(0, 0);
     }
     __syncthreads();
 #ifdef ATDN_CONV_STAMP
@@ -249,7 +255,7 @@
           if constexpr (NORM) {
             if (hs >= NH - 1 - NP && hs <= NH - 2) store_row_norm((c + 1) & 1, hs - (NH - 1 - NP), nmu, nrs);
           } else {
-            if (!(ABL & 2) && hs == NH - 2) store_patch((c + 1) & 1);
+            if (!(ABL & 2) && hs == NH - 2 && (!FED || c + 1 < nck)) store_patch((c + 1) & 1, cn);
           }
           if (live) mfma_half(half, wr[st % RT]);
           {
diff --git a/atdn_vslam_amd/csrc/flow_branch.hip b/atdn_vslam_amd/csrc/flow_branch.hip
--- /dev/null
+++ b/atdn_vslam_amd/csrc/flow_branch.hip
@@ -0,0 +1,158 @@
+#include "conv_sf6.h"
+#include "small_convs.h"
+
+namespace atdn {
+
+constexpr int FB_TH = 8, FB_TW = 16;
+constexpr int FB_PH = FB_TH + 2, FB_PW = FB_TW + 2;
+constexpr int FB_NPP = FB_PH * FB_PW;
+constexpr int FB_WH = FB_PH + 6 + 1, FB_WW = FB_PW + 6 + 1;
+constexpr int FB_NW = FB_WH * FB_WW;
+static_assert((FB_NPP + 15) / 16 == 3 * 4, "three pixel blocks per wave, four waves");
+
+template <bool FAST>
+struct Convf1Feed {
+  const unsigned int* plane;
+  const char* wfrag;
+  const float* bias;
+  float wscale;
+  int poff[3];
+  int pimg[3];
+  bool* sat;
+  __device__ __forceinline__ void produce(int c, char* image) {
+    typedef unsigned int u32x4 __attribute__((ext_vector_type(4)));
+    f32x4v acc[3][2];
+#pragma unroll
+    for (int j = 0; j < 3; ++j)
+#pragma unroll
+      for (int cb = 0; cb < 2; ++cb)
+#pragma unroll
+        for (int e = 0; e < 4; ++e) acc[j][cb][e] = 0.f;
+#pragma unroll
+    for (int s = 0; s < 4; ++s) {
+      f16x8 wh[2], wl[2];
+#pragma unroll
+      for (int cb = 0; cb < 2; ++cb) {
+        const long f = (((long)c * 2 + cb) * 4 + s) * 2;
+        wh[cb] = *reinterpret_cast<const f16x8*>(wfrag + f * 1024);
+        if (!FAST) wl[cb] = *reinterpret_cast<const f16x8*>(wfrag + (f + 1) * 1024);
+      }
+#pragma unroll
+      for (int j = 0; j < 3; ++j) {
+        const unsigned int* q = plane + poff[j] + 2 * s * FB_WW;
+        u32x4 h4, l4;
+#pragma unroll
+        for (int k = 0; k < 4; ++k) { h4[k] = q[k]; if (!FAST) l4[k] = q[FB_NW + k]; }
+        const f16x8 ph = __builtin_bit_cast(f16x8, h4);
+#pragma unroll
+        for (int cb = 0; cb < 2; ++cb) {
+          f32x4v a = acc[j][cb];
+          if (!FAST) {
+            const f16x8 pl = __builtin_bit_cast(f16x8, l4);
+            a = __builtin_amdgcn_mfma_f32_16x16x32_f16(wh[cb], pl, a, 0, 0, 0);
+            a = __builtin_amdgcn_mfma_f32_16x16x32_f16(wl[cb], ph, a, 0, 0, 0);
+          }
+          a = __builtin_amdgcn_mfma_f32_16x16x32_f16(wh[cb], ph, a, 0, 0, 0);
+          acc[j][cb] = a;
+        }
+      }
+    }
+    float4 b4[2];
+#pragma unroll
+    for (int cb = 0; cb < 2; ++cb) b4[cb] = *reinterpret_cast<const float4*>(bias + 32 * c + 16 * cb);
+    const int g8 = 8 * ((threadIdx.x & 63) >> 4);
+#pragma unroll
+    for (int j = 0; j < 3; ++j) {
+      if (pimg[j] < 0) continue;
+      const bool inside = (pimg[j] & (1 << 30)) == 0;
+      char* px = image + (pimg[j] & 0xFFFFFF) + g8;
+#pragma unroll
+      for (int cb = 0; cb < 2; ++cb) {
+        uint2 hi = make_uint2(0u, 0u), lo = make_uint2(0u, 0u);
+        if (inside) sf_pack4_flag(convf1_act4(acc[j][cb][0], acc[j][cb][1], acc[j][cb][2], acc[j][cb][3], wscale, b4[cb]), *sat, hi, lo);
+        *reinterpret_cast<uint2*>(px + 32 * cb) = hi;
+        *reinterpret_cast<uint2*>(px + 64 + 32 * cb) = lo;
+      }
+    }
+  }
+};
+
+template <bool FAST>
+__global__ __launch_bounds__(256, 2) void flow_branch_sf_kernel(const Conv2Geom g, const SfBias<ACT_RELU> ep, const FlowBranchArgs a) {
+  __shared__ unsigned int plane[2 * FB_NW];
+  const int tid = threadIdx.x, lane = tid & 63, wave = tid >> 6;
+  const int tiles_img = g.tiles_x * g.tiles_y;
+  const int id = xcd_remap((int)blockIdx.x, g.nimg * tiles_img);
+  const int img = id / tiles_img, tloc = id - img * tiles_img;
+  const int ty0 = (tloc / g.tiles_x) * FB_TH, tx0 = (tloc % g.tiles_x) * FB_TW;
+  const int H = g.H, W = g.W;
+  const long pix0 = (long)img * H * W;
+
+  bool sat = false;
+  const float fb0 = a.fh2_bias[0], fb1 = a.fh2_bias[1];
+  for (int i = tid; i < FB_NW; i += 256) {
+    const int wy = i / FB_WW, wx = i - wy * FB_WW;
+    const int iy = ty0 - 4 + wy, ix = tx0 - 4 + wx;
+    unsigned int hi = 0u, lo = 0u;
+    if ((unsigned)iy < (unsigned)H && (unsigned)ix < (unsigned)W) {
+      const int m = iy * W + ix;
+      const float2 s = flow_gather_sum(a.G, a.gstride, img, H, W, iy, ix);
+      const float2 c = *reinterpret_cast<const float2*>(a.coords_in + (pix0 + m) * 2);
+      const float c1x = c.x + (s.x + fb0), c1y = c.y + (s.y + fb1);
+      const float fx = c1x - (float)ix, fy = c1y - (float)iy;
+      const SfPair X = sf_split_flag(fx, sat), Y = sf_split_flag(fy, sat);
+      hi = __builtin_bit_cast(unsigned int, f16x2{X.hi, Y.hi});
+      lo = __builtin_bit_cast(unsigned int, f16x2{X.lo, Y.lo});
+      if ((unsigned)(wy - 4) < (unsigned)FB_TH && (unsigned)(wx - 4) < (unsigned)FB_TW) {
+        *reinterpret_cast<float2*>(a.coords_out + (pix0 + m) * 2) = make_float2(c1x, c1y);
+        *reinterpret_cast<float2*>(a.flow4_out + (pix0 + m) * 4) = make_float2(fx, fy);
+        _Float16* q = sf_ptr(a.x, (long)img * a.xb + (long)m * a.ldx, a.cflow);
+        *reinterpret_cast<unsigned int*>(q) = hi;
+        *reinterpret_cast<unsigned int*>(q + 32) = lo;
+      }
+    }
+    plane[i] = hi;
+    plane[FB_NW + i] = lo;
+  }
+  __syncthreads();
+
+  Convf1Feed<FAST> feed;
+  feed.plane = plane;
+  feed.wfrag = reinterpret_cast<const char*>(a.w1frag) + lane * 16;
+  feed.bias = a.b1 + 4 * (lane >> 4);
+  feed.wscale = a.w1scale;
+  feed.sat = &sat;
+  {
+    const int n16 = lane & 15, g16 = lane >> 4;
+#pragma unroll
+    for (int j = 0; j < 3; ++j) {
+      const int p = 16 * (wave + 4 * j) + n16;
+      const int pc = min(p, FB_NPP - 1);
+      const int py = pc / FB_PW, px = pc - py * FB_PW;
+      feed.poff[j] = (py + (g16 >> 1)) * FB_WW + px + 4 * (g16 & 1);
+      const int iy = ty0 - 1 + py, ix = tx0 - 1 + px;
+      const bool inside = (unsigned)iy < (unsigned)H && (unsigned)ix < (unsigned)W;
+      feed.pimg[j] = p < FB_NPP ? (p * 160) | (inside ? 0 : (1 << 30)) : -1;
+    }
+  }
+  conv_sf6_body<FB_TH, FB_TW, 64, 2, 2, 3, 3, SfBias<ACT_RELU>, FAST, false, 0, Convf1Feed<FAST>>(g, ep, (int)blockIdx.x, feed);
+  sf_report(sat);
+}
+
+void launch_flow_branch_sf(const ConvShape& convf2, float wscale2, const SfBias<ACT_RELU>& ep, const FlowBranchArgs& a, bool fast,
+                           hipStream_t st) {
+  ATDN_CHECK(convf2.N == 64 && convf2.C0 == 128 && convf2.C1 == 0 && convf2.padH == 1 && convf2.padW == 1,
+             "the flow branch is built for convf2 = 3x3, 128 -> 64, padding 1");
+  ATDN_CHECK(a.G && a.fh2_bias && a.coords_in && a.coords_out && a.flow4_out && a.x && a.w1frag && a.b1, "null tensor");
+  ATDN_CHECK(a.coords_in != a.coords_out, "the coordinates are read on the halo: they need a buffer of their own to be written to");
+  ATDN_CHECK((a.cflow & 1) == 0 && (a.cflow & 31) <= 30, "the two flow channels share one 32-channel group");
+  const Conv2Geom g = fast ? conv_sf6_geom<FB_TH, 64, 2, 2, 3, 3, SfBias<ACT_RELU>, true>(convf2, wscale2)
+                           : conv_sf6_geom<FB_TH, 64, 2, 2, 3, 3, SfBias<ACT_RELU>, false>(convf2, wscale2);
+  ATDN_CHECK(g.ntile_n == 1 && g.Ho == g.H && g.Wo == g.W, "one block per pixel tile, output of the input's size");
+  const int nblk = g.nimg * g.tiles_x * g.tiles_y;
+  if (fast) hipLaunchKernelGGL(flow_branch_sf_kernel<true>, dim3(nblk), dim3(256), 0, st, g, ep, a);
+  else hipLaunchKernelGGL(flow_branch_sf_kernel<false>, dim3(nblk), dim3(256), 0, st, g, ep, a);
+  ATDN_HIP(hipGetLastError());
+}
+
+}
diff --git a/atdn_vslam_amd/csrc/gma.h b/atdn_vslam_amd/csrc/gma.h
--- a/atdn_vslam_amd/csrc/gma.h
+++ b/atdn_vslam_amd/csrc/gma.h
@@ -85,7 +85,7 @@
   void run_body_sf(int B, int iters, hipStream_t st);
   void run_encoder_sf(const EncoderWeights& E, bool instance, int nimg, hipStream_t st, float** out_buf, int first_img = 0,
                       DeviceBuf* bufs = nullptr);
-  void iteration_sf(int B, hipStream_t st);
+  void iteration_sf(int B, hipStream_t st, bool first, bool last);
   void capture(int B, int iters);
   void launch_body(int B, int iters, hipStream_t st);
   int seq_ = 0;
@@ -115,6 +115,10 @@
   DeviceBuf img4_, enc_[4], scratch_, pcnt_, fin_, fmap_, psum_, pm2_, mean_[3], rstd_[3];
   DeviceBuf pyr_[4], h_[2], x_, qk_, attn_, vT_, corrfeat_, cor1_, corflo_, flo1_, z_, rh_, fh_, mask_;
   DeviceBuf coords1_, flow4_, pre_zr_[2], pre_q_[2];
+  DeviceBuf coords1b_, flow4b_;
+  int cfb_ = 0;
+  float* coords_cur() const { return cfb_ ? coords1b_.p : coords1_.p; }
+  float* flow4_cur() const { return cfb_ ? flow4b_.p : flow4_.p; }
   int pyrH_[4], pyrW_[4];
   size_t ws_bytes_ = 0;
 
@@ -124,6 +128,7 @@
 
   hipStream_t cap_stream_ = nullptr;
   std::map<std::pair<int, int>, hipGraphExec_t> graphs_;
+  std::map<std::pair<int, int>, int> graph_cfb_;
 };
 
 }
diff --git a/atdn_vslam_amd/csrc/gma.hip b/atdn_vslam_amd/csrc/gma.hip
--- a/atdn_vslam_amd/csrc/gma.hip
+++ b/atdn_vslam_amd/csrc/gma.hip
@@ -165,7 +165,7 @@
   for (auto& e : par_events_) (void)hipEventDestroy(e);
   DeviceBuf* all[] = {&img4_, &enc_[0], &enc_[1], &enc_[2], &enc_[3], &scratch_, &pcnt_, &fin_, &fmap_, &psum_, &pm2_, &mean_[0], &mean_[1], &mean_[2], &rstd_[0],
                       &rstd_[1], &rstd_[2], &pyr_[0], &pyr_[1], &pyr_[2], &pyr_[3], &h_[0], &h_[1], &x_, &qk_, &attn_, &vT_,
-                      &corrfeat_, &cor1_, &corflo_, &flo1_, &z_, &rh_, &fh_, &mask_, &coords1_, &flow4_, &pre_zr_[0],
+                      &corrfeat_, &cor1_, &corflo_, &flo1_, &z_, &rh_, &fh_, &mask_, &coords1_, &flow4_, &coords1b_, &flow4b_, &pre_zr_[0],
                       &pre_zr_[1], &pre_q_[0], &pre_q_[1], &rowmax_, &rinv_,
                       &fbrick_[0], &fbrick_[1], &fbrick_[2], &fbrick_[3], &fplain_[0], &fplain_[1], &fplain_[2], &coords_used_, &fhG_,
                       &attn_part_, &enc2_[0], &enc2_[1], &enc2_[2], &enc2_[3]};
@@ -222,31 +222,7 @@
   if (sf) pack_fragment_major16(arena_, convc1_);
   convc2_ = tap({u + "encoder.convc2"});
   convf1_ = pack_conv(arena_, sd_, {u + "encoder.convf1"}, MODE_ROW, 4);
-  {
-    const HostTensor& w = sd_.get(u + "encoder.convf1.weight");
-    ATDN_CHECK(w.shape[0] == 128 && w.shape[1] == 2 && w.shape[2] == 7 && w.shape[3] == 7, "convf1 is 7x7, 2 -> 128");
-    float mx = 0.f;
-    for (float v : w.data) mx = std::max(mx, std::fabs(v));
-    int e = 0;
-    if (mx > 0.f) (void)std::frexp(mx, &e);
-    const int p = 1 - e;
-    convf1_wscale_ = std::ldexp(1.0f, -p);
-    convf1_sf_off_ = arena_.alloc(4L * 2 * 4 * 2 * 64 * 4);
-    _Float16* f = reinterpret_cast<_Float16*>(arena_.at(convf1_sf_off_));
-    for (int wv = 0; wv < 4; ++wv)
-      for (int cb = 0; cb < 2; ++cb)
-        for (int s = 0; s < 4; ++s)
-          for (int lane = 0; lane < 64; ++lane)
-            for (int i = 0; i < 8; ++i) {
-              const int n = 32 * wv + 16 * cb + (lane & 15), g = lane >> 4;
-              const int ky = 2 * s + (g >> 1), kx = 4 * (g & 1) + (i >> 1), c = i & 1;
-              const float v = (ky < 7 && kx < 7) ? std::ldexp(w.data[(((long)n * 2 + c) * 7 + ky) * 7 + kx], p) : 0.f;
-              const _Float16 hi = (_Float16)v, lo = (_Float16)(v - (float)hi);
-              const long frag = (((long)wv * 2 + cb) * 4 + s) * 2;
-              f[(frag * 64 + lane) * 8 + i] = hi;
-              f[((frag + 1) * 64 + lane) * 8 + i] = lo;
-            }
-  }
+  convf1_sf_off_ = pack_convf1_sf(arena_, sd_.get(u + "encoder.convf1.weight"), &convf1_wscale_);
   convf2_ = tap({u + "encoder.convf2"});
   convm_ = tap({u + "encoder.conv"});
   to_v_ = tap({u + "aggregator.to_v"}, false);
@@ -327,16 +303,18 @@
   z_.alloc(n8 * 128); rh_.alloc(n8 * 128); fh_.alloc(n8 * 256); mask_.alloc(n8 * 576);
   if (sf) fhG_.alloc(2 * n8 * 18);
   coords1_.alloc(n8 * 2); flow4_.alloc(n8 * 4);
+  if (sf) { coords1b_.alloc(n8 * 2); flow4b_.alloc(n8 * 4); }
   if (sf) for (int p = 0; p < 2; ++p) { pre_zr_[p].alloc(n8 * 256); pre_q_[p].alloc(n8 * 128); }
   ATDN_HIP(hipMemset(corrfeat_.p, 0, corrfeat_.n * sizeof(float)));
   ATDN_HIP(hipMemset(vT_.p, 0, vT_.n * sizeof(float)));
   ATDN_HIP(hipMemset(attn_.p, 0, attn_.n * sizeof(float)));
   ATDN_HIP(hipMemset(flow4_.p, 0, flow4_.n * sizeof(float)));
+  if (sf) ATDN_HIP(hipMemset(flow4b_.p, 0, flow4b_.n * sizeof(float)));
   ATDN_HIP(hipDeviceSynchronize());
   ws_bytes_ = 0;
   DeviceBuf* all[] = {&img4_, &enc_[0], &enc_[1], &enc_[2], &enc_[3], &fmap_, &psum_, &pm2_, &pyr_[0], &pyr_[1], &pyr_[2],
                       &pyr_[3], &h_[0], &h_[1], &x_, &qk_, &attn_, &vT_, &corrfeat_, &cor1_, &corflo_, &flo1_, &z_,
-                      &rh_, &fh_, &mask_, &coords1_, &flow4_};
+                      &rh_, &fh_, &mask_, &coords1_, &flow4_, &coords1b_, &flow4b_};
   for (auto* b : all) ws_bytes_ += (size_t)b->n * sizeof(float);
   (void)zero_line();
   sf_counter_attach();
@@ -646,24 +624,39 @@
   *out_buf = X;
 }
 
-void GmaNet::iteration_sf(int B, hipStream_t st) {
+void GmaNet::iteration_sf(int B, hipStream_t st, bool first, bool last) {
   const long n8 = (long)B * N;
   ConvShape s;
   if (par_) fork(st, par_stream_);
-  launch_lookup_conv(brick_pyramid(), coords1_.p, n8, coords_used_.p, convc1_.wf16, convc1_.wscale, convc1_.b, cor1_.p,
+  const bool fused = !par_ && !preds_out_;
+  const SfBias<ACT_RELU> epf2{convf2_.b, corflo_.p + 192, (long)N * 256, 256};
+  const long fh_gs = (long)maxB * N * 18;
+  const ConvShape sf2 = conv_shape(convf2_, flo1_.p, 128, (long)N * 128, B, H8, W8, 1, 1, 1);
+  if (fused && !first) {
+    FlowBranchArgs fa;
+    fa.G = fhG_.p; fa.gstride = fh_gs; fa.fh2_bias = fh2_.b;
+    fa.coords_in = coords_cur(); fa.coords_out = cfb_ ? coords1_.p : coords1b_.p; fa.flow4_out = cfb_ ? flow4_.p : flow4b_.p;
+    fa.x = x_.p; fa.ldx = XLD; fa.xb = (long)N * XLD; fa.cflow = 254;
+    fa.w1frag = arena_.dev(convf1_sf_off_); fa.w1scale = convf1_wscale_; fa.b1 = convf1_.b;
+    launch_flow_branch_sf(sf2, convf2_.wscale, epf2, fa, sf_fast_mode(), st);
+    cfb_ ^= 1;
+    mark(ST_MOTION, st);
+  }
+  launch_lookup_conv(brick_pyramid(), coords_cur(), n8, coords_used_.p, convc1_.wf16, convc1_.wscale, convc1_.b, cor1_.p,
                      sf_fast_mode(), st);
   mark(ST_LOOKUP, st);
   s = conv_shape(convc2_, cor1_.p, 256, (long)N * 256, B, H8, W8, 1, 1, 1);
-  const ConvShape sf2 = conv_shape(convf2_, flo1_.p, 128, (long)N * 128, B, H8, W8, 1, 1, 1);
   if (par_) {
-    launch_flow_conv7_sf(flow4_.p, B, H8, W8, arena_.dev(convf1_sf_off_), convf1_wscale_, convf1_.b, flo1_.p, sf_fast_mode(), par_stream_);
-    conv_sf_dispatch(sf2, convf2_.wscale, SfBias<ACT_RELU>{convf2_.b, corflo_.p + 192, (long)N * 256, 256}, par_stream_);
+    launch_flow_conv7_sf(flow4_cur(), B, H8, W8, arena_.dev(convf1_sf_off_), convf1_wscale_, convf1_.b, flo1_.p, sf_fast_mode(), par_stream_);
+    conv_sf_dispatch(sf2, convf2_.wscale, epf2, par_stream_);
     conv_sf_dispatch(s, convc2_.wscale, SfBias<ACT_RELU>{convc2_.b, corflo_.p, (long)N * 256, 256}, st);
     fork(par_stream_, st);
+  } else if (fused && !first) {
+    conv_sf_dispatch(s, convc2_.wscale, SfBias<ACT_RELU>{convc2_.b, corflo_.p, (long)N * 256, 256}, st);
   } else {
-    launch_flow_conv7_sf(flow4_.p, B, H8, W8, arena_.dev(convf1_sf_off_), convf1_wscale_, convf1_.b, flo1_.p, sf_fast_mode(), st);
+    launch_flow_conv7_sf(flow4_cur(), B, H8, W8, arena_.dev(convf1_sf_off_), convf1_wscale_, convf1_.b, flo1_.p, sf_fast_mode(), st);
     conv_sf_dispatch_pair(s, convc2_.wscale, SfBias<ACT_RELU>{convc2_.b, corflo_.p, (long)N * 256, 256},
-                          sf2, convf2_.wscale, SfBias<ACT_RELU>{convf2_.b, corflo_.p + 192, (long)N * 256, 256}, st);
+                          sf2, convf2_.wscale, epf2, st);
   }
   s = conv_shape(convm_, corflo_.p, 256, (long)N * 256, B, H8, W8, 1, 1, 1);
   float* mf = x_.p + 128;
@@ -694,10 +687,9 @@
   }
 
   s = conv_shape(fh1_, h_[0].p, 128, (long)N * 128, B, H8, W8, 1, 1, 1);
-  const SfFlowDelta fd{fh2_.b, coords1_.p, flow4_.p, x_.p, XLD, (long)N * XLD, 254, W8, (long)N};
-  const long fh_gs = (long)maxB * N * 18;
+  const SfFlowDelta fd{fh2_.b, coords_cur(), flow4_cur(), x_.p, XLD, (long)N * XLD, 254, W8, (long)N};
   launch_flow_head_fused(s, fh1_.wscale, SfFlowHeadPartial{fh1_.b, arena_.dev(fh2_w32_off_), fhG_.p, (long)N, fh2_mul_, 1.0f / fh2_mul_, fh_gs}, st);
-  launch_flow_gather(fhG_.p, fh_gs, B, H8, W8, fd, st);
+  if (!fused || last) launch_flow_gather(fhG_.p, fh_gs, B, H8, W8, fd, st);
   mark(ST_FLOWHEAD, st);
 }
 
@@ -756,11 +748,12 @@
   mark(ST_GRU_CTX, st);
   if (par_) fork(sB, st);
 
+  cfb_ = 0;
   for (int it = 0; it < iters; ++it) {
-    iteration_sf(B, st);
+    iteration_sf(B, st, it == 0, it + 1 == iters);
     if (preds_out_) {
       mask_head_sf(B, st);
-      launch_upsample(mask_.p, flow4_.p, B, H8, W8, nullptr, preds_out_ + it * preds_stride_, st);
+      launch_upsample(mask_.p, flow4_cur(), B, H8, W8, nullptr, preds_out_ + it * preds_stride_, st);
     }
   }
   if (!preds_out_) mask_head_sf(B, st);
@@ -805,6 +798,7 @@
     }
     (void)hipGraphDestroy(graph);
     graphs_[{B, iters * 4 + seq_}] = exec;
+    graph_cfb_[{B, iters * 4 + seq_}] = cfb_;
     return;
   }
 }
@@ -829,7 +823,7 @@
   launch_prep_images(frames, frames + (long)B * frame, B, H, W, img4_.p, st, 1);
   launch_init_coords_sf(flow_init, B, H8, W8, coords1_.p, flow4_.p, x_.p, XLD, 254, st);
   launch_body(B, iters, st);
-  launch_upsample(mask_.p, flow4_.p, B, H8, W8, flow_low, flow_up, st);
+  launch_upsample(mask_.p, flow4_cur(), B, H8, W8, flow_low, flow_up, st);
   last_frame_ = B;
 }
 
@@ -839,6 +833,7 @@
     auto key = std::make_pair(B, iters * 4 + seq_);
     if (!graphs_.count(key)) capture(B, iters);
     ATDN_HIP(hipGraphLaunch(graphs_[key], st));
+    cfb_ = graph_cfb_[key];
   } else {
     if (precision >= 1) { FastGuard fg(precision == 2); run_body_sf(B, iters, st); } else run_body(B, iters, st);
   }
@@ -861,7 +856,7 @@
     probe("flow_init", true, flow4_.p, (long)B * N, 2, 4, st);
   }
   launch_body(B, iters, st);
-  launch_upsample(mask_.p, flow4_.p, B, H8, W8, flow_low, flow_up, st);
+  launch_upsample(mask_.p, flow4_cur(), B, H8, W8, flow_low, flow_up, st);
   if (probe_) {
     probe("flow_low", false, flow_low, 1, 2L * B * N, 2L * B * N, st);
     probe("flow_up", false, flow_up, 1, 2L * B * H * W, 2L * B * H * W, st);
@@ -929,7 +924,7 @@
   if (k == "fmap") b = &fmap_; else if (k == "pyr0") b = &pyr_[0]; else if (k == "pyr1") b = &pyr_[1];
   else if (k == "pyr2") b = &pyr_[2]; else if (k == "pyr3") b = &pyr_[3]; else if (k == "net") b = &h_[0];
   else if (k == "x") b = &x_; else if (k == "attn") b = &attn_; else if (k == "corrfeat") b = &corrfeat_;
-  else if (k == "mask") b = &mask_; else if (k == "coords1") b = &coords1_; else if (k == "flow4") b = &flow4_;
+  else if (k == "mask") b = &mask_; else if (k == "coords1") b = cfb_ ? &coords1b_ : &coords1_; else if (k == "flow4") b = cfb_ ? &flow4b_ : &flow4_;
   else if (k == "qk") b = &qk_; else if (k == "img4") b = &img4_;
   else if (k == "cor1") b = &cor1_;
   if (!b) return -1;
diff --git a/atdn_vslam_amd/csrc/sf.h b/atdn_vslam_amd/csrc/sf.h
--- a/atdn_vslam_amd/csrc/sf.h
+++ b/atdn_vslam_amd/csrc/sf.h
@@ -98,7 +98,7 @@
   asm("v_fma_mixhi_f16 %0, %1, -1.0, %2 op_sel:[1,0,0] op_sel_hi:[1,0,0]" : "+v"(d) : "v"(hp), "v"(b));
   return d;
 }
-__device__ __forceinline__ void sf_store4_flag(float* base, long off, int c, float4 v, bool& clamped) {
+__device__ __forceinline__ void sf_pack4_flag(float4 v, bool& clamped, uint2& hi, uint2& lo) {
   const float lim = 65504.f;
   const float m = fmaxf(fmaxf(fabsf(v.x), fabsf(v.y)), fmaxf(fabsf(v.z), fabsf(v.w)));
   clamped |= !(m <= lim) | __builtin_isunordered(v.x, v.y) | __builtin_isunordered(v.z, v.w);
@@ -106,9 +106,15 @@
   v.z = __builtin_amdgcn_fmed3f(v.z, -lim, lim); v.w = __builtin_amdgcn_fmed3f(v.w, -lim, lim);
   const unsigned h0 = sf_cvt_pk_(v.x, v.y), h1 = sf_cvt_pk_(v.z, v.w);
   const unsigned l0 = sf_residual_pk_(h0, v.x, v.y), l1 = sf_residual_pk_(h1, v.z, v.w);
+  hi = make_uint2(h0, h1);
+  lo = make_uint2(l0, l1);
+}
+__device__ __forceinline__ void sf_store4_flag(float* base, long off, int c, float4 v, bool& clamped) {
+  uint2 hi, lo;
+  sf_pack4_flag(v, clamped, hi, lo);
   _Float16* q = sf_ptr(base, off, c);
-  *reinterpret_cast<uint2*>(q) = make_uint2(h0, h1);
-  *reinterpret_cast<uint2*>(q + 32) = make_uint2(l0, l1);
+  *reinterpret_cast<uint2*>(q) = hi;
+  *reinterpret_cast<uint2*>(q + 32) = lo;
 }
 __device__ __forceinline__ float sf_join_lo_(unsigned hi, unsigned lo) {
   return (float)__builtin_bit_cast(f16x2, hi)[0] + (float)__builtin_bit_cast(f16x2, lo)[0];
diff --git a/atdn_vslam_amd/csrc/small_convs.h b/atdn_vslam_amd/csrc/small_convs.h
--- a/atdn_vslam_amd/csrc/small_convs.h
+++ b/atdn_vslam_amd/csrc/small_convs.h
@@ -10,4 +10,40 @@
 void launch_flow_head_fused(const ConvShape& s, float wscale, const SfFlowHeadPartial& ep, hipStream_t st);
 void launch_flow_gather(const float* G, long gstride, int nimg, int H, int W, const SfFlowDelta& ep, hipStream_t st);
 
+__device__ __forceinline__ float2 flow_gather_sum(const float* __restrict__ G, long gstride, int img, int H, int W, int y, int x) {
+  const long HW = (long)H * W;
+  float s0 = 0.f, s1 = 0.f;
+#pragma unroll
+  for (int t = 0; t < 9; ++t) {
+    const int sy = y + t / 3 - 1, sx = x + t % 3 - 1;
+    if ((unsigned)sy < (unsigned)H && (unsigned)sx < (unsigned)W) {
+      const float* gp = G + ((long)img * HW + (long)sy * W + sx) * 18 + 2 * t;
+      float2 g = *reinterpret_cast<const float2*>(gp);
+      if (gstride) {
+        const float2 g1 = *reinterpret_cast<const float2*>(gp + gstride);
+        g.x += g1.x; g.y += g1.y;
+      }
+      s0 += g.x; s1 += g.y;
+    }
+  }
+  return make_float2(s0, s1);
 }
+__device__ __forceinline__ float4 convf1_act4(float a0, float a1, float a2, float a3, float wscale, float4 b) {
+  return make_float4(fmaxf(a0 * wscale + b.x, 0.f), fmaxf(a1 * wscale + b.y, 0.f), fmaxf(a2 * wscale + b.z, 0.f),
+                     fmaxf(a3 * wscale + b.w, 0.f));
+}
+
+struct FlowBranchArgs {
+  const float* G; long gstride;
+  const float* fh2_bias;
+  const float* coords_in;
+  float* coords_out;
+  float* flow4_out;
+  float* x; int ldx; long xb; int cflow;
+  const float* w1frag; float w1scale;
+  const float* b1;
+};
+void launch_flow_branch_sf(const ConvShape& convf2, float wscale2, const SfBias<ACT_RELU>& ep, const FlowBranchArgs& a, bool fast,
+                           hipStream_t st);
+
+}
diff --git a/atdn_vslam_amd/csrc/small_convs.hip b/atdn_vslam_amd/csrc/small_convs.hip
--- a/atdn_vslam_amd/csrc/small_convs.hip
+++ b/atdn_vslam_amd/csrc/small_convs.hip
@@ -103,8 +103,7 @@
           const long off = (long)img * ob + ((long)oy * W + ox) * 128;
 #pragma unroll
           for (int cb = 0; cb < 2; ++cb) {
-            const float4 o = make_float4(fmaxf(acc[rb][cb][0] * wscale + b4[cb].x, 0.f), fmaxf(acc[rb][cb][1] * wscale + b4[cb].y, 0.f),
-                                         fmaxf(acc[rb][cb][2] * wscale + b4[cb].z, 0.f), fmaxf(acc[rb][cb][3] * wscale + b4[cb].w, 0.f));
+            const float4 o = convf1_act4(acc[rb][cb][0], acc[rb][cb][1], acc[rb][cb][2], acc[rb][cb][3], wscale, b4[cb]);
             sf_store4_flag(out, off, 32 * wave + 16 * cb + 4 * g16, o, clamped);
           }
         }
@@ -137,23 +136,10 @@
   const long HW = (long)H * W;
   const int img = (int)(i / HW), m = (int)(i - img * HW);
   const int y = m / W, x = m - y * W;
-  float s0 = 0.f, s1 = 0.f;
-#pragma unroll
-  for (int t = 0; t < 9; ++t) {
-    const int sy = y + t / 3 - 1, sx = x + t % 3 - 1;
-    if ((unsigned)sy < (unsigned)H && (unsigned)sx < (unsigned)W) {
-      const float* gp = G + ((long)img * HW + (long)sy * W + sx) * 18 + 2 * t;
-      float2 g = *reinterpret_cast<const float2*>(gp);
-      if (gstride) {
-        const float2 g1 = *reinterpret_cast<const float2*>(gp + gstride);
-        g.x += g1.x; g.y += g1.y;
-      }
-      s0 += g.x; s1 += g.y;
-    }
-  }
+  const float2 s = flow_gather_sum(G, gstride, img, H, W, y, x);
   const SfFlowDelta::Aux a0 = ep.load(img, m, 0), a1 = ep.load(img, m, 1);
-  ep.apply(img, m, 0, s0, a0);
-  ep.apply(img, m, 1, s1, a1);
+  ep.apply(img, m, 0, s.x, a0);
+  ep.apply(img, m, 1, s.y, a1);
 }
 
 void launch_flow_gather(const float* G, long gstride, int nimg, int H, int W, const SfFlowDelta& ep, hipStream_t st) {
diff --git a/atdn_vslam_amd/csrc/weights.h b/atdn_vslam_amd/csrc/weights.h
--- a/atdn_vslam_amd/csrc/weights.h
+++ b/atdn_vslam_amd/csrc/weights.h
@@ -234,6 +234,32 @@
   return pack_conv_sf(A, tmp, tnames, nullptr, has_bias);
 }
 
+inline long pack_convf1_sf(WeightArena& A, const HostTensor& w, float* wscale) {
+  ATDN_CHECK(w.shape.size() == 4 && w.shape[0] == 128 && w.shape[1] == 2 && w.shape[2] == 7 && w.shape[3] == 7, "convf1 is 7x7, 2 -> 128");
+  float mx = 0.f;
+  for (float v : w.data) mx = std::max(mx, std::fabs(v));
+  int e = 0;
+  if (mx > 0.f) (void)std::frexp(mx, &e);
+  const int p = 1 - e;
+  *wscale = std::ldexp(1.0f, -p);
+  const long off = A.alloc(4L * 2 * 4 * 2 * 64 * 4);
+  _Float16* f = reinterpret_cast<_Float16*>(A.at(off));
+  for (int wv = 0; wv < 4; ++wv)
+    for (int cb = 0; cb < 2; ++cb)
+      for (int s = 0; s < 4; ++s)
+        for (int lane = 0; lane < 64; ++lane)
+          for (int i = 0; i < 8; ++i) {
+            const int n = 32 * wv + 16 * cb + (lane & 15), g = lane >> 4;
+            const int ky = 2 * s + (g >> 1), kx = 4 * (g & 1) + (i >> 1), c = i & 1;
+            const float v = (ky < 7 && kx < 7) ? std::ldexp(w.data[(((long)n * 2 + c) * 7 + ky) * 7 + kx], p) : 0.f;
+            const _Float16 hi = (_Float16)v, lo = (_Float16)(v - (float)hi);
+            const long frag = (((long)wv * 2 + cb) * 4 + s) * 2;
+            f[(frag * 64 + lane) * 8 + i] = hi;
+            f[((frag + 1) * 64 + lane) * 8 + i] = lo;
+          }
+  return off;
+}
+
 inline long pack_vector(WeightArena& A, const std::vector<float>& v) {
   const long off = A.alloc((long)v.size());
   std::memcpy(A.at(off), v.data(), v.size() * sizeof(float));
diff --git a/include/atdn_hip.h b/include/atdn_hip.h
--- a/include/atdn_hip.h
+++ b/include/atdn_hip.h
@@ -132,6 +132,11 @@
                             float* pyr0, float* pyr1, float* pyr2, float* pyr3, float* samples,
                             const float* convc1_weight_host, const float* convc1_bias_host, float* cor1, void* stream);
 
+int atdn_flow_branch_debug(int fused, int fast, int B, int H8, int W8, const float* G, const float* coords_in,
+                           const float* fh2_bias_host, const float* convf1_weight_host, const float* convf1_bias_host,
+                           const float* convf2_weight_host, const float* convf2_bias_host, float* coords_out, float* flow4_out,
+                           float* x_sf, float* corflo_sf, void* stream);
+
 int atdn_conv2d_nhwc(const float* src, int nimg, int H, int W, int Cin, const float* weight_host,
                      const float* bias_host, int Cout, int KH, int KW, int stride, int padH, int padW, int relu,
                      float* dst, void* stream);
```

Result: no change. 419.7 frame-pairs/s (median of 2 runs) (+0.0%).
